# rebots-online/InstantIR

Measured on AMD Instinct MI355X. Metric: denoising steps/sec at 1024x1024 (InstantIR step: previewer UNet + LCM + Aggregator + UNet, CFG), higher is better.
Workload: dtype f16 (fp32 accumulate)

## Files before the change

### include/instantir_hip.h

```cpp
#ifndef INSTANTIR_HIP_H
#define INSTANTIR_HIP_H

#include <stdint.h>

#ifdef __cplusplus
extern "C" {
#endif

#define IIR_ABI_VERSION 1

#define IIR_EPI_PLAIN 0
#define IIR_EPI_GEGLU 1
#define IIR_EPI_SFT 2
#define IIR_EPI_XATTN 3
#define IIR_ACT_NONE 0
#define IIR_ACT_SILU 1
#define IIR_ACT_GELU 2
#define IIR_ACT_QUICKGELU 3


#define IIR_DT_F16 0
#define IIR_DT_BF16 1

typedef struct iir_attn_kv {
// ... 11 lines not shown
    const void* rowbias; int64_t ldrb; int32_t rows_per_rb;
    const void* res; int64_t ldr;
    int32_t epi, act;
    float out_scale;
    int32_t tile;
    const void* prefetch;
    int64_t prefetch_bytes;
    void* splitk_ws;
    int64_t splitk_ws_bytes;
    void* Ct; int64_t ldct;
    int32_t tr_from;
    int32_t dtype;
    int32_t c_f32;
    const void* wscale;
    void* ln_stats_out;
    const void* ln_stats_in;
    int32_t ln_parts, ln_part_cols;
    float ln_eps;
    const void* ln_colsum;
    void* gn_stats_out;
    const iir_attn_kv* xattn_kv;
    int32_t xattn_tq;
    int32_t a_fp8;
    float a_scale;
    int32_t c_fp8;
} iir_gemm_desc;

int iir_gemm_f16(const iir_gemm_desc* d, void* stream);
int iir_gemm_ln_parts(int32_t M, int32_t N, int32_t K);
int iir_gemm_pick_tile(int32_t M, int32_t N, int32_t K, int32_t paired);
int iir_gemm_resolve_tile(const iir_gemm_desc* d);
int iir_gemm_gn_supported(int32_t M, int32_t N, int32_t K, int32_t is_conv);
int iir_gemm_fp8_out_supported(int32_t M, int32_t N, int32_t K, int32_t paired);
int64_t iir_gemm_splitk_workspace_bytes(int32_t M, int32_t N);
int iir_gemm_uses_splitk(int32_t M, int32_t N, int32_t K, int64_t ws_bytes);
int iir_gemm_tile_bn(int32_t tile);

typedef struct iir_conv_desc {
    const void* X; int64_t ldx;
    int32_t R, H, Wd, Cin;
    const void* Wt;
    void* Y; int64_t ldy;
    int32_t Cout, ksize, stride, upsample;
    const void* bias;
    const void* rowbias; int64_t ldrb; int32_t rows_per_rb;
    const void* res; int64_t ldr;
    int32_t epi, act;
    float out_scale;
    int32_t tile;
    const void* zero_page;
    int64_t x_img_stride;
    int32_t y_img_rows;
    int32_t res_img_rows;
    int32_t pad_mode;
    const void* prefetch;
    int64_t prefetch_bytes;
    void* splitk_ws;
    int64_t splitk_ws_bytes;
    int32_t dtype;
    void* gn_stats_out;
} iir_conv_desc;

int iir_conv2d_nhwc_f16(const iir_conv_desc* c, void* stream);

typedef struct iir_attn_desc {
    const void* Q; int64_t ldq, q_batch_stride;
    void* O; int64_t ldo, o_batch_stride;
    int32_t batch, heads, Tq, nseg;
    float scale;
    iir_attn_kv kv[2];
    int32_t causal;
    int32_t q_prescaled;
    int32_t o_fp8;
} iir_attn_desc;

int iir_attention_d64_f16(const iir_attn_desc* a, void* stream);
int iir_attention_d64_ident_f16(const iir_attn_desc* a, int32_t ident_from, void* stream);

int iir_attention_f16(const iir_attn_desc* a, int32_t head_dim, void* stream);

int iir_groupnorm_nhwc_f16(const void* X, int64_t ldx, void* Y, int64_t ldy, int32_t R, int32_t HW, int32_t C,
                           int32_t groups, const void* gamma, const void* beta, float eps, int32_t silu,
                           void* workspace, int64_t workspace_bytes, void* stream);
int iir_groupnorm_from_partials(const void* partials, int64_t ldp, const void* X, int64_t ldx, void* Y, int64_t ldy, int32_t R,
                                int32_t HW, int32_t C, int32_t groups, const void* gamma, const void* beta, float eps, int32_t silu,
                                void* workspace, int64_t workspace_bytes, int32_t dtype, void* stream);
int iir_groupnorm_nhwc(const void* X, int64_t ldx, void* Y, int64_t ldy, int32_t R, int32_t HW, int32_t C,
                       int32_t groups, const void* gamma, const void* beta, float eps, int32_t silu,
                       void* workspace, int64_t workspace_bytes, int32_t dtype, void* stream);
int64_t iir_groupnorm_workspace_bytes(int32_t R, int32_t groups);

int iir_layernorm_f16(const void* X, int64_t ldx, void* Y, int64_t ldy, int32_t rows, int32_t C, const void* gamma,
                      const void* beta, float eps, const void* shift, const void* scale, int64_t ldmod,
                      int32_t rows_per_mod, int32_t transposed, int32_t tr_rows, int64_t tr_bstride, void* stream);

typedef struct iir_adaln_job {
    const void* X; void* Y; const void* shift; const void* scale;
    int64_t ldx, ldy;
    int32_t C, transposed;
} iir_adaln_job;
int iir_adaln_batch_f16(const iir_adaln_job* jobs_dev, int32_t njobs, int32_t rows, int32_t max_C, float eps, int64_t ldmod,
                        int32_t rows_per_mod, int32_t tr_rows, int64_t tr_bstride, void* stream);

int iir_softmax_rows_f16(void* X, int64_t ld, int32_t rows, int32_t cols, void* stream);
int iir_softmax_rows_f32(const float* S, int64_t lds, void* P, int64_t ldp, int32_t rows, int32_t cols, int32_t dtype, void* stream);

int iir_sinusoid_f16(const float* vals, int32_t n_vals, int32_t rows, int32_t dim, void* out, int64_t ldo,
                     int32_t col_off, void* stream);
int iir_silu_f16(const void* x, void* y, int64_t n, void* stream);

int iir_copy_add_f16(const void* src, int64_t lds, void* dst, int64_t ldd, int64_t dst_off, int64_t M, int32_t C,
                     const void* add, int64_t lda, const float* add_scale, int32_t rows_per_scale, void* stream);

#define IIR_FREEU_SLABS 16
int64_t iir_freeu_partials_bytes(int64_t rows, int32_t H, int32_t W, int32_t C);
int iir_freeu_stats_f16(const void* skip, int64_t lds, const void* add, int64_t lda, const float* add_scale, int64_t rows,
                        int32_t H, int32_t W, int32_t C, float* partials, int64_t partials_bytes, void* stream);
int iir_freeu_concat_f16(const void* x, int64_t ldx, int32_t cx, const void* mid_add, int64_t ldm, const void* skip, int64_t lds,
                         int32_t cs, const void* add, int64_t lda, const float* add_scale, int64_t rows, int32_t H, int32_t W,
                         float b, float s, const float* partials, int64_t partials_bytes, void* cat, int64_t ldc,
                         int64_t cat_off, void* stream);

int iir_pack_latent(const float* x, int32_t B, int32_t C, int32_t HW, void* out, int64_t ldo, int32_t rep, float scale,
                    void* stream);
int iir_unpack_latent(const void* in, int64_t ldi, int32_t R, int32_t C, int32_t HW, float* out, void* stream);
int iir_pack_latent_t(const float* x, int32_t B, int32_t C, int32_t HW, void* out, int64_t ldo, int32_t rep, float scale,
                      int32_t dtype, void* stream);
int iir_unpack_latent_t(const void* in, int64_t ldi, int32_t R, int32_t C, int32_t HW, float* out, int32_t dtype, void* stream);
int iir_pack_latent_dscale(const float* x, int32_t B, int32_t C, int32_t HW, void* out, int64_t ldo, int32_t rep, const float* scale,
                           int32_t dtype, void* stream);

int iir_sched_step(const void* eps_nhwc, int64_t lde, int32_t B, int32_t C, int32_t HW, int32_t cfg, const float* coef,
                   const float* x, const float* noise, float* prev, float* x0_out, float* eps_out,
                   const float* eps_factor, void* stream);
int iir_sched_step_hist(const void* eps_nhwc, int64_t lde, int32_t B, int32_t C, int32_t HW, int32_t cfg, const float* coef,
                        const float* x, const float* noise, float* hist, float* prev, float* x0_out, const float* eps_factor,
                        void* stream);
int iir_cfg_rescale_factor(const void* eps_nhwc, int64_t lde, int32_t B, int32_t C, int32_t HW, const float* coef,
                           float guidance_rescale, float* factor, void* stream);
int iir_sched_step_pag(const void* eps_nhwc, int64_t lde, int32_t B, int32_t C, int32_t HW, int32_t cfg, const float* coef,
                       const float* pag_scale, const float* x, const float* noise, float* prev, float* x0_out, float* eps_out,
                       const float* eps_factor, void* stream);
int iir_sched_step_hist_pag(const void* eps_nhwc, int64_t lde, int32_t B, int32_t C, int32_t HW, int32_t cfg, const float* coef,
                            const float* pag_scale, const float* x, const float* noise, float* hist, float* prev, float* x0_out,
                            const float* eps_factor, void* stream);
int iir_cfg_rescale_factor_pag(const void* eps_nhwc, int64_t lde, int32_t B, int32_t C, int32_t HW, const float* coef,
                               const float* pag_scale, float guidance_rescale, float* factor, void* stream);
int iir_copy_segments(const void* jobs, int32_t njobs, int64_t max_units, void* stream);

int iir_lcm_step(const void* eps_nhwc, int64_t lde, int32_t B, int32_t rep, int32_t C, int32_t HW, const float* coef,
                 const float* x, void* out_nhwc, int64_t ldo, float* out_nchw, void* stream);

int iir_sched_step_f32(const float* eps, const float* x, const float* noise, const float* coef, int64_t n, float* prev,
                       float* x0_out, void* stream);
int iir_axpby_f32(const float* x, const float* y, const float* coef, int64_t n, float* out, void* stream);
int iir_sched_step_hist_f32(const float* eps, const float* x, const float* noise, const float* coef, float* hist, int64_t n,
                            float* prev, float* x0_out, void* stream);

int iir_prefetch(const void* p, int64_t bytes, int32_t blocks, void* stream);

int iir_blend_tiles_f32(const float* a, float* b, int32_t planes, int32_t Ha, int32_t Wa, int32_t Hb, int32_t Wb,
                        int32_t extent, int32_t vertical, void* stream);

#define IIR_COLORFIX_SLABS 64
int64_t iir_colorfix_workspace_bytes(int32_t B, int32_t C, int32_t H, int32_t W);
int iir_colorfix_wavelet_f32(const float* content, const float* style, float* out, int32_t B, int32_t C, int32_t H, int32_t W,
                             void* ws, int64_t ws_bytes, void* stream);
int iir_colorfix_adain_f32(const float* content, const float* style, float* out, int32_t B, int32_t C, int32_t H, int32_t W,
                           void* ws, int64_t ws_bytes, void* stream);

int iir_transpose_f16(const void* in, int64_t ldi, int32_t rows, int32_t cols, void* out, int64_t ldo, int32_t rows_pad,
                      void* stream);
void* iir_timing_event_create(void);
void iir_timing_event_destroy(void* event);
int iir_timing_arm(void* start_event, void* stop_event);
int iir_timing_elapsed_us(void* start_event, void* stop_event, float* us);

int iir_abi_version(void);

#ifdef __cplusplus
}
#endif
#endif
```

### instantir_amd/csrc/freeu.hip

```cpp
#include "common.h"
#include "../../include/instantir_hip.h"

namespace {

constexpr int NSLAB = IIR_FREEU_SLABS;
constexpr int NSUM = 7;
constexpr int CB = 64;
constexpr int RL = 32;
constexpr int CONCAT_ROWS = 256;

__device__ __forceinline__ void phase_sc(int n, int N, float* s, float* c) {
    int m = 2 * n;
    if (m > N) m -= 2 * N;
    sincospif((float)m / (float)N, s, c);
}

__device__ __forceinline__ void pixel_trig(int p, int H, int W, float sc[6]) {
    const int h = p / W, w = p - h * W;
    const int HW = H * W;
    int n11 = h * W + w * H;
    if (n11 >= HW) n11 -= HW;
    phase_sc(h, H, &sc[1], &sc[0]);
    phase_sc(w, W, &sc[3], &sc[2]);
    phase_sc(n11, HW, &sc[5], &sc[4]);
}

__global__ __launch_bounds__(256) void freeu_stats_kernel(const f16* sk, long lds_, const f16* add, long lda, const float* add_scale,
                                                           int H, int W, int C, float* part) {
    __shared__ float red[RL][NSUM][CB];
    const int tid = threadIdx.x, oct = tid & 7, rl = tid >> 3;
    const int r = blockIdx.x / NSLAB, slab = blockIdx.x % NSLAB;
    const int HW = H * W;
    const int per = (HW + NSLAB - 1) / NSLAB;
    const int lo = min(slab * per, HW), hi = min(lo + per, HW);
    const int c0 = blockIdx.y * CB + oct * 8;
    const int cl = min(c0, C - 8);
    const float sc_r = add_scale ? add_scale[r] : 1.0f;
    float acc[NSUM][8];
#pragma unroll
    for (int k = 0; k < NSUM; ++k)
#pragma unroll
        for (int j = 0; j < 8; ++j) acc[k][j] = 0.0f;
    const int iters = (per + RL - 1) / RL;
    for (int it = 0; it < iters; ++it) {
        const int p = lo + it * RL + rl;
        const bool valid = p < hi;
        const int pl = min(p, HW - 1);
        const long m = (long)r * HW + pl;
        f16x8 v = *(const f16x8*)(sk + m * lds_ + cl);
        float t[8];
        if (add) {
            const f16x8 a = *(const f16x8*)(add + m * lda + cl);
#pragma unroll
            for (int j = 0; j < 8; ++j) t[j] = (float)v[j] + (float)a[j] * sc_r;
        } else {
#pragma unroll
            for (int j = 0; j < 8; ++j) t[j] = (float)v[j];
        }
#pragma unroll
        for (int j = 0; j < 8; ++j) t[j] = valid ? t[j] : 0.0f;
        float tr[6];
        pixel_trig(pl, H, W, tr);
#pragma unroll
        for (int j = 0; j < 8; ++j) {
            acc[0][j] += t[j];
#pragma unroll
            for (int k = 0; k < 6; ++k) acc[1 + k][j] += t[j] * tr[k];
        }
    }
#pragma unroll
    for (int k = 0; k < NSUM; ++k)
#pragma unroll
        for (int j = 0; j < 8; ++j) red[rl][k][oct * 8 + j] = acc[k][j];
    __syncthreads();
    for (int idx = tid; idx < NSUM * CB; idx += 256) {
        const int k = idx / CB, c = idx % CB;
        float s = 0.0f;
        for (int q = 0; q < RL; ++q) s += red[q][k][c];
        const int cg = blockIdx.y * CB + c;
        if (cg < C) part[(((long)r * NSLAB + slab) * NSUM + k) * C + cg] = s;
    }
}

__global__ __launch_bounds__(256) void freeu_concat_kernel(const f16* x, long ldx, int cx, const f16* mid, long ldm, const f16* sk,
                                                            long lds_, int cs, const f16* add, long lda, const float* add_scale,
                                                            int H, int W, float b, float s, const float* part, f16* cat,
                                                            long ldc, long cat_off) {
    __shared__ float coef[NSUM][CB];
    const int tid = threadIdx.x, oct = tid & 7, rl = tid >> 3;
    const int HW = H * W;
    const int ntile = (HW + CONCAT_ROWS - 1) / CONCAT_ROWS;
    const int r = blockIdx.x / ntile, p0 = (blockIdx.x % ntile) * CONCAT_ROWS;
    const int nbx = (cx + CB - 1) / CB;
    const float sc_r = add_scale ? add_scale[r] : 1.0f;
    if ((int)blockIdx.y < nbx) {
        const int c0 = blockIdx.y * CB + oct * 8;
        const int cl = min(c0, cx - 8);
        const int half = cx / 2;
#pragma unroll 4
        for (int i = 0; i < CONCAT_ROWS / RL; ++i) {
            const int p = p0 + i * RL + rl;
            const long m = (long)r * HW + min(p, HW - 1);
            const f16x8 v = *(const f16x8*)(x + m * ldx + cl);
            float t[8];
            if (mid) {
                const f16x8 a = *(const f16x8*)(mid + m * ldm + cl);
#pragma unroll
                for (int j = 0; j < 8; ++j) t[j] = (float)v[j] + (float)a[j] * sc_r;
            } else {
#pragma unroll
                for (int j = 0; j < 8; ++j) t[j] = (float)v[j];
            }
            f16x8 o;
#pragma unroll
            for (int j = 0; j < 8; ++j) o[j] = (f16)(cl + j < half ? t[j] * b : t[j]);
            if (p < HW && c0 < cx) *(f16x8*)(cat + m * ldc + cat_off + c0) = o;
        }
        return;
    }
    const int cb = blockIdx.y - nbx;
    for (int idx = tid; idx < NSUM * CB; idx += 256) {
        const int k = idx / CB, c = idx % CB;
        const int cc = min(cb * CB + c, cs - 1);
        float a = 0.0f;
        for (int sl = 0; sl < NSLAB; ++sl) a += part[(((long)r * NSLAB + sl) * NSUM + k) * cs + cc];
        const bool keep = k == 0 || ((k == 1 || k == 2) && H > 1) || ((k == 3 || k == 4) && W > 1) || (k >= 5 && H > 1 && W > 1);
        coef[k][c] = keep ? a : 0.0f;
    }
    __syncthreads();
    const int c0 = cb * CB + oct * 8;
    const int cl = min(c0, cs - 8);
    float cf[NSUM][8];
#pragma unroll
    for (int k = 0; k < NSUM; ++k)
#pragma unroll
        for (int j = 0; j < 8; ++j) cf[k][j] = coef[k][oct * 8 + j];
    const float ks = (s - 1.0f) / (float)HW;
#pragma unroll 4
    for (int i = 0; i < CONCAT_ROWS / RL; ++i) {
        const int p = p0 + i * RL + rl;
        const int pl = min(p, HW - 1);
        const long m = (long)r * HW + pl;
        const f16x8 v = *(const f16x8*)(sk + m * lds_ + cl);
        float t[8];
        if (add) {
            const f16x8 a = *(const f16x8*)(add + m * lda + cl);
#pragma unroll
            for (int j = 0; j < 8; ++j) t[j] = (float)v[j] + (float)a[j] * sc_r;
        } else {
#pragma unroll
            for (int j = 0; j < 8; ++j) t[j] = (float)v[j];
        }
        if (ks != 0.0f) {
            float tr[6];
            pixel_trig(pl, H, W, tr);
#pragma unroll
            for (int j = 0; j < 8; ++j) {
                float corr = cf[0][j];
#pragma unroll
                for (int k = 0; k < 6; ++k) corr = corr + cf[1 + k][j] * tr[k];
                t[j] = t[j] + ks * corr;
            }
        }
        f16x8 o;
#pragma unroll
        for (int j = 0; j < 8; ++j) o[j] = (f16)t[j];
        if (p < HW && c0 < cs) *(f16x8*)(cat + m * ldc + cat_off + cx + c0) = o;
    }
}

long planes(int64_t rows, int32_t H, int32_t W) {
    if (rows <= 0 || H < 1 || W < 1 || H > 65535 || W > 65535) return -1;
    const int64_t HW = (int64_t)H * W;
    if (HW > (1 << 26) || rows % HW) return -1;
    const int64_t R = rows / HW;
    if (R > 65535) return -1;
    return (long)R;
}

}

extern "C" int64_t iir_freeu_partials_bytes(int64_t rows, int32_t H, int32_t W, int32_t C) {
    const long R = planes(rows, H, W);
    if (R < 0 || C <= 0 || C % 8) return -1;
    return (int64_t)R * NSLAB * NSUM * C * (int64_t)sizeof(float);
}

extern "C" int iir_freeu_stats_f16(const void* skip, int64_t lds, const void* add, int64_t lda, const float* add_scale, int64_t rows,
                                   int32_t H, int32_t W, int32_t C, float* partials, int64_t partials_bytes, void* stream) {
    (void)hipGetLastError();
    const long R = planes(rows, H, W);
    if (!skip || !partials || R < 0 || C <= 0 || C % 8 || lds % 8 || lds < C) return IIR_EINVAL;
    if (add && (lda % 8 || lda < C)) return IIR_EINVAL;
    if (partials_bytes < iir_freeu_partials_bytes(rows, H, W, C)) return IIR_EINVAL;
    hipLaunchKernelGGL(freeu_stats_kernel, dim3((unsigned)(R * NSLAB), (C + CB - 1) / CB), dim3(256), 0, (hipStream_t)stream,
                       (const f16*)skip, (long)lds, (const f16*)add, (long)lda, add_scale, H, W, C, partials);
    return iir_launch_status();
}

extern "C" int iir_freeu_concat_f16(const void* x, int64_t ldx, int32_t cx, const void* mid_add, int64_t ldm, const void* skip,
                                    int64_t lds, int32_t cs, const void* add, int64_t lda, const float* add_scale, int64_t rows,
                                    int32_t H, int32_t W, float b, float s, const float* partials, int64_t partials_bytes,
                                    void* cat, int64_t ldc, int64_t cat_off, void* stream) {
    (void)hipGetLastError();
    const long R = planes(rows, H, W);
    if (!x || !skip || !cat || !partials || R < 0) return IIR_EINVAL;
    if (cx <= 0 || cx % 8 || cs <= 0 || cs % 8 || ldx % 8 || ldx < cx || lds % 8 || lds < cs) return IIR_EINVAL;
    if (mid_add && (ldm % 8 || ldm < cx)) return IIR_EINVAL;
    if (add && (lda % 8 || lda < cs)) return IIR_EINVAL;
    if (ldc % 8 || cat_off < 0 || cat_off % 8 || ldc < cat_off + cx + cs) return IIR_EINVAL;
    if (partials_bytes < iir_freeu_partials_bytes(rows, H, W, cs)) return IIR_EINVAL;
    const int64_t HW = (int64_t)H * W;
    const int ntile = (int)((HW + CONCAT_ROWS - 1) / CONCAT_ROWS);
    hipLaunchKernelGGL(freeu_concat_kernel, dim3((unsigned)(R * ntile), (cx + CB - 1) / CB + (cs + CB - 1) / CB), dim3(256), 0,
                       (hipStream_t)stream, (const f16*)x, (long)ldx, cx, (const f16*)mid_add, (long)ldm, (const f16*)skip, (long)lds,
                       cs, (const f16*)add, (long)lda, add_scale, H, W, b, s, partials, (f16*)cat, (long)ldc, (long)cat_off);
    return iir_launch_status();
}
```

### instantir_amd/csrc/norm.hip

```cpp
#include "common.h"
#include "../../include/instantir_hip.h"

namespace {

constexpr int GN_MAXC = 2560;
constexpr int GN_MIN_PIX = 8;

__device__ __forceinline__ void chan_merge(float& n, float& mean, float& m2, float nb, float mb, float m2b) {
    if (nb <= 0.f) return;
    const float tot = n + nb, d = mb - mean;
    mean += d * (nb / tot);
    m2 += m2b + d * d * (n * nb / tot);
    n = tot;
}

template <typename E>
__global__ __launch_bounds__(256) void gn_stats_kernel(const f16* Xp, long ldx, int HW, int C, int G, int pix_per_slab,
                                                       float* part ) {
    using E8 = typename ET<E>::x8;
    const E* X = (const E*)Xp;
    __shared__ float cmean[2048], cm2[2048];
    __shared__ float chmean[GN_MAXC], chm2[GN_MAXC];
    const int r = blockIdx.y, slab = blockIdx.x, nslab = gridDim.x;
    const int nchunk = C >> 3;
    const int p0 = slab * pix_per_slab;
    const int p1 = min(HW, p0 + pix_per_slab);
    const E* base = X + (long)r * HW * ldx;
    const int lanes_c = nchunk < 256 ? nchunk : 256;
    const int prows = 256 / lanes_c;
    const int tc = threadIdx.x % lanes_c, tp = threadIdx.x / lanes_c;
    for (int c0 = 0; c0 < nchunk; c0 += lanes_c) {
        const int ch = c0 + tc;
        if (tp < prows && ch < nchunk) {
            float s[8], q[8], k0[8];
#pragma unroll
            for (int j = 0; j < 8; ++j) { s[j] = 0.f; q[j] = 0.f; k0[j] = 0.f; }
            int p = p0 + tp, cnt = 0;
            if (p < p1) {
                const E8 v = *(const E8*)(base + (long)p * ldx + ch * 8);
#pragma unroll
                for (int j = 0; j < 8; ++j) k0[j] = (float)v[j];
            }
            for (; p + 3 * prows < p1; p += 4 * prows) {
                E8 v[4];
#pragma unroll
                for (int u = 0; u < 4; ++u) v[u] = *(const E8*)(base + (long)(p + u * prows) * ldx + ch * 8);
#pragma unroll
                for (int u = 0; u < 4; ++u)
#pragma unroll
                    for (int j = 0; j < 8; ++j) { const float f = (float)v[u][j] - k0[j]; s[j] += f; q[j] += f * f; }
                cnt += 4;
            }
            for (; p < p1; p += prows) {
                const E8 v = *(const E8*)(base + (long)p * ldx + ch * 8);
#pragma unroll
                for (int j = 0; j < 8; ++j) { const float f = (float)v[j] - k0[j]; s[j] += f; q[j] += f * f; }
                cnt += 1;
            }
            const float inv = cnt > 0 ? 1.0f / (float)cnt : 0.f;
#pragma unroll
            for (int j = 0; j < 8; ++j) {
                cmean[(tp * lanes_c + tc) * 8 + j] = k0[j] + s[j] * inv;
                cm2[(tp * lanes_c + tc) * 8 + j] = fmaxf(q[j] - s[j] * s[j] * inv, 0.f);
            }
        }
        __syncthreads();
        for (int c = threadIdx.x; c < lanes_c * 8 && c0 * 8 + c < C; c += 256) {
            float n = 0.f, mean = 0.f, m2 = 0.f;
            for (int t = 0; t < prows; ++t) {
                const int first = p0 + t;
                const float nt = first < p1 ? (float)((p1 - first + prows - 1) / prows) : 0.f;
                chan_merge(n, mean, m2, nt, cmean[t * lanes_c * 8 + c], cm2[t * lanes_c * 8 + c]);
            }
            chmean[c0 * 8 + c] = mean; chm2[c0 * 8 + c] = m2;
        }
        __syncthreads();
    }
    const int cpg = C / G;
    const float npix = (float)(p1 - p0);
    for (int gi = threadIdx.x; gi < G; gi += 256) {
        float n = 0.f, mean = 0.f, m2 = 0.f;
        for (int c = gi * cpg; c < (gi + 1) * cpg; ++c) chan_merge(n, mean, m2, npix, chmean[c], chm2[c]);
        float* o = part + (((long)r * nslab + slab) * G + gi) * 2;
        o[0] = mean; o[1] = m2;
    }
}

__global__ __launch_bounds__(256) void gn_finalize_kernel(const float* part, int nslab, int G, int HW, int pix_per_slab, int cpg,
                                                          float eps, float* stat , int gblocks) {
    __shared__ float sn[256], smean[256], sm2[256];
    const int r = blockIdx.x / gblocks, gb = blockIdx.x - r * gblocks;
    const int g8 = threadIdx.x & 7, sl = threadIdx.x >> 3;
    const int gi = gb * 8 + g8;
    constexpr int MAXS = 8;
    float n = 0.f, mean = 0.f, m2 = 0.f;
    if (gi < G) {
        const float* base = part + ((long)r * nslab * G + gi) * 2;
        float2 a[MAXS];
#pragma unroll
        for (int k = 0; k < MAXS; ++k) {
            const int s_ = min(sl + k * 32, nslab - 1);
            a[k] = *(const float2*)(base + (long)s_ * G * 2);
        }
#pragma unroll
        for (int k = 0; k < MAXS; ++k) {
            const int s_ = sl + k * 32;
            if (s_ < nslab) {
                const int p0 = s_ * pix_per_slab, p1 = min(HW, p0 + pix_per_slab);
                chan_merge(n, mean, m2, (float)(p1 - p0) * (float)cpg, a[k].x, a[k].y);
            }
        }
    }
    sn[threadIdx.x] = n; smean[threadIdx.x] = mean; sm2[threadIdx.x] = m2;
    __syncthreads();
    if (threadIdx.x < 64) {
        const int seg = threadIdx.x >> 3;
        float tn = 0.f, tm = 0.f, tq = 0.f;
#pragma unroll
        for (int l = 0; l < 4; ++l) {
            const int src = (seg * 4 + l) * 8 + g8;
            chan_merge(tn, tm, tq, sn[src], smean[src], sm2[src]);
        }
        n = tn; mean = tm; m2 = tq;
    }
    __syncthreads();
    if (threadIdx.x < 64) { sn[threadIdx.x] = n; smean[threadIdx.x] = mean; sm2[threadIdx.x] = m2; }
    __syncthreads();
    if (threadIdx.x < 8 && gi < G) {
        float tn = 0.f, tm = 0.f, tq = 0.f;
#pragma unroll
        for (int sgm = 0; sgm < 8; ++sgm) chan_merge(tn, tm, tq, sn[sgm * 8 + g8], smean[sgm * 8 + g8], sm2[sgm * 8 + g8]);
        stat[((long)r * G + gi) * 2] = tm;
        stat[((long)r * G + gi) * 2 + 1] = rsqrtf(tq / tn + eps);
    }
}

__global__ __launch_bounds__(256) void gn_finalize_cols_kernel(const float2* part, long ldp, int slabs_per_img, int G, int cpg, float eps,
                                                               float* stat ) {
    __shared__ float red[256];
    const int r = blockIdx.x / G, gi = blockIdx.x - r * G;
    const int n = slabs_per_img * cpg;
    constexpr int MAXP = 20;
    float2 a[MAXP];
    const float2* base = part + (long)r * slabs_per_img * ldp + gi * cpg;
#pragma unroll
    for (int k = 0; k < MAXP; ++k) {
        const int i = min((int)threadIdx.x + k * 256, n - 1);
        const int sl = i / cpg, c = i - sl * cpg;
        a[k] = base[(long)sl * ldp + c];
    }
    auto block_sum = [&](float v) {
        red[threadIdx.x] = v;
        __syncthreads();
#pragma unroll
        for (int o = 128; o > 0; o >>= 1) {
            if ((int)threadIdx.x < o) red[threadIdx.x] += red[threadIdx.x + o];
            __syncthreads();
        }
        const float t = red[0];
        __syncthreads();
        return t;
    };
    float sm = 0.f;
#pragma unroll
    for (int k = 0; k < MAXP; ++k) sm += ((int)threadIdx.x + k * 256 < n) ? a[k].x : 0.f;
    const float mean = block_sum(sm) / (float)n;
    float q = 0.f;
#pragma unroll
    for (int k = 0; k < MAXP; ++k) {
        const float d = a[k].x - mean;
        q += ((int)threadIdx.x + k * 256 < n) ? fmaf(64.0f * d, d, a[k].y) : 0.f;
    }
    const float m2 = block_sum(q);
    if (threadIdx.x == 0) {
        stat[((long)r * G + gi) * 2] = mean;
        stat[((long)r * G + gi) * 2 + 1] = rsqrtf(m2 / ((float)n * 64.0f) + eps);
    }
}

template <typename E>
__global__ __launch_bounds__(256) void gn_apply_kernel(const f16* Xp, long ldx, f16* Yp, long ldy, int HW, int C, int G,
                                                       int pix_per_blk, const float* stat, const f16* gammap,
                                                       const f16* betap, int silu) {
    using E8 = typename ET<E>::x8;
    const E* X = (const E*)Xp; E* Y = (E*)Yp; const E* gamma = (const E*)gammap; const E* beta = (const E*)betap;
    const int r = blockIdx.y;
    const int cpg = C / G;
    const int nchunk = C >> 3;
    const int lanes_c = nchunk < 256 ? nchunk : 256;
    const int prows = 256 / lanes_c;
    const int tc = threadIdx.x % lanes_c, tp = threadIdx.x / lanes_c;
    if (tp >= prows) return;
    const int p0 = blockIdx.x * pix_per_blk;
    const int p1 = min(HW, p0 + pix_per_blk);
    const E* xb = X + (long)r * HW * ldx;
    E* yb = Y + (long)r * HW * ldy;
    const float* st = stat + (long)r * G * 2;
    for (int ch = tc; ch < nchunk; ch += lanes_c) {
        float a[8], b[8];
        const E8 gm = *(const E8*)(gamma + ch * 8), bt = *(const E8*)(beta + ch * 8);
#pragma unroll
        for (int j = 0; j < 8; ++j) {
            const int gi = (ch * 8 + j) / cpg;
            const float mean = st[gi * 2], rstd = st[gi * 2 + 1];
            a[j] = rstd * (float)gm[j];
            b[j] = (float)bt[j] - mean * a[j];
        }
        for (int p = p0 + tp; p < p1; p += prows) {
            const E8 v = *(const E8*)(xb + (long)p * ldx + ch * 8);
            E8 o;
#pragma unroll
            for (int j = 0; j < 8; ++j) {
                float f = fmaf((float)v[j], a[j], b[j]);
                if (silu) f = silu_f(f);
                o[j] = (E)f;
            }
            *(E8*)(yb + (long)p * ldy + ch * 8) = o;
        }
    }
}

__device__ __forceinline__ void ln_row(const f16* X, long ldx, f16* Y, long ldy, int row, int C, const f16* gamma,
                                       const f16* beta, float eps, const f16* shift, const f16* scale, long ldmod,
                                       int rows_per_mod, int transposed, int tr_rows, long tr_bstride) {
    const int lane = threadIdx.x & 63;
    const int nchunk = C >> 3;
    constexpr int MAXK = GN_MAXC / 8 / 64;
    f16x8 v[MAXK];
    float s = 0.f;
    const f16* x = X + (long)row * ldx;
#pragma unroll
    for (int k = 0; k < MAXK; ++k) v[k] = *(const f16x8*)(x + min(lane + k * 64, nchunk - 1) * 8);
#pragma unroll
    for (int k = 0; k < MAXK; ++k) {
        const int ch = lane + k * 64;
        if (ch < nchunk) {
#pragma unroll
            for (int j = 0; j < 8; ++j) s += (float)v[k][j];
        }
    }
    const float mean = wave_sum(s) / (float)C;
    float q = 0.f;
#pragma unroll
    for (int k = 0; k < MAXK; ++k) {
        const int ch = lane + k * 64;
        if (ch < nchunk) {
#pragma unroll
            for (int j = 0; j < 8; ++j) { const float d = (float)v[k][j] - mean; q += d * d; }
        }
    }
    const float rstd = rsqrtf(wave_sum(q) / (float)C + eps);
    const f16* sh = shift ? shift + (long)(row / rows_per_mod) * ldmod : nullptr;
    const f16* sc = scale ? scale + (long)(row / rows_per_mod) * ldmod : nullptr;
#pragma unroll
    for (int k = 0; k < MAXK; ++k) {
        const int ch = lane + k * 64;
        if (ch < nchunk) {
            f16x8 o;
            f16x8 gm, bt, s8, c8;
            if (gamma) gm = *(const f16x8*)(gamma + ch * 8);
            if (beta) bt = *(const f16x8*)(beta + ch * 8);
            if (sh) { s8 = *(const f16x8*)(sh + ch * 8); c8 = *(const f16x8*)(sc + ch * 8); }
#pragma unroll
            for (int j = 0; j < 8; ++j) {
                float f = ((float)v[k][j] - mean) * rstd;
                if (gamma) f *= (float)gm[j];
                if (beta) f += (float)bt[j];
                if (sh) f = f * (1.0f + (float)c8[j]) + (float)s8[j];
                o[j] = (f16)f;
            }
            if (transposed == 2) {
                *(long*)((char*)Y + (long)row * ldy + ch * 8) = iir_fp8x8(o);
            } else if (!transposed) {
                *(f16x8*)(Y + (long)row * ldy + ch * 8) = o;
            } else {
                const long col = (long)(row / tr_rows) * tr_bstride + (row % tr_rows);
#pragma unroll
                for (int j = 0; j < 8; ++j) Y[(long)(ch * 8 + j) * ldy + col] = o[j];
            }
        }
    }
}

__global__ __launch_bounds__(256) void ln_kernel(const f16* X, long ldx, f16* Y, long ldy, int rows, int C, const f16* gamma,
                                                 const f16* beta, float eps, const f16* shift, const f16* scale, long ldmod,
                                                 int rows_per_mod, int transposed, int tr_rows, long tr_bstride) {
    const int row = blockIdx.x * 4 + (threadIdx.x >> 6);
    if (row >= rows) return;
    ln_row(X, ldx, Y, ldy, row, C, gamma, beta, eps, shift, scale, ldmod, rows_per_mod, transposed, tr_rows, tr_bstride);
}

__global__ __launch_bounds__(256) void adaln_batch_kernel(const iir_adaln_job* jobs, int rows, float eps, long ldmod,
                                                          int rows_per_mod, int tr_rows, long tr_bstride) {
    const int row = blockIdx.x * 4 + (threadIdx.x >> 6);
    if (row >= rows) return;
    const iir_adaln_job j = jobs[blockIdx.y];
    ln_row((const f16*)j.X, j.ldx, (f16*)j.Y, j.ldy, row, j.C, nullptr, nullptr, eps, (const f16*)j.shift, (const f16*)j.scale,
           ldmod, rows_per_mod, j.transposed, tr_rows, tr_bstride);
}

__global__ __launch_bounds__(256) void softmax_rows_kernel(f16* X, long ld, int cols) {
    __shared__ float red[4];
// ... 10 lines not shown
        const int ch = threadIdx.x + k * 256;
        if (ch < nchunk) {
#pragma unroll
            for (int j = 0; j < 8; ++j) mx = fmaxf(mx, (float)v[k][j]);
        }
    }
    mx = wave_max(mx);
    if (lane == 0) red[wv] = mx;
    __syncthreads();
    mx = fmaxf(fmaxf(red[0], red[1]), fmaxf(red[2], red[3]));
    __syncthreads();
    float e[MAXK][8];
    float sum = 0.f;
#pragma unroll
    for (int k = 0; k < MAXK; ++k) {
        const int ch = threadIdx.x + k * 256;
        if (ch < nchunk) {
#pragma unroll
            for (int j = 0; j < 8; ++j) { e[k][j] = __expf((float)v[k][j] - mx); sum += e[k][j]; }
        }
    }
    sum = wave_sum(sum);
    if (lane == 0) red[wv] = sum;
    __syncthreads();
    const float inv = 1.0f / (red[0] + red[1] + red[2] + red[3]);
#pragma unroll
    for (int k = 0; k < MAXK; ++k) {
        const int ch = threadIdx.x + k * 256;
        if (ch < nchunk) {
            f16x8 o;
#pragma unroll
            for (int j = 0; j < 8; ++j) o[j] = (f16)(e[k][j] * inv);
            *(f16x8*)(x + ch * 8) = o;
        }
    }
}

template <typename E>
__global__ __launch_bounds__(256) void softmax_rows_f32_kernel(const float* S, long lds, f16* Pp, long ldp, int cols) {
    using E4 = typename ET<E>::x4;
    __shared__ float red[4];
    const float* x = S + (long)blockIdx.x * lds;
    E* y = (E*)Pp + (long)blockIdx.x * ldp;
    const int nchunk = cols >> 2;
    const int lane = threadIdx.x & 63, wv = threadIdx.x >> 6;
    constexpr int MAXK = 16;
    f32x4 v[MAXK];
    float mx = -INFINITY;
#pragma unroll
    for (int k = 0; k < MAXK; ++k) v[k] = *(const f32x4*)(x + min((int)threadIdx.x + k * 256, nchunk - 1) * 4);
#pragma unroll
    for (int k = 0; k < MAXK; ++k) {
        const int ch = threadIdx.x + k * 256;
        if (ch < nchunk) mx = fmaxf(fmaxf(mx, fmaxf(v[k][0], v[k][1])), fmaxf(v[k][2], v[k][3]));
    }
    mx = wave_max(mx);
    if (lane == 0) red[wv] = mx;
    __syncthreads();
    mx = fmaxf(fmaxf(red[0], red[1]), fmaxf(red[2], red[3]));
    __syncthreads();
    float sum = 0.f;
#pragma unroll
    for (int k = 0; k < MAXK; ++k) {
        const int ch = threadIdx.x + k * 256;
        if (ch < nchunk) {
#pragma unroll
            for (int j = 0; j < 4; ++j) { v[k][j] = __expf(v[k][j] - mx); sum += v[k][j]; }
        }
    }
    sum = wave_sum(sum);
    if (lane == 0) red[wv] = sum;
    __syncthreads();
    const float inv = 1.0f / (red[0] + red[1] + red[2] + red[3]);
#pragma unroll
    for (int k = 0; k < MAXK; ++k) {
        const int ch = threadIdx.x + k * 256;
        if (ch < nchunk) {
            E4 o;
#pragma unroll
            for (int j = 0; j < 4; ++j) o[j] = (E)(v[k][j] * inv);
            *(E4*)(y + ch * 4) = o;
        }
    }
}

}

extern "C" int iir_softmax_rows_f32(const float* S, int64_t lds, void* P, int64_t ldp, int32_t rows, int32_t cols, int32_t dtype,
                                    void* stream) {
    (void)hipGetLastError();
    if (!S || !P || rows <= 0 || cols <= 0 || cols % 4 || cols > 16384 || lds % 4 || ldp % 4) return IIR_EINVAL;
    if (dtype == IIR_DT_BF16) hipLaunchKernelGGL(softmax_rows_f32_kernel<bf16>, dim3(rows), dim3(256), 0, (hipStream_t)stream, S, (long)lds, (f16*)P, (long)ldp, cols);
    else if (dtype == IIR_DT_F16) hipLaunchKernelGGL(softmax_rows_f32_kernel<f16>, dim3(rows), dim3(256), 0, (hipStream_t)stream, S, (long)lds, (f16*)P, (long)ldp, cols);
    else return IIR_EINVAL;
    return iir_launch_status();
}

extern "C" int iir_softmax_rows_f16(void* X, int64_t ld, int32_t rows, int32_t cols, void* stream) {
    (void)hipGetLastError();
    if (!X || rows <= 0 || cols <= 0 || cols % 8 || cols > 16384 || ld % 8) return IIR_EINVAL;
    hipLaunchKernelGGL(softmax_rows_kernel, dim3(rows), dim3(256), 0, (hipStream_t)stream, (f16*)X, (long)ld, cols);
    return iir_launch_status();
}

extern "C" int iir_groupnorm_nhwc(const void* X, int64_t ldx, void* Y, int64_t ldy, int32_t R, int32_t HW, int32_t C,
                                  int32_t groups, const void* gamma, const void* beta, float eps, int32_t silu,
                                  void* workspace, int64_t workspace_bytes, int32_t dtype, void* stream) {
    (void)hipGetLastError();
    if (!X || !Y || !gamma || !beta || !workspace) return IIR_EINVAL;
    if (C % 8 || C > GN_MAXC || groups <= 0 || groups > 64 || C % groups || ldx % 8 || ldy % 8) return IIR_EINVAL;
    if (R <= 0 || HW <= 0 || (dtype != IIR_DT_F16 && dtype != IIR_DT_BF16)) return IIR_EINVAL;
    int nslab = (HW + GN_MIN_PIX - 1) / GN_MIN_PIX;
    const int want = (1024 + R - 1) / R;
    if (nslab > want) nslab = want;
    if (nslab > 256) nslab = 256;
    if (nslab < 1) nslab = 1;
    const int pps = (HW + nslab - 1) / nslab;
    nslab = (HW + pps - 1) / pps;
    const int64_t part_floats = (int64_t)R * nslab * groups * 2;
    if ((part_floats + (int64_t)R * groups * 2) * 4 > workspace_bytes) return IIR_EINVAL;
    float* part = (float*)workspace;
    float* stat = part + part_floats;
    const hipStream_t st = (hipStream_t)stream;
    int nblk = (1024 + R - 1) / R;
    int ppb = (HW + nblk - 1) / nblk; if (ppb < GN_MIN_PIX) ppb = GN_MIN_PIX;
    nblk = (HW + ppb - 1) / ppb;
    if (dtype == IIR_DT_BF16) hipLaunchKernelGGL(gn_stats_kernel<bf16>, dim3(nslab, R), dim3(256), 0, st, (const f16*)X, (long)ldx, HW, C, groups, pps, part);
    else hipLaunchKernelGGL(gn_stats_kernel<f16>, dim3(nslab, R), dim3(256), 0, st, (const f16*)X, (long)ldx, HW, C, groups, pps, part);
    const int gblocks = (groups + 7) / 8;
    hipLaunchKernelGGL(gn_finalize_kernel, dim3(R * gblocks), dim3(256), 0, st, (const float*)part, nslab, groups, HW, pps, C / groups, eps, stat, gblocks);
    if (dtype == IIR_DT_BF16) hipLaunchKernelGGL(gn_apply_kernel<bf16>, dim3(nblk, R), dim3(256), 0, st, (const f16*)X, (long)ldx, (f16*)Y, (long)ldy, HW, C, groups, ppb, (const float*)stat, (const f16*)gamma, (const f16*)beta, silu);
    else hipLaunchKernelGGL(gn_apply_kernel<f16>, dim3(nblk, R), dim3(256), 0, st, (const f16*)X, (long)ldx, (f16*)Y, (long)ldy, HW, C, groups, ppb, (const float*)stat, (const f16*)gamma, (const f16*)beta, silu);
    return iir_launch_status();
}

extern "C" int iir_groupnorm_from_partials(const void* partials, int64_t ldp, const void* X, int64_t ldx, void* Y, int64_t ldy, int32_t R,
                                           int32_t HW, int32_t C, int32_t groups, const void* gamma, const void* beta, float eps,
                                           int32_t silu, void* workspace, int64_t workspace_bytes, int32_t dtype, void* stream) {
    (void)hipGetLastError();
    if (!partials || !X || !Y || !gamma || !beta || !workspace || (uintptr_t)partials % 8) return IIR_EINVAL;
    if (C % 8 || C > GN_MAXC || groups <= 0 || groups > 64 || C % groups || ldx % 8 || ldy % 8 || ldp < C) return IIR_EINVAL;
    if (R <= 0 || HW <= 0 || HW % 64 || (dtype != IIR_DT_F16 && dtype != IIR_DT_BF16)) return IIR_EINVAL;
    const int slabs = HW / 64, cpg = C / groups;
    if ((long)slabs * cpg > 20 * 256) return IIR_EINVAL;
    if ((int64_t)R * groups * 2 * 4 > workspace_bytes) return IIR_EINVAL;
    float* stat = (float*)workspace;
    const hipStream_t st = (hipStream_t)stream;
    hipLaunchKernelGGL(gn_finalize_cols_kernel, dim3(R * groups), dim3(256), 0, st, (const float2*)partials, (long)ldp, slabs, groups, cpg, eps, stat);
    int nblk = (1024 + R - 1) / R;
    int ppb = (HW + nblk - 1) / nblk; if (ppb < GN_MIN_PIX) ppb = GN_MIN_PIX;
    nblk = (HW + ppb - 1) / ppb;
    if (dtype == IIR_DT_BF16) hipLaunchKernelGGL(gn_apply_kernel<bf16>, dim3(nblk, R), dim3(256), 0, st, (const f16*)X, (long)ldx, (f16*)Y, (long)ldy, HW, C, groups, ppb, (const float*)stat, (const f16*)gamma, (const f16*)beta, silu);
    else hipLaunchKernelGGL(gn_apply_kernel<f16>, dim3(nblk, R), dim3(256), 0, st, (const f16*)X, (long)ldx, (f16*)Y, (long)ldy, HW, C, groups, ppb, (const float*)stat, (const f16*)gamma, (const f16*)beta, silu);
    return iir_launch_status();
}

extern "C" int iir_groupnorm_nhwc_f16(const void* X, int64_t ldx, void* Y, int64_t ldy, int32_t R, int32_t HW, int32_t C,
                                      int32_t groups, const void* gamma, const void* beta, float eps, int32_t silu,
                                      void* workspace, int64_t workspace_bytes, void* stream) {
    return iir_groupnorm_nhwc(X, ldx, Y, ldy, R, HW, C, groups, gamma, beta, eps, silu, workspace, workspace_bytes, IIR_DT_F16, stream);
}

extern "C" int64_t iir_groupnorm_workspace_bytes(int32_t R, int32_t groups) { return (int64_t)R * 257 * groups * 2 * 4; }

extern "C" int iir_layernorm_f16(const void* X, int64_t ldx, void* Y, int64_t ldy, int32_t rows, int32_t C, const void* gamma,
                                 const void* beta, float eps, const void* shift, const void* scale, int64_t ldmod,
                                 int32_t rows_per_mod, int32_t transposed, int32_t tr_rows, int64_t tr_bstride, void* stream) {
    (void)hipGetLastError();
    if (!X || !Y || rows <= 0 || C % 8 || C > GN_MAXC || ldx % 8) return IIR_EINVAL;
    if ((shift == nullptr) != (scale == nullptr)) return IIR_EINVAL;
    if (shift && (rows_per_mod <= 0 || ldmod % 8)) return IIR_EINVAL;
    if (transposed < 0 || transposed > 2) return IIR_EINVAL;
    if (transposed != 1 && ldy % 8) return IIR_EINVAL;
    if (transposed == 1 && tr_rows <= 0) return IIR_EINVAL;
    hipLaunchKernelGGL(ln_kernel, dim3((rows + 3) / 4), dim3(256), 0, (hipStream_t)stream, (const f16*)X, (long)ldx, (f16*)Y,
                       (long)ldy, rows, C, (const f16*)gamma, (const f16*)beta, eps, (const f16*)shift, (const f16*)scale,
                       (long)ldmod, rows_per_mod, transposed, tr_rows, (long)tr_bstride);
    return iir_launch_status();
}

extern "C" int iir_adaln_batch_f16(const iir_adaln_job* jobs_dev, int32_t njobs, int32_t rows, int32_t max_C, float eps,
                                   int64_t ldmod, int32_t rows_per_mod, int32_t tr_rows, int64_t tr_bstride, void* stream) {
    (void)hipGetLastError();
    if (!jobs_dev || njobs <= 0 || njobs > 65535 || rows <= 0 || rows_per_mod <= 0) return IIR_EINVAL;
    if (max_C <= 0 || max_C > GN_MAXC || max_C % 8) return IIR_EINVAL;
    hipLaunchKernelGGL(adaln_batch_kernel, dim3((rows + 3) / 4, njobs), dim3(256), 0, (hipStream_t)stream, jobs_dev, rows, eps,
                       (long)ldmod, rows_per_mod, tr_rows, (long)tr_bstride);
    return iir_launch_status();
}
```

### instantir_amd/csrc/pointwise.hip

```cpp
#include "common.h"
#include "../../include/instantir_hip.h"

namespace {

__global__ void sinusoid_kernel(const float* vals, int n_vals, int rows, int dim, f16* out, long ldo, int col_off) {
    const int half = dim >> 1;
    const int idx = blockIdx.x * blockDim.x + threadIdx.x;
    const int total = rows * n_vals * half;
    if (idx >= total) return;
    const int k = idx % half;
    const int v = (idx / half) % n_vals;
    const int r = idx / (half * n_vals);
    const float w = expf(-9.210340371976184f * (float)k / (float)half);
    const float a = vals[r * n_vals + v] * w;
    f16* o = out + (long)r * ldo + col_off + v * dim;
    o[k] = (f16)cosf(a);
    o[half + k] = (f16)sinf(a);
}

__global__ void silu_kernel(const f16* x, f16* y, long n8) {
    const long i = (long)blockIdx.x * blockDim.x + threadIdx.x;
    if (i >= n8) return;
    const f16x8 v = *(const f16x8*)(x + i * 8);
    f16x8 o;
#pragma unroll
    for (int j = 0; j < 8; ++j) o[j] = (f16)silu_f((float)v[j]);
    *(f16x8*)(y + i * 8) = o;
}

__global__ void copy_add_kernel(const f16* src, long lds_, f16* dst, long ldd, long dst_off, long M, int C, const f16* add,
                                long lda, const float* add_scale, int rows_per_scale) {
    const int nchunk = C >> 3;
    const long i = (long)blockIdx.x * blockDim.x + threadIdx.x;
    if (i >= M * nchunk) return;
    const long m = i / nchunk;
    const int ch = (int)(i % nchunk);
    f16x8 v = *(const f16x8*)(src + m * lds_ + ch * 8);
    if (add) {
        const f16x8 a = *(const f16x8*)(add + m * lda + ch * 8);
        const float s = add_scale ? add_scale[m / rows_per_scale] : 1.0f;
#pragma unroll
        for (int j = 0; j < 8; ++j) v[j] = (f16)((float)v[j] + (float)a[j] * s);
    }
    *(f16x8*)(dst + m * ldd + dst_off + ch * 8) = v;
}

template <typename E>
__global__ void pack_latent_kernel(const float* x, int B, int C, int HW, E* out, long ldo, int rep, float scale) {
    const long i = (long)blockIdx.x * blockDim.x + threadIdx.x;
    if (i >= (long)B * HW) return;
    const int b = (int)(i / HW), p = (int)(i % HW);
    for (int c = 0; c < C; ++c) {
        const E v = (E)(x[((long)b * C + c) * HW + p] * scale);
        for (int k = 0; k < rep; ++k) out[((long)(k * B + b) * HW + p) * ldo + c] = v;
    }
}

template <typename E>
__global__ void unpack_latent_kernel(const E* in, long ldi, int R, int C, int HW, float* out) {
    const long i = (long)blockIdx.x * blockDim.x + threadIdx.x;
    if (i >= (long)R * HW) return;
    const int r = (int)(i / HW), p = (int)(i % HW);
    for (int c = 0; c < C; ++c) out[((long)r * C + c) * HW + p] = (float)in[((long)r * HW + p) * ldi + c];
}

template <bool PAG>
__global__ __launch_bounds__(1024) void cfg_rescale_kernel(const f16* eps_nhwc, long lde, int B, int C, int HW, const float* coef,
                                                           const float* pag_s, float phi, float* factor) {
    __shared__ double red[4][16];
    const int b = blockIdx.x;
    const float g = coef[0];
    const float ps = PAG ? *pag_s : 0.f;
    double st = 0., st2 = 0., sc = 0., sc2 = 0.;
    for (int p = threadIdx.x; p < HW; p += blockDim.x)
        for (int c = 0; c < C; ++c) {
            const float u = (float)eps_nhwc[((long)b * HW + p) * lde + c];
            const float t = (float)eps_nhwc[((long)(B + b) * HW + p) * lde + c];
            float e = u + g * (t - u);
            if (PAG && ps != 0.f) e = e + ps * (t - (float)eps_nhwc[((long)(2 * B + b) * HW + p) * lde + c]);
            st += t; st2 += (double)t * t; sc += e; sc2 += (double)e * e;
        }
    double v[4] = {st, st2, sc, sc2};
    const int lane = threadIdx.x & 63, wv = threadIdx.x >> 6;
    for (int k = 0; k < 4; ++k) {
        for (int o = 32; o > 0; o >>= 1) v[k] += __shfl_xor(v[k], o, 64);
        if (lane == 0) red[k][wv] = v[k];
    }
    __syncthreads();
    if (threadIdx.x == 0) {
        const int nw = blockDim.x >> 6;
        double s[4] = {0., 0., 0., 0.};
        for (int k = 0; k < 4; ++k)
            for (int w = 0; w < nw; ++w) s[k] += red[k][w];
        const double n = (double)C * HW;
        const double var_t = (s[1] - s[0] * s[0] / n) / (n - 1.), var_c = (s[3] - s[2] * s[2] / n) / (n - 1.);
        factor[b] = (float)((double)phi * sqrt(var_t / var_c) + (1. - (double)phi));
    }
}

template <bool PAG>
__device__ __forceinline__ float guided_eps(const f16* eps_nhwc, long lde, int B, int HW, int cfg, float g, float ps,
                                            const float* eps_factor, int b, int p, int c) {
    float e;
    if (cfg) {
        const float u = (float)eps_nhwc[((long)b * HW + p) * lde + c];
        const float t = (float)eps_nhwc[((long)(B + b) * HW + p) * lde + c];
        e = u + g * (t - u);
        if (PAG && ps != 0.f) e = e + ps * (t - (float)eps_nhwc[((long)(2 * B + b) * HW + p) * lde + c]);
        if (eps_factor) e *= eps_factor[b];
    } else {
        e = (float)eps_nhwc[((long)b * HW + p) * lde + c];
        if (PAG && ps != 0.f) e = e + ps * (e - (float)eps_nhwc[((long)(B + b) * HW + p) * lde + c]);
    }
    return e;
}

template <bool PAG>
__global__ void sched_step_kernel(const f16* eps_nhwc, long lde, int B, int C, int HW, int cfg, const float* coef,
                                  const float* pag_s, const float* x, const float* noise, float* prev, float* x0_out,
                                  float* eps_out, const float* eps_factor) {
    const long i = (long)blockIdx.x * blockDim.x + threadIdx.x;
    if (i >= (long)B * HW) return;
    const int b = (int)(i / HW), p = (int)(i % HW);
    const float g = coef[0], sb = coef[1], sa = coef[2], k0 = coef[3], k1 = coef[4], k2 = coef[5], k3 = coef[6];
    const float ps = PAG ? *pag_s : 0.f;
    for (int c = 0; c < C; ++c) {
        const long o = ((long)b * C + c) * HW + p;
// ... 38 lines not shown
    for (int j = threadIdx.y; j < 32; j += blockDim.y) {
        const int c = bx + j, r = by + threadIdx.x;
        if (c < cols && r < rows_pad) out[(long)c * ldo + r] = tile[threadIdx.x][j];
    }
}

template <typename E>
__global__ void pack_latent_dscale_kernel(const float* x, int B, int C, int HW, E* out, long ldo, int rep, const float* scale_dev) {
    const long i = (long)blockIdx.x * blockDim.x + threadIdx.x;
    if (i >= (long)B * HW) return;
    const float scale = *scale_dev;
    const int b = (int)(i / HW), p = (int)(i % HW);
    for (int c = 0; c < C; ++c) {
        const E v = (E)(x[((long)b * C + c) * HW + p] * scale);
        for (int k = 0; k < rep; ++k) out[((long)(k * B + b) * HW + p) * ldo + c] = v;
    }
}

template <bool PAG>
__global__ void sched_step_hist_kernel(const f16* eps_nhwc, long lde, int B, int C, int HW, int cfg, const float* coef,
                                       const float* pag_s, const float* x, const float* noise, float* hist, float* prev,
                                       float* x0_out, const float* eps_factor) {
    const long i = (long)blockIdx.x * blockDim.x + threadIdx.x;
    if (i >= (long)B * HW) return;
    const int b = (int)(i / HW), p = (int)(i % HW);
    const float g = coef[0], sb = coef[1], sa = coef[2], k0 = coef[3], k1 = coef[4], k2 = coef[5], k3 = coef[6], kh = coef[7];
    const float ps = PAG ? *pag_s : 0.f;
    for (int c = 0; c < C; ++c) {
        const long o = ((long)b * C + c) * HW + p;
        const float e = guided_eps<PAG>(eps_nhwc, lde, B, HW, cfg, g, ps, eps_factor, b, p, c);
        const float xv = x[o];
        const float x0 = (xv - sb * e) / sa;
        float pv = k0 * x0 + k1 * xv;
        if (k2 != 0.f) pv = pv + k2 * e;
        if (kh != 0.f) pv = pv + kh * hist[o];
        if (noise && k3 != 0.f) pv = pv + k3 * noise[o];
        prev[o] = pv;
        hist[o] = x0;
        if (x0_out) x0_out[o] = x0;
    }
}

__global__ void copy_segments_kernel(const long long* jobs) {
    const long long* jb = jobs + 3 * blockIdx.y;
    const long n = (long)jb[2];
    const uint4* src = (const uint4*)jb[0];
    uint4* dst = (uint4*)jb[1];
    for (long i = (long)blockIdx.x * blockDim.x + threadIdx.x; i < n; i += (long)gridDim.x * blockDim.x) dst[i] = src[i];
}

inline int nblk(long n, int t) { return (int)((n + t - 1) / t); }

}

extern "C" int iir_sinusoid_f16(const float* vals, int32_t n_vals, int32_t rows, int32_t dim, void* out, int64_t ldo,
                                int32_t col_off, void* stream) {
    (void)hipGetLastError();
    if (!vals || !out || n_vals <= 0 || rows <= 0 || dim <= 0 || dim % 2) return IIR_EINVAL;
    const int total = rows * n_vals * (dim / 2);
    hipLaunchKernelGGL(sinusoid_kernel, dim3(nblk(total, 256)), dim3(256), 0, (hipStream_t)stream, vals, n_vals, rows, dim,
                       (f16*)out, (long)ldo, col_off);
    return iir_launch_status();
}

extern "C" int iir_silu_f16(const void* x, void* y, int64_t n, void* stream) {
    (void)hipGetLastError();
    if (!x || !y || n <= 0 || n % 8) return IIR_EINVAL;
    hipLaunchKernelGGL(silu_kernel, dim3(nblk(n / 8, 256)), dim3(256), 0, (hipStream_t)stream, (const f16*)x, (f16*)y, n / 8);
    return iir_launch_status();
}

extern "C" int iir_copy_add_f16(const void* src, int64_t lds, void* dst, int64_t ldd, int64_t dst_off, int64_t M, int32_t C,
                                const void* add, int64_t lda, const float* add_scale, int32_t rows_per_scale, void* stream) {
    (void)hipGetLastError();
    if (!src || !dst || M <= 0 || C <= 0 || C % 8 || lds % 8 || ldd % 8 || dst_off % 8) return IIR_EINVAL;
    if (add && (lda % 8)) return IIR_EINVAL;
    if (add_scale && rows_per_scale <= 0) return IIR_EINVAL;
    hipLaunchKernelGGL(copy_add_kernel, dim3(nblk(M * (C / 8), 256)), dim3(256), 0, (hipStream_t)stream, (const f16*)src,
                       (long)lds, (f16*)dst, (long)ldd, (long)dst_off, (long)M, C, (const f16*)add, (long)lda, add_scale,
                       rows_per_scale);
    return iir_launch_status();
}

extern "C" int iir_pack_latent_t(const float* x, int32_t B, int32_t C, int32_t HW, void* out, int64_t ldo, int32_t rep,
                                 float scale, int32_t dtype, void* stream) {
    (void)hipGetLastError();
    if (!x || !out || B <= 0 || C <= 0 || HW <= 0 || rep <= 0 || ldo < C) return IIR_EINVAL;
    if (dtype == IIR_DT_BF16) hipLaunchKernelGGL(pack_latent_kernel<bf16>, dim3(nblk((long)B * HW, 256)), dim3(256), 0, (hipStream_t)stream, x, B, C, HW, (bf16*)out, (long)ldo, rep, scale);
    else if (dtype == IIR_DT_F16) hipLaunchKernelGGL(pack_latent_kernel<f16>, dim3(nblk((long)B * HW, 256)), dim3(256), 0, (hipStream_t)stream, x, B, C, HW, (f16*)out, (long)ldo, rep, scale);
    else return IIR_EINVAL;
    return iir_launch_status();
}

extern "C" int iir_pack_latent(const float* x, int32_t B, int32_t C, int32_t HW, void* out, int64_t ldo, int32_t rep,
                               float scale, void* stream) {
    return iir_pack_latent_t(x, B, C, HW, out, ldo, rep, scale, IIR_DT_F16, stream);
}

extern "C" int iir_pack_latent_dscale(const float* x, int32_t B, int32_t C, int32_t HW, void* out, int64_t ldo, int32_t rep,
                                      const float* scale, int32_t dtype, void* stream) {
    (void)hipGetLastError();
    if (!x || !out || !scale || B <= 0 || C <= 0 || HW <= 0 || rep <= 0 || ldo < C) return IIR_EINVAL;
    if (dtype != IIR_DT_F16 && dtype != IIR_DT_BF16) return IIR_EINVAL;
    if (dtype == IIR_DT_BF16) hipLaunchKernelGGL(pack_latent_dscale_kernel<bf16>, dim3(nblk((long)B * HW, 256)), dim3(256), 0, (hipStream_t)stream, x, B, C, HW, (bf16*)out, (long)ldo, rep, scale);
    else hipLaunchKernelGGL(pack_latent_dscale_kernel<f16>, dim3(nblk((long)B * HW, 256)), dim3(256), 0, (hipStream_t)stream, x, B, C, HW, (f16*)out, (long)ldo, rep, scale);
    return iir_launch_status();
}

extern "C" int iir_unpack_latent_t(const void* in, int64_t ldi, int32_t R, int32_t C, int32_t HW, float* out, int32_t dtype,
                                   void* stream) {
    (void)hipGetLastError();
    if (!in || !out || R <= 0 || C <= 0 || HW <= 0 || ldi < C) return IIR_EINVAL;
    if (dtype == IIR_DT_BF16) hipLaunchKernelGGL(unpack_latent_kernel<bf16>, dim3(nblk((long)R * HW, 256)), dim3(256), 0, (hipStream_t)stream, (const bf16*)in, (long)ldi, R, C, HW, out);
    else if (dtype == IIR_DT_F16) hipLaunchKernelGGL(unpack_latent_kernel<f16>, dim3(nblk((long)R * HW, 256)), dim3(256), 0, (hipStream_t)stream, (const f16*)in, (long)ldi, R, C, HW, out);
    else return IIR_EINVAL;
    return iir_launch_status();
}

extern "C" int iir_unpack_latent(const void* in, int64_t ldi, int32_t R, int32_t C, int32_t HW, float* out, void* stream) {
    return iir_unpack_latent_t(in, ldi, R, C, HW, out, IIR_DT_F16, stream);
}

extern "C" int iir_cfg_rescale_factor(const void* eps_nhwc, int64_t lde, int32_t B, int32_t C, int32_t HW, const float* coef,
                                      float guidance_rescale, float* factor, void* stream) {
    (void)hipGetLastError();
    if (!eps_nhwc || !coef || !factor || B <= 0 || C <= 0 || HW <= 0 || lde < C || (long)C * HW < 2) return IIR_EINVAL;
    hipLaunchKernelGGL(cfg_rescale_kernel<false>, dim3(B), dim3(1024), 0, (hipStream_t)stream, (const f16*)eps_nhwc, (long)lde, B, C,
                       HW, coef, (const float*)nullptr, guidance_rescale, factor);
    return iir_launch_status();
}

extern "C" int iir_cfg_rescale_factor_pag(const void* eps_nhwc, int64_t lde, int32_t B, int32_t C, int32_t HW, const float* coef,
                                          const float* pag_scale, float guidance_rescale, float* factor, void* stream) {
    if (!eps_nhwc || !coef || !pag_scale || !factor || B <= 0 || C <= 0 || HW <= 0 || lde < C || (long)C * HW < 2) return IIR_EINVAL;
    (void)hipGetLastError();
    hipLaunchKernelGGL(cfg_rescale_kernel<true>, dim3(B), dim3(1024), 0, (hipStream_t)stream, (const f16*)eps_nhwc, (long)lde, B, C,
                       HW, coef, pag_scale, guidance_rescale, factor);
    return iir_launch_status();
}

extern "C" int iir_sched_step(const void* eps_nhwc, int64_t lde, int32_t B, int32_t C, int32_t HW, int32_t cfg,
                              const float* coef, const float* x, const float* noise, float* prev, float* x0_out,
                              float* eps_out, const float* eps_factor, void* stream) {
    (void)hipGetLastError();
    if (!eps_nhwc || !coef || !x || !prev || B <= 0 || C <= 0 || HW <= 0 || lde < C) return IIR_EINVAL;
    if (eps_factor && !cfg) return IIR_EINVAL;
    hipLaunchKernelGGL(sched_step_kernel<false>, dim3(nblk((long)B * HW, 256)), dim3(256), 0, (hipStream_t)stream,
                       (const f16*)eps_nhwc, (long)lde, B, C, HW, cfg, coef, (const float*)nullptr, x, noise, prev, x0_out, eps_out,
                       eps_factor);
    return iir_launch_status();
}

extern "C" int iir_sched_step_pag(const void* eps_nhwc, int64_t lde, int32_t B, int32_t C, int32_t HW, int32_t cfg,
                                  const float* coef, const float* pag_scale, const float* x, const float* noise, float* prev,
                                  float* x0_out, float* eps_out, const float* eps_factor, void* stream) {
    if (!eps_nhwc || !coef || !pag_scale || !x || !prev || B <= 0 || C <= 0 || HW <= 0 || lde < C) return IIR_EINVAL;
    if (eps_factor && !cfg) return IIR_EINVAL;
    (void)hipGetLastError();
    hipLaunchKernelGGL(sched_step_kernel<true>, dim3(nblk((long)B * HW, 256)), dim3(256), 0, (hipStream_t)stream,
                       (const f16*)eps_nhwc, (long)lde, B, C, HW, cfg, coef, pag_scale, x, noise, prev, x0_out, eps_out, eps_factor);
    return iir_launch_status();
}

extern "C" int iir_sched_step_hist(const void* eps_nhwc, int64_t lde, int32_t B, int32_t C, int32_t HW, int32_t cfg,
                                   const float* coef, const float* x, const float* noise, float* hist, float* prev, float* x0_out,
                                   const float* eps_factor, void* stream) {
// ... 174 lines not shown
```

### instantir_amd/engine.py

```python
from __future__ import annotations

import os

from typing import Dict, List, Optional

import torch

from . import ops, pag
from .config import UNetConfig
from .packing import conv_weight_nhwc, pair_rows
from .weights import skip_channels

F16 = torch.float16
CPAD = 64


class _NullOps:

    def __getattr__(self, name):
        return lambda *a, **k: None


class Arena:

# ... 7 lines not shown
    def reserve(self, n_elems):
        self.buf = torch.empty(n_elems, dtype=self.dtype, device=self.device)

    def alloc(self, rows, cols):
        n = (rows * cols + 127) // 128 * 128
        off = self.off
        self.off += n
        self.high = max(self.high, self.off)
        if self.buf is None:
            return torch.empty(rows, cols, dtype=self.dtype, device="meta")
        if self.off > self.buf.numel():
            raise RuntimeError("activation arena overflow (forward differs from its sizing run)")
        return self.buf[off:off + rows * cols].view(rows, cols)

    def mark(self):
        return self.off

    def release(self, m):
        self.off = m

    def reset(self):
        self.off = 0


def _merge_lora(sd: Dict[str, torch.Tensor], lora: Dict[str, torch.Tensor], scaling: float) -> Dict[str, torch.Tensor]:
    out = dict(sd)
    for k in lora:
        if not k.endswith(".lora_A.weight"):
            continue
        path = k[: -len(".lora_A.weight")]
        w = sd[path + ".weight"]
        dev = w.device
        if not w.is_cuda:
            raise RuntimeError("_merge_lora: weights must be on the GPU (the merge runs in the HIP library)")
        a, b = lora[k].to(dev), lora[path + ".lora_B.weight"].to(dev)
        r = a.shape[0]
        rp = (r + 63) // 64 * 64
        n_out = w.shape[0]
        kk = w.numel() // n_out
        bs = torch.zeros(n_out, rp, dtype=F16, device=dev)
        bs[:, :r] = (b.reshape(n_out, r).float() * scaling).to(F16)
        at = torch.zeros(kk, rp, dtype=F16, device=dev)
        at[:, :r] = a.reshape(r, kk).t().to(F16)
        w2 = w.reshape(n_out, kk).to(F16).contiguous()
        merged = torch.empty_like(w2)
        ops.gemm(bs, at, merged, res=w2)
        out[path + ".weight"] = merged.reshape(w.shape).to(w.dtype)
    return out


class _RecDict(dict):

    def __init__(self, base, note):
        super().__init__(base)
        self._note = note

    def __getitem__(self, k):
        self._note(k)
        return dict.__getitem__(self, k)


class _Net:

    def __init__(self, cfg: UNetConfig, sd: Dict[str, torch.Tensor], cross: bool, device, fp8_linear: bool = False):
        self.cfg = cfg
        self.cross = cross
        self.device = device
        self.fp8_linear = fp8_linear
        self.arena = Arena(device)
        self.o = ops
        self.w: Dict[str, torch.Tensor] = {}
        self._temb_slices: Dict[str, slice] = {}
        self._ada_slices: Dict[str, slice] = {}
        self.units: List[tuple] = []
        self._use_log: Optional[list] = None
        self._gnws = None
        self._skws = None
        self._warena = None
        self.inkernel_prefetch = True
        self.arena_gen = 0
        self.fuse_qkv = os.environ.get("IIR_FUSE_QKV", "1") != "0"
        self.ln_fold = os.environ.get("IIR_LN_FOLD", "1") != "0" and not fp8_linear
        self.gn_fuse = os.environ.get("IIR_GN_FUSE", "1") != "0"
        self.xattn_fuse = os.environ.get("IIR_XATTN_FUSE", "1") != "0"
        self.pag = None
        self.fp8_act = fp8_linear and os.environ.get("IIR_FP8_ACT", "1") != "0"
        self._pack_encoder(sd)

    def _t(self, sd, name):
        return sd[name].to(device=self.device, dtype=F16)

    def _qw(self, sd, name):
        f = ops.attn_q_factor(self.cfg.head_dim ** -0.5)
        return (sd[name].to(device=self.device, dtype=torch.float32) * f).to(F16)

    def _pack_linear(self, sd, path, dst=None):
        dst = dst or path
        self.w[dst + ".w"] = self._t(sd, path + ".weight").contiguous()
        if (path + ".bias") in sd:
            self.w[dst + ".b"] = self._t(sd, path + ".bias").contiguous()

    def _pack_conv3(self, sd, path, cin_pad=None):
        self.w[path + ".w"] = conv_weight_nhwc(self._t(sd, path + ".weight"), cin_pad)
        self.w[path + ".b"] = self._t(sd, path + ".bias").contiguous()

    def _pack_fold(self, dst, w32, sd, norm, bias=None, pair=None):
        f = ops.LnFold(w32, sd[norm + ".weight"].to(self.device), sd[norm + ".bias"].to(self.device), bias=bias, eps=1e-5, pair=pair)
        self.w[dst + ".lnw"], self.w[dst + ".lnb"], self.w[dst + ".lncs"] = f.w, f.bias, f.colsum

    def _pack_norm(self, sd, path):
        self.w[path + ".g"] = self._t(sd, path + ".weight").contiguous()
        self.w[path + ".b"] = self._t(sd, path + ".bias").contiguous()

    def _pack_resnet(self, sd, path, temb_list):
        self._pack_norm(sd, path + ".norm1")
        self._pack_conv3(sd, path + ".conv1")
        self._pack_norm(sd, path + ".norm2")
        self._pack_conv3(sd, path + ".conv2")
        temb_list.append((path, self._t(sd, path + ".time_emb_proj.weight"), self._t(sd, path + ".time_emb_proj.bias")))
        if (path + ".conv_shortcut.weight") in sd:
            w = self._t(sd, path + ".conv_shortcut.weight")
            self.w[path + ".conv_shortcut.w"] = w.reshape(w.shape[0], w.shape[1]).contiguous()
            self.w[path + ".conv_shortcut.b"] = self._t(sd, path + ".conv_shortcut.bias").contiguous()

    def _pack_transformer(self, sd, path, depth, ada_list):
        self._pack_norm(sd, path + ".norm")
        self._pack_linear(sd, path + ".proj_in")
        self._pack_linear(sd, path + ".proj_out")
        for k in range(depth):
            p = f"{path}.transformer_blocks.{k}"
            self._pack_norm(sd, p + ".norm1")
            self.w[p + ".attn1.qkv.w"] = torch.cat([self._qw(sd, p + ".attn1.to_q.weight"), self._t(sd, p + ".attn1.to_k.weight"),
                                                    self._t(sd, p + ".attn1.to_v.weight")], 0).contiguous()
            f32 = lambda n_: sd[n_].to(device=self.device, dtype=torch.float32)
            qf = ops.attn_q_factor(self.cfg.head_dim ** -0.5)
            if self.ln_fold:
                self._pack_fold(p + ".attn1.qkv", torch.cat([f32(p + ".attn1.to_q.weight") * qf, f32(p + ".attn1.to_k.weight"),
                                                             f32(p + ".attn1.to_v.weight")], 0), sd, p + ".norm1")
            self._pack_linear(sd, p + ".attn1.to_out.0")
            if self.cross:
                self._pack_norm(sd, p + ".norm2")
                if self.ln_fold:
                    self._pack_fold(p + ".attn2.to_q", f32(p + ".attn2.to_q.weight") * qf, sd, p + ".norm2")
                self.w[p + ".attn2.to_q.w"] = self._qw(sd, p + ".attn2.to_q.weight").contiguous()
                self._pack_linear(sd, p + ".attn2.to_k")
                self._pack_linear(sd, p + ".attn2.to_v")
                self._pack_linear(sd, p + ".attn2.to_out.0")
                pp = p + ".attn2.processor"
                self._pack_linear(sd, pp + ".to_k_ip")
                self._pack_linear(sd, pp + ".to_v_ip")
                for kv in ("k", "v"):
                    ada_list.append((f"{p}.{kv}", self._t(sd, f"{pp}.ln_{kv}_ip.linear.weight"), self._t(sd, f"{pp}.ln_{kv}_ip.linear.bias")))
            self._pack_norm(sd, p + ".norm3")
            w1, b1 = self._t(sd, p + ".ff.net.0.proj.weight"), self._t(sd, p + ".ff.net.0.proj.bias")
            n = w1.shape[0] // 2
            self.w[p + ".ff1.w"] = pair_rows(w1[:n], w1[n:])
            self.w[p + ".ff1.b"] = pair_rows(b1[:n], b1[n:])
            if self.ln_fold:
                self._pack_fold(p + ".ff1", f32(p + ".ff.net.0.proj.weight"), sd, p + ".norm3", bias=f32(p + ".ff.net.0.proj.bias"), pair=pair_rows)
            self._pack_linear(sd, p + ".ff.net.2", p + ".ff2")
            if self.fp8_linear:
                for key in ([p + ".attn1.qkv.w", p + ".attn1.to_out.0.w", p + ".ff1.w", p + ".ff2.w"]
                            + ([p + ".attn2.to_q.w", p + ".attn2.to_out.0.w"] if self.cross else [])):
                    self.w[key] = ops.Fp8Weight(*ops.quantize_fp8_rows(self.w[key]))
        if self.fp8_linear:
            for key in (path + ".proj_in.w", path + ".proj_out.w"):
# ... 46 lines not shown
            self._skws = torch.zeros(4096 + 256 * 128 * 160 * 4, dtype=torch.uint8, device=self.device)
        if first:
            self._use_log = []
            self.w = _RecDict(plain, lambda k: self._use_log.append(k))
        try:
            fn()
        finally:
            self.o = ops
            self.w = plain
        if first:
            self._consolidate_weights()
        self.arena.reserve(self.arena.high + 1024)
        self.arena.reset()

    def _consolidate_weights(self):
        order, seen, marks = [], set(), []
        for k in self._use_log:
            if isinstance(k, tuple):
                marks.append(len(order))
            elif k not in seen:
                seen.add(k)
                order.append(k)
        order += [k for k in self.w if k not in seen]
        order = [k for k in order if torch.is_tensor(self.w[k]) and self.w[k].dtype == F16]
        al = lambda n: (n + 127) // 128 * 128
        offs, tot = [], 0
        for k in order:
            offs.append(tot)
            tot += al(self.w[k].numel())
        arena = torch.empty(tot, dtype=F16, device=self.device)
        for k, off in zip(order, offs):
            t = self.w[k]
            v = arena[off:off + t.numel()].view(t.shape)
            v.copy_(t)
            self.w[k] = v
        self._warena = arena
        self.units = [None]
        self._use_log = None

    def _unit(self, name):
        if self._use_log is not None:
            self._use_log.append(("unit", name))

    import os as _os
    PF_MULT = float(_os.environ.get("IIR_PF_MULT", "1"))
    PF_LOOKAHEAD = int(_os.environ.get("IIR_PF_MB", "0")) << 20

    def _pf(self, wt):
        if not self.inkernel_prefetch or self._warena is None or self.o is not ops:
            return None
        base, end = self._warena.data_ptr(), self._warena.data_ptr() + self._warena.numel() * 2
        n = wt.numel() * 2
        lo = wt.data_ptr() + n + self.PF_LOOKAHEAD
        if lo < base or lo >= end or n < (256 << 10):
            return None
        return (lo, min(int(n * self.PF_MULT), end - lo))

    def _begin(self):
        self.arena.reset()

    def _gn_alloc(self, rows, hw, C, K, conv):
        if not self.gn_fuse or hw % 64 or self.arena.dtype != F16 or not ops.gn_supported(rows, C, K, conv):
            return None
        if (hw // 64) * (C // self.cfg.norm_groups) > ops.GN_PARTIALS_MAX:
            return None
        return self.arena.alloc(rows // 64 * C, 4).view(torch.float32).view(rows // 64, C, 2)

    @staticmethod
    def _gn_of(x):
        return getattr(x, "_gn_parts", None)

    def _resnet(self, path, x, R, H, W, temb_all, out=None, eps=1e-5):
        self._unit(path)
        o, w, A = self.o, self.w, self.arena
        HW = H * W
        cin = x.shape[1]
        cout = w[path + ".conv1.w"].shape[0]
        if out is None:
            out = A.alloc(R * HW, cout)
        p_out = self._gn_alloc(R * HW, HW, cout, 9 * cout, True) if self._skws is None else None
        m = A.mark()
        h = A.alloc(R * HW, cin)
        o.groupnorm(x, h, R, HW, w[path + ".norm1.g"], w[path + ".norm1.b"], eps, True, self.cfg.norm_groups, self._gnws,
                    partials=self._gn_of(x))
        h2 = A.alloc(R * HW, cout)
        p2 = self._gn_alloc(R * HW, HW, cout, 9 * cin, True) if self._skws is None else None
        o.conv2d(h.view(R, H, W, cin), w[path + ".conv1.w"], h2, bias=w[path + ".conv1.b"],
                 rowbias=temb_all[:, self._temb_slices[path]], rows_per_rb=HW, prefetch=self._pf(w[path + ".conv1.w"]),
                 splitk_ws=self._skws, gn_out=p2)
        h3 = A.alloc(R * HW, cout)
        o.groupnorm(h2, h3, R, HW, w[path + ".norm2.g"], w[path + ".norm2.b"], eps, True, self.cfg.norm_groups, self._gnws, partials=p2)
        if (path + ".conv_shortcut.w") in w:
            sc = A.alloc(R * HW, cout)
            o.gemm(x, w[path + ".conv_shortcut.w"], sc, bias=w[path + ".conv_shortcut.b"])
        else:
            sc = x
        o.conv2d(h3.view(R, H, W, cout), w[path + ".conv2.w"], out, bias=w[path + ".conv2.b"], res=sc,
                 prefetch=self._pf(w[path + ".conv2.w"]), splitk_ws=self._skws, gn_out=p_out)
        if p_out is not None:
            out._gn_parts = p_out
        A.release(m)
        return out

    def _tblock(self, p, h, R, T, heads, st, ada, lnst=None, last=False):
        self._unit(p)
        o, w, A = self.o, self.w, self.arena
        C = h.shape[1]
        M = R * T
        m = A.mark()
        fold = lnst is not None
        if self.fp8_act and not fold and C % 128 == 0 and isinstance(w[p + ".attn1.qkv.w"], ops.Fp8Weight) and h.dtype == F16:
            assert self.pag is None
            self._tblock_fp8(p, h, R, T, heads, st)
            A.release(m)
            return
        n = None if fold else A.alloc(M, C)
        qk = A.alloc(M, 2 * C)
        vt = A.alloc(C, M)
        if fold:
            wqkv = w[p + ".attn1.qkv.lnw"]
            o.gemm(h, wqkv, qk, bias=w[p + ".attn1.qkv.lnb"], prefetch=self._pf(wqkv), out_t=(vt, 2 * C),
                   ln_in=(lnst, w[p + ".attn1.qkv.lncs"], 1e-5))
        else:
            o.layernorm(h, n, w[p + ".norm1.g"], w[p + ".norm1.b"], 1e-5)
            wqkv = w[p + ".attn1.qkv.w"]
            if self.fuse_qkv:
                o.gemm(n, wqkv, qk, prefetch=self._pf(wqkv), out_t=(vt, 2 * C))
            else:
                o.gemm(n, wqkv[:2 * C], qk, prefetch=self._pf(wqkv))
                o.gemm(wqkv[2 * C:], n, vt)
        a = A.alloc(M, C)
        ident = self.pag[1] if self.pag is not None and (p + ".attn1") in self.pag[0] else 0
        o.attention(qk[:, :C], a, [(qk[:, C:], T, vt, T, T)], R, heads, T, q_prescaled=True, ident_from=ident)
        o.gemm(a, w[p + ".attn1.to_out.0.w"], h, bias=w[p + ".attn1.to_out.0.b"], res=h,
               prefetch=self._pf(w[p + ".attn1.to_out.0.w"]), ln_out=lnst)
        if self.cross:
            q = qk[:, :C]
            cfg = self.cfg
            nip, ipad = cfg.num_ip_tokens, (cfg.num_ip_tokens + 7) // 8 * 8
            kv = st["kv"][p]
            ipk, ipvt = kv["ipk"], kv["ipvt"]
            segs = [(kv["tk"], cfg.text_len, kv["tvt"], kv["tpad"], cfg.text_len), (ipk, nip, ipvt, ipad, nip)]
            wq = w[p + (".attn2.to_q.lnw" if fold else ".attn2.to_q.w")]
            fuse = (self.xattn_fuse and cfg.head_dim == 64 and C % 128 == 0 and T % 64 == 0 and cfg.text_len <= 80 and nip <= 64 and h.dtype == F16
                    and not isinstance(wq, ops.Fp8Weight))
            if not fold:
                o.layernorm(h, n, w[p + ".norm2.g"], w[p + ".norm2.b"], 1e-5)
            src = h if fold else n
            kw = dict(bias=w[p + ".attn2.to_q.lnb"], ln_in=(lnst, w[p + ".attn2.to_q.lncs"], 1e-5)) if fold else {}
            if fuse:
                o.gemm(src, wq, a, prefetch=self._pf(wq), epi=ops.EPI_XATTN, xattn=(segs, T), **kw)
            else:
                o.gemm(src, wq, q, prefetch=self._pf(wq), **kw)
                o.attention(q, a, segs, R, heads, T, q_prescaled=True)
            o.gemm(a, w[p + ".attn2.to_out.0.w"], h, bias=w[p + ".attn2.to_out.0.b"], res=h,
                   prefetch=self._pf(w[p + ".attn2.to_out.0.w"]), ln_out=lnst)
        f = A.alloc(M, 4 * C)
        if fold:
            o.gemm(h, w[p + ".ff1.lnw"], f, bias=w[p + ".ff1.lnb"], epi=ops.EPI_GEGLU, prefetch=self._pf(w[p + ".ff1.lnw"]),
                   ln_in=(lnst, w[p + ".ff1.lncs"], 1e-5))
        else:
            o.layernorm(h, n, w[p + ".norm3.g"], w[p + ".norm3.b"], 1e-5)
            o.gemm(n, w[p + ".ff1.w"], f, bias=w[p + ".ff1.b"], epi=ops.EPI_GEGLU, prefetch=self._pf(w[p + ".ff1.w"]))
        o.gemm(f, w[p + ".ff2.w"], h, bias=w[p + ".ff2.b"], res=h, prefetch=self._pf(w[p + ".ff2.w"]),
               splitk_ws=None if fold else self._skws, ln_out=None if last else lnst)
        A.release(m)

    def _tblock_fp8(self, p, h, R, T, heads, st):
        o, w, A, cfg = self.o, self.w, self.arena, self.cfg
        C, M = h.shape[1], R * T
        a8 = lambda rows, cols: A.alloc(rows, cols // 2).view(torch.uint8).view(rows, cols)
        n8 = a8(M, C)
        qk = A.alloc(M, 2 * C)
        vt = A.alloc(C, M)
        o.layernorm(h, n8, w[p + ".norm1.g"], w[p + ".norm1.b"], 1e-5)
        wqkv = w[p + ".attn1.qkv.w"]
        o.gemm_fp8(n8, wqkv, qk, prefetch=self._pf(wqkv), out_t=(vt, 2 * C))
        at8 = a8(M, C)
        o.attention(qk[:, :C], at8, [(qk[:, C:], T, vt, T, T)], R, heads, T, q_prescaled=True)
        o.gemm_fp8(at8, w[p + ".attn1.to_out.0.w"], h, bias=w[p + ".attn1.to_out.0.b"], res=h, prefetch=self._pf(w[p + ".attn1.to_out.0.w"]))
        if self.cross:
            q = qk[:, :C]
            nip, ipad = cfg.num_ip_tokens, (cfg.num_ip_tokens + 7) // 8 * 8
            kv = st["kv"][p]
            o.layernorm(h, n8, w[p + ".norm2.g"], w[p + ".norm2.b"], 1e-5)
            o.gemm_fp8(n8, w[p + ".attn2.to_q.w"], q, prefetch=self._pf(w[p + ".attn2.to_q.w"]))
            o.attention(q, at8, [(kv["tk"], cfg.text_len, kv["tvt"], kv["tpad"], cfg.text_len), (kv["ipk"], nip, kv["ipvt"], ipad, nip)],
                        R, heads, T, q_prescaled=True)
            o.gemm_fp8(at8, w[p + ".attn2.to_out.0.w"], h, bias=w[p + ".attn2.to_out.0.b"], res=h, prefetch=self._pf(w[p + ".attn2.to_out.0.w"]))
        o.layernorm(h, n8, w[p + ".norm3.g"], w[p + ".norm3.b"], 1e-5)
        if ops.fp8_out_supported(M, 8 * C, C, True):
            f8 = a8(M, 4 * C)
            o.gemm_fp8(n8, w[p + ".ff1.w"], f8, bias=w[p + ".ff1.b"], epi=ops.EPI_GEGLU, prefetch=self._pf(w[p + ".ff1.w"]))
            o.gemm_fp8(f8, w[p + ".ff2.w"], h, bias=w[p + ".ff2.b"], res=h, prefetch=self._pf(w[p + ".ff2.w"]))
        else:
            f = A.alloc(M, 4 * C)
            o.gemm_fp8(n8, w[p + ".ff1.w"], f, bias=w[p + ".ff1.b"], epi=ops.EPI_GEGLU, prefetch=self._pf(w[p + ".ff1.w"]))
            o.gemm(f, w[p + ".ff2.w"], h, bias=w[p + ".ff2.b"], res=h, prefetch=self._pf(w[p + ".ff2.w"]))

    def _transformer(self, path, x, depth, R, H, W, st, ada, out=None):
        o, w, A = self.o, self.w, self.arena
        C = x.shape[1]
        T = H * W
        if out is None:
            out = A.alloc(R * T, C)
        p_out = self._gn_alloc(R * T, T, C, C, False)
        m = A.mark()
        g = A.alloc(R * T, C)
        o.groupnorm(x, g, R, T, w[path + ".norm.g"], w[path + ".norm.b"], 1e-6, False, self.cfg.norm_groups, self._gnws,
                    partials=self._gn_of(x))
        h = A.alloc(R * T, C)
        lnst = None
        if self.ln_fold and depth > 0:
            parts = {ops.ln_parts(R * T, C, K) for K in (C, 4 * C)}
            if len(parts) == 1 and 0 not in parts:
                lnst = A.alloc(parts.pop() * R * T, 4).view(torch.float32).view(-1, R * T, 2)
        o.gemm(g, w[path + ".proj_in.w"], h, bias=w[path + ".proj_in.b"], ln_out=lnst)
        for k in range(depth):
            self._tblock(f"{path}.transformer_blocks.{k}", h, R, T, C // self.cfg.head_dim, st, ada, lnst, last=k == depth - 1)
        o.gemm(h, w[path + ".proj_out.w"], out, bias=w[path + ".proj_out.b"], res=x,
               gn_out=p_out if not isinstance(w[path + ".proj_out.w"], ops.Fp8Weight) else None)
        if p_out is not None and not isinstance(w[path + ".proj_out.w"], ops.Fp8Weight):
            out._gn_parts = p_out
        A.release(m)
        return out

    def _embeddings(self, t_dev, st):
        o, w, A, cfg = self.o, self.w, self.arena, self.cfg
        R = st["R"]
        c0, td = cfg.block_out_channels[0], cfg.time_embed_dim
        sin = A.alloc(R, c0)
        o.sinusoid(t_dev, sin, c0)
        e1 = A.alloc(R, td)
        o.gemm(sin, w["time_embedding.linear_1.w"], e1, bias=w["time_embedding.linear_1.b"], act=ops.ACT_SILU)
        emb = A.alloc(R, td)
        o.gemm(e1, w["time_embedding.linear_2.w"], emb, bias=w["time_embedding.linear_2.b"], res=st["aug_emb"])
        act = A.alloc(R, td)
        o.silu(emb, act)
        temb_all = A.alloc(R, w["temb_all.w"].shape[0])
        o.gemm(act, w["temb_all.w"], temb_all, bias=w["temb_all.b"])
        ada = None
        if "ada_all.w" in w:
            ada = st["ada"]
            o.gemm(act, w["ada_all.w"], ada, bias=w["ada_all.b"])
            nip = cfg.num_ip_tokens
            o.adaln_batch(st["ada_jobs"], st["ada_njobs"], R * nip, max(cfg.block_out_channels), ada.stride(0), nip, nip,
                          (nip + 7) // 8 * 8)
        return temb_all, ada

    def _aug_emb(self, text_embeds, time_ids):
        cfg, w = self.cfg, self.w
        R = text_embeds.shape[0]
        a = torch.zeros(R, cfg.add_embed_in, dtype=F16, device=self.device)
        a[:, :cfg.pooled_dim] = text_embeds.to(self.device, F16)
        ops.sinusoid(time_ids.to(self.device, torch.float32).contiguous(), a, cfg.addition_time_embed_dim, col_off=cfg.pooled_dim)
        h = torch.empty(R, cfg.time_embed_dim, dtype=F16, device=self.device)
        ops.gemm(a, w["add_embedding.linear_1.w"], h, bias=w["add_embedding.linear_1.b"], act=ops.ACT_SILU)
        out = torch.empty(R, cfg.time_embed_dim, dtype=F16, device=self.device)
        ops.gemm(h, w["add_embedding.linear_2.w"], out, bias=w["add_embedding.linear_2.b"])
        return out

    def _down_and_mid(self, x, R, H, W, temb_all, ada, st):
        cfg, o, w, A = self.cfg, self.o, self.w, self.arena
        skips = [(x, H, W)]
        nb = len(cfg.block_out_channels)
        for i, c in enumerate(cfg.block_out_channels):
            for j in range(cfg.layers_per_block):
                x = self._resnet(f"down_blocks.{i}.resnets.{j}", x, R, H, W, temb_all)
                if cfg.transformer_depth[i] > 0:
                    x = self._transformer(f"down_blocks.{i}.attentions.{j}", x, cfg.transformer_depth[i], R, H, W, st, ada)
                skips.append((x, H, W))
            if i < nb - 1:
                p = f"down_blocks.{i}.downsamplers.0.conv"
                H2, W2 = (H + 1) // 2, (W + 1) // 2
                y = A.alloc(R * H2 * W2, c)
                py = self._gn_alloc(R * H2 * W2, H2 * W2, c, 9 * c, True)
                o.conv2d(x.view(R, H, W, c), w[p + ".w"], y, stride=2, bias=w[p + ".b"], gn_out=py)
                if py is not None:
                    y._gn_parts = py
                x, H, W = y, H2, W2
                skips.append((x, H, W))
        x = self._resnet("mid_block.resnets.0", x, R, H, W, temb_all)
        x = self._transformer("mid_block.attentions.0", x, cfg.mid_depth, R, H, W, st, ada)
        x = self._resnet("mid_block.resnets.1", x, R, H, W, temb_all)
        return x, H, W, skips


class HipUNet(_Net):

    def __init__(self, cfg: UNetConfig, sd: Dict[str, torch.Tensor], device, lora=None, lora_scaling=1.0, fp8_linear=False):
        if lora is not None:
            sd = _merge_lora({k: v.to(device) for k, v in sd.items()}, {k: v.to(device) for k, v in lora.items()}, lora_scaling)
        super().__init__(cfg, sd, True, device, fp8_linear=fp8_linear)
# ... 93 lines not shown
        R, L = ctx.shape[0], ctx.shape[1]
        assert L == cfg.text_len and ip_tokens.shape[1] == cfg.num_ip_tokens
        ctx2 = ctx.to(dev, F16).reshape(R * L, -1).contiguous()
        ip2 = ip_tokens.to(dev, F16).reshape(R * cfg.num_ip_tokens, -1).contiguous()
        tpad = (L + 7) // 8 * 8
        nip, ipad = cfg.num_ip_tokens, (cfg.num_ip_tokens + 7) // 8 * 8
        st = {"R": R, "H": H, "W": W, "aug_emb": self._aug_emb(text_embeds, time_ids), "kv": {}}
        blocks = sorted({k[: -len(".attn2.to_k.w")] for k in w if k.endswith(".attn2.to_k.w")})
        for p in blocks:
            C = w[p + ".attn2.to_k.w"].shape[0]
            tk = torch.empty(R * L, C, dtype=F16, device=dev)
            ops.gemm(ctx2, w[p + ".attn2.to_k.w"], tk)
            tv = torch.empty(R * L, C, dtype=F16, device=dev)
            ops.gemm(ctx2, w[p + ".attn2.to_v.w"], tv)
            tvt = torch.zeros(C, R * tpad, dtype=F16, device=dev)
            for r in range(R):
                ops.transpose(tv[r * L:(r + 1) * L], tvt[:, r * tpad:(r + 1) * tpad], tpad)
            ipk = torch.empty(R * cfg.num_ip_tokens, C, dtype=F16, device=dev)
            ops.gemm(ip2, w[p + ".attn2.processor.to_k_ip.w"], ipk)
            ipv = torch.empty(R * cfg.num_ip_tokens, C, dtype=F16, device=dev)
            ops.gemm(ip2, w[p + ".attn2.processor.to_v_ip.w"], ipv)
            st["kv"][p] = {"tk": tk, "tvt": tvt, "tpad": tpad, "ipk_raw": ipk, "ipv_raw": ipv,
                           "ipk": torch.zeros(R * nip, C, dtype=F16, device=dev), "ipvt": torch.zeros(C, R * ipad, dtype=F16, device=dev)}
        st["ada"] = torch.zeros(R, w["ada_all.w"].shape[0], dtype=F16, device=dev)
        jobs = []
        for p in blocks:
            kv, C = st["kv"][p], w[p + ".attn2.to_k.w"].shape[0]
            sk, sv = self._ada_slices[p + ".k"], self._ada_slices[p + ".v"]
            ada = st["ada"]
            jobs.append((kv["ipk_raw"], kv["ipk"], ada[:, sk.start:sk.start + C], ada[:, sk.start + C:sk.stop], False))
            jobs.append((kv["ipv_raw"], kv["ipvt"], ada[:, sv.start:sv.start + C], ada[:, sv.start + C:sv.stop], True))
        st["ada_jobs"], st["ada_njobs"] = ops.adaln_job_table(jobs, dev), len(jobs)
        key = (R, H, W, self.freeu is not None)
        if self._sized != key:
            dummy = torch.empty(R * H * W, CPAD, dtype=F16, device="meta")
            self._size_arena(lambda: self._forward(dummy, None, st, None, None, None))
            self._sized = key
        return st

    def forward(self, sample, t_dev, st, down_res=None, mid_res=None, res_scale=None):
        self._begin()
        return self._forward(sample, t_dev, st, down_res, mid_res, res_scale)

    def encode(self, sample, t_dev, st):
        self._begin()
        return self._encode(sample, t_dev, st)

    def decode(self, enc, st, down_res=None, mid_res=None, res_scale=None, late_event=None):
        return self._decode(enc, st, down_res, mid_res, res_scale, late_event)

    def _forward(self, sample, t_dev, st, down_res, mid_res, res_scale):
        return self._decode(self._encode(sample, t_dev, st), st, down_res, mid_res, res_scale)

    def _encode(self, sample, t_dev, st):
        cfg, o, w, A = self.cfg, self.o, self.w, self.arena
        R, H, W = st["R"], st["H"], st["W"]
        temb_all, ada = self._embeddings(t_dev, st)
        x = A.alloc(R * H * W, cfg.block_out_channels[0])
        px = self._gn_alloc(R * H * W, H * W, cfg.block_out_channels[0], 9 * CPAD, True)
        o.conv2d(sample.view(R, H, W, CPAD), w["conv_in.w"], x, bias=w["conv_in.b"], gn_out=px)
        if px is not None:
            x._gn_parts = px
        x, h, wd, skips = self._down_and_mid(x, R, H, W, temb_all, ada, st)
        return x, h, wd, skips, temb_all, ada

    def _decode(self, enc, st, down_res, mid_res, res_scale, late_event=None, late_from_block=1):
        cfg, o, w, A = self.cfg, self.o, self.w, self.arena
        R = st["R"]
        x, h, wd, skips, temb_all, ada = enc
        skips = list(skips)
        rev = list(reversed(cfg.block_out_channels))
        depth = list(reversed(cfg.transformer_depth))
        nb = len(rev)
        pending_mid = mid_res
        for i, c in enumerate(rev):
            if late_event is not None and i == late_from_block:
                torch.cuda.current_stream().wait_event(late_event)
            for j in range(cfg.layers_per_block + 1):
                sk, sh, sw = skips.pop()
                k = len(skips)
                cx, cs = x.shape[1], sk.shape[1]
                cat = A.alloc(R * h * wd, cx + cs)
                add = down_res[k] if down_res is not None else None
                if self.freeu is not None and i < 2:
                    s_f, b_f = self.freeu[i], self.freeu[2 + i]
                    parts = A.alloc(R * ops.FREEU_SLABS * 7, 2 * cs).view(torch.float32)
                    o.freeu_stats(sk, parts, h, wd, add=add, add_scale=res_scale if add is not None else None)
                    o.freeu_concat(x, sk, cat, parts, h, wd, b_f, s_f, mid_add=pending_mid, add=add,
                                   add_scale=res_scale if (add is not None or pending_mid is not None) else None)
                    pending_mid = None
                else:
                    o.copy_add(x, cat, 0, add=pending_mid, add_scale=res_scale if pending_mid is not None else None,
                               rows_per_scale=h * wd)
                    pending_mid = None
                    o.copy_add(sk, cat, cx, add=add, add_scale=res_scale if down_res is not None else None,
                               rows_per_scale=h * wd)
                x = self._resnet(f"up_blocks.{i}.resnets.{j}", cat, R, h, wd, temb_all)
                if depth[i] > 0:
                    x = self._transformer(f"up_blocks.{i}.attentions.{j}", x, depth[i], R, h, wd, st, ada)
            if i < nb - 1:
                p = f"up_blocks.{i}.upsamplers.0.conv"
                y = A.alloc(R * 4 * h * wd, c)
                o.conv2d(x.view(R, h, wd, c), w[p + ".w"], y, upsample=True, bias=w[p + ".b"])
                x, h, wd = y, 2 * h, 2 * wd
        c0 = cfg.block_out_channels[0]
        g = A.alloc(R * h * wd, c0)
        o.groupnorm(x, g, R, h * wd, w["conv_norm_out.g"], w["conv_norm_out.b"], 1e-5, True, cfg.norm_groups, self._gnws,
                    partials=self._gn_of(x))
        eps = A.alloc(R * h * wd, cfg.out_channels)
        o.conv2d(g.view(R, h, wd, c0), w["conv_out.w"], eps, bias=w["conv_out.b"])
        return eps


class HipAggregator(_Net):

    def __init__(self, cfg: UNetConfig, sd: Dict[str, torch.Tensor], device):
        super().__init__(cfg, sd, False, device)
        self.defer_shallow = False
        self._late = []
        self._pack_conv3(sd, "ref_conv_in", CPAD)
        names = [f"controlnet_down_blocks.{k}" for k in range(len(skip_channels(cfg)))] + ["controlnet_mid_block"]
        for p in names:
            w0 = conv_weight_nhwc(self._t(sd, p + ".0.mlp_shared.0.weight"))
            self.w[p + ".shared.w"], self.w[p + ".shared.b"] = w0, self._t(sd, p + ".0.mlp_shared.0.bias").contiguous()
            wm, wa = conv_weight_nhwc(self._t(sd, p + ".0.mul.weight")), conv_weight_nhwc(self._t(sd, p + ".0.add.weight"))
            self.w[p + ".ga.w"] = pair_rows(wm, wa)
            self.w[p + ".ga.b"] = pair_rows(self._t(sd, p + ".0.mul.bias"), self._t(sd, p + ".0.add.bias"))
            w1 = self._t(sd, p + ".1.weight")
            self.w[p + ".zero.w"] = w1.reshape(w1.shape[0], w1.shape[1]).contiguous()
            self.w[p + ".zero.b"] = self._t(sd, p + ".1.bias").contiguous()
        self._finish_pack()
        self._sized = None
        self._out: Optional[List[torch.Tensor]] = None

    def prepare(self, text_embeds, time_ids, H, W, out_rows=None):
        R = text_embeds.shape[0]
        st = {"R": R, "H": H, "W": W, "aug_emb": self._aug_emb(text_embeds, time_ids), "kv": {}}
        Ro = R if out_rows is None else int(out_rows)
        assert Ro >= R
        key = (R, H, W) if Ro == R else (R, H, W, Ro)
        if self._sized != key:
            cfgc = skip_channels(self.cfg)
            hs, h, wd = [], H, W
            hs.append((h, wd))
            for i in range(len(self.cfg.block_out_channels)):
                hs += [(h, wd)] * self.cfg.layers_per_block
                if i < len(self.cfg.block_out_channels) - 1:
                    h, wd = (h + 1) // 2, (wd + 1) // 2
                    hs.append((h, wd))
            self._out = [torch.empty(Ro * a * b, c, dtype=F16, device=self.device) for (a, b), c in zip(hs, cfgc)]
            self._out_mid = torch.empty(Ro * h * wd, self.cfg.block_out_channels[-1], dtype=F16, device=self.device)
            dummy = torch.empty(R * H * W, CPAD, dtype=F16, device="meta")
            self._size_arena(lambda: self._forward(dummy, dummy, None, st))
            self._sized = key
        return st

    def forward(self, lq, preview, t_dev, st):
        self._begin()
        return self._forward(lq, preview, t_dev, st)

    def _sft(self, p, s, R, h2, wd, out):
        self._unit(p)
        o, w, A, cfg = self.o, self.w, self.arena, self.cfg
        C = s.shape[1]
        h = h2 // 2
        m = A.mark()
        s4 = s.view(R, h2, wd, C)
        actv = A.alloc(R * h * wd, cfg.sft_hidden)
        o.conv2d(s4[:, :h], w[p + ".shared.w"], actv, bias=w[p + ".shared.b"], act=ops.ACT_SILU)
        mod = A.alloc(R * h * wd, C)
        ref = s[h * wd:]
        o.conv2d(actv.view(R, h, wd, cfg.sft_hidden), w[p + ".ga.w"], mod, bias=w[p + ".ga.b"], res=ref, epi=ops.EPI_SFT,
                 res_img_rows=h2 * wd)
        o.gemm(mod, w[p + ".zero.w"], out[:R * h * wd], bias=w[p + ".zero.b"])
        A.release(m)

    def _forward(self, lq, preview, t_dev, st):
        cfg, o, w, A = self.cfg, self.o, self.w, self.arena
        R, H, W = st["R"], st["H"], st["W"]
        temb_all, ada = self._embeddings(t_dev, st)
        c0 = cfg.block_out_channels[0]
        x = A.alloc(R * 2 * H * W, c0)
        o.conv2d(lq.view(R, H, W, CPAD), w["conv_in.w"], x, bias=w["conv_in.b"], y_img_rows=2 * H * W)
        o.conv2d(preview.view(R, H, W, CPAD), w["ref_conv_in.w"], x[H * W:], bias=w["ref_conv_in.b"], y_img_rows=2 * H * W)
        xm, h2, wd, skips = self._down_and_mid(x, R, 2 * H, W, temb_all, ada, st)
        self._sft("controlnet_mid_block", xm, R, h2, wd, self._out_mid)
        n_deep = cfg.layers_per_block + 1
        self._late = []
        for k in reversed(range(len(skips))):
            s, sh, sw = skips[k]
            if self.defer_shallow and k < len(skips) - n_deep:
# ... 11 lines not shown
```

### instantir_amd/lib.py

```python
from __future__ import annotations

import ctypes as C
import os
import re

_HERE = os.path.dirname(os.path.abspath(__file__))
LIB_PATH = os.path.join(_HERE, "libinstantir_hip.so")
HEADER_PATH = os.path.join(os.path.dirname(_HERE), "include", "instantir_hip.h")

EPI_PLAIN, EPI_GEGLU, EPI_SFT, EPI_XATTN = 0, 1, 2, 3
ACT_NONE, ACT_SILU, ACT_GELU, ACT_QUICKGELU = 0, 1, 2, 3


class AttnKV(C.Structure):
    _fields_ = [
        ("K", C.c_void_p), ("ldk", C.c_int64), ("k_batch_stride", C.c_int64),
        ("Vt", C.c_void_p), ("ldvt", C.c_int64), ("vt_batch_stride", C.c_int64),
        ("Tkv", C.c_int32),
    ]


class GemmDesc(C.Structure):
    _fields_ = [
        ("A", C.c_void_p), ("lda", C.c_int64),
        ("W", C.c_void_p),
        ("C", C.c_void_p), ("ldc", C.c_int64),
        ("M", C.c_int32), ("N", C.c_int32), ("K", C.c_int32),
        ("bias", C.c_void_p),
        ("rowbias", C.c_void_p), ("ldrb", C.c_int64), ("rows_per_rb", C.c_int32),
        ("res", C.c_void_p), ("ldr", C.c_int64),
        ("epi", C.c_int32), ("act", C.c_int32),
        ("out_scale", C.c_float),
        ("tile", C.c_int32),
        ("prefetch", C.c_void_p), ("prefetch_bytes", C.c_int64),
        ("splitk_ws", C.c_void_p), ("splitk_ws_bytes", C.c_int64),
        ("Ct", C.c_void_p), ("ldct", C.c_int64), ("tr_from", C.c_int32),
        ("dtype", C.c_int32), ("c_f32", C.c_int32),
        ("wscale", C.c_void_p),
        ("ln_stats_out", C.c_void_p), ("ln_stats_in", C.c_void_p), ("ln_parts", C.c_int32), ("ln_part_cols", C.c_int32),
        ("ln_eps", C.c_float), ("ln_colsum", C.c_void_p),
        ("gn_stats_out", C.c_void_p),
        ("xattn_kv", C.POINTER(AttnKV)), ("xattn_tq", C.c_int32),
        ("a_fp8", C.c_int32), ("a_scale", C.c_float), ("c_fp8", C.c_int32),
    ]


class ConvDesc(C.Structure):
    _fields_ = [
        ("X", C.c_void_p), ("ldx", C.c_int64),
        ("R", C.c_int32), ("H", C.c_int32), ("Wd", C.c_int32), ("Cin", C.c_int32),
        ("Wt", C.c_void_p),
        ("Y", C.c_void_p), ("ldy", C.c_int64),
        ("Cout", C.c_int32), ("ksize", C.c_int32), ("stride", C.c_int32), ("upsample", C.c_int32),
        ("bias", C.c_void_p),
        ("rowbias", C.c_void_p), ("ldrb", C.c_int64), ("rows_per_rb", C.c_int32),
        ("res", C.c_void_p), ("ldr", C.c_int64),
        ("epi", C.c_int32), ("act", C.c_int32),
        ("out_scale", C.c_float),
        ("tile", C.c_int32),
        ("zero_page", C.c_void_p),
        ("x_img_stride", C.c_int64), ("y_img_rows", C.c_int32), ("res_img_rows", C.c_int32), ("pad_mode", C.c_int32),
        ("prefetch", C.c_void_p), ("prefetch_bytes", C.c_int64),
        ("splitk_ws", C.c_void_p), ("splitk_ws_bytes", C.c_int64),
        ("dtype", C.c_int32),
        ("gn_stats_out", C.c_void_p),
    ]


class AdaLNJob(C.Structure):
    _fields_ = [
        ("X", C.c_void_p), ("Y", C.c_void_p), ("shift", C.c_void_p), ("scale", C.c_void_p),
        ("ldx", C.c_int64), ("ldy", C.c_int64), ("C", C.c_int32), ("transposed", C.c_int32),
    ]


class AttnDesc(C.Structure):
    _fields_ = [
        ("Q", C.c_void_p), ("ldq", C.c_int64), ("q_batch_stride", C.c_int64),
        ("O", C.c_void_p), ("ldo", C.c_int64), ("o_batch_stride", C.c_int64),
        ("batch", C.c_int32), ("heads", C.c_int32), ("Tq", C.c_int32), ("nseg", C.c_int32),
        ("scale", C.c_float),
        ("kv", AttnKV * 2),
        ("causal", C.c_int32),
        ("q_prescaled", C.c_int32),
        ("o_fp8", C.c_int32),
    ]


_P, _I32, _I64, _F = C.c_void_p, C.c_int32, C.c_int64, C.c_float

SIGNATURES = {
    "iir_gemm_f16": (C.c_int, [C.POINTER(GemmDesc), _P]),
    "iir_gemm_splitk_workspace_bytes": (C.c_int64, [_I32, _I32]),
    "iir_gemm_uses_splitk": (C.c_int, [_I32, _I32, _I32, _I64]),
    "iir_gemm_pick_tile": (C.c_int, [_I32, _I32, _I32, _I32]),
    "iir_gemm_resolve_tile": (C.c_int, [_P]),
    "iir_gemm_gn_supported": (C.c_int, [_I32, _I32, _I32, _I32]),
    "iir_gemm_fp8_out_supported": (C.c_int, [_I32, _I32, _I32, _I32]),
    "iir_gemm_tile_bn": (C.c_int, [_I32]),
    "iir_gemm_ln_parts": (C.c_int, [_I32, _I32, _I32]),
    "iir_conv2d_nhwc_f16": (C.c_int, [C.POINTER(ConvDesc), _P]),
    "iir_attention_d64_f16": (C.c_int, [C.POINTER(AttnDesc), _P]),
    "iir_attention_d64_ident_f16": (C.c_int, [C.POINTER(AttnDesc), _I32, _P]),
    "iir_attention_f16": (C.c_int, [C.POINTER(AttnDesc), _I32, _P]),
    "iir_groupnorm_nhwc_f16": (C.c_int, [_P, _I64, _P, _I64, _I32, _I32, _I32, _I32, _P, _P, _F, _I32, _P, _I64, _P]),
    "iir_groupnorm_nhwc": (C.c_int, [_P, _I64, _P, _I64, _I32, _I32, _I32, _I32, _P, _P, _F, _I32, _P, _I64, _I32, _P]),
    "iir_groupnorm_from_partials": (C.c_int, [_P, _I64, _P, _I64, _P, _I64, _I32, _I32, _I32, _I32, _P, _P, _F, _I32, _P, _I64, _I32, _P]),
    "iir_groupnorm_workspace_bytes": (C.c_int64, [_I32, _I32]),
    "iir_layernorm_f16": (C.c_int, [_P, _I64, _P, _I64, _I32, _I32, _P, _P, _F, _P, _P, _I64, _I32, _I32, _I32, _I64, _P]),
    "iir_adaln_batch_f16": (C.c_int, [_P, _I32, _I32, _I32, _F, _I64, _I32, _I32, _I64, _P]),
    "iir_softmax_rows_f16": (C.c_int, [_P, _I64, _I32, _I32, _P]),
    "iir_softmax_rows_f32": (C.c_int, [_P, _I64, _P, _I64, _I32, _I32, _I32, _P]),
    "iir_sinusoid_f16": (C.c_int, [_P, _I32, _I32, _I32, _P, _I64, _I32, _P]),
    "iir_silu_f16": (C.c_int, [_P, _P, _I64, _P]),
    "iir_copy_add_f16": (C.c_int, [_P, _I64, _P, _I64, _I64, _I64, _I32, _P, _I64, _P, _I32, _P]),
    "iir_freeu_partials_bytes": (C.c_int64, [_I64, _I32, _I32, _I32]),
    "iir_freeu_stats_f16": (C.c_int, [_P, _I64, _P, _I64, _P, _I64, _I32, _I32, _I32, _P, _I64, _P]),
    "iir_freeu_concat_f16": (C.c_int, [_P, _I64, _I32, _P, _I64, _P, _I64, _I32, _P, _I64, _P, _I64, _I32, _I32, _F, _F, _P, _I64,
                                       _P, _I64, _I64, _P]),
    "iir_pack_latent": (C.c_int, [_P, _I32, _I32, _I32, _P, _I64, _I32, _F, _P]),
    "iir_unpack_latent": (C.c_int, [_P, _I64, _I32, _I32, _I32, _P, _P]),
    "iir_pack_latent_t": (C.c_int, [_P, _I32, _I32, _I32, _P, _I64, _I32, _F, _I32, _P]),
    "iir_unpack_latent_t": (C.c_int, [_P, _I64, _I32, _I32, _I32, _P, _I32, _P]),
    "iir_pack_latent_dscale": (C.c_int, [_P, _I32, _I32, _I32, _P, _I64, _I32, _P, _I32, _P]),
    "iir_sched_step": (C.c_int, [_P, _I64, _I32, _I32, _I32, _I32, _P, _P, _P, _P, _P, _P, _P, _P]),
    "iir_sched_step_hist": (C.c_int, [_P, _I64, _I32, _I32, _I32, _I32, _P, _P, _P, _P, _P, _P, _P, _P]),
    "iir_cfg_rescale_factor": (C.c_int, [_P, _I64, _I32, _I32, _I32, _P, _F, _P, _P]),
    "iir_sched_step_pag": (C.c_int, [_P, _I64, _I32, _I32, _I32, _I32, _P, _P, _P, _P, _P, _P, _P, _P, _P]),
    "iir_sched_step_hist_pag": (C.c_int, [_P, _I64, _I32, _I32, _I32, _I32, _P, _P, _P, _P, _P, _P, _P, _P, _P]),
    "iir_cfg_rescale_factor_pag": (C.c_int, [_P, _I64, _I32, _I32, _I32, _P, _P, _F, _P, _P]),
    "iir_copy_segments": (C.c_int, [_P, _I32, _I64, _P]),
    "iir_lcm_step": (C.c_int, [_P, _I64, _I32, _I32, _I32, _I32, _P, _P, _P, _I64, _P, _P]),
    "iir_sched_step_f32": (C.c_int, [_P, _P, _P, _P, _I64, _P, _P, _P]),
    "iir_axpby_f32": (C.c_int, [_P, _P, _P, _I64, _P, _P]),
    "iir_sched_step_hist_f32": (C.c_int, [_P, _P, _P, _P, _P, _I64, _P, _P, _P]),
    "iir_prefetch": (C.c_int, [_P, _I64, _I32, _P]),
    "iir_blend_tiles_f32": (C.c_int, [_P, _P, _I32, _I32, _I32, _I32, _I32, _I32, _I32, _P]),
    "iir_colorfix_workspace_bytes": (C.c_int64, [_I32, _I32, _I32, _I32]),
    "iir_colorfix_wavelet_f32": (C.c_int, [_P, _P, _P, _I32, _I32, _I32, _I32, _P, _I64, _P]),
    "iir_colorfix_adain_f32": (C.c_int, [_P, _P, _P, _I32, _I32, _I32, _I32, _P, _I64, _P]),
    "iir_transpose_f16": (C.c_int, [_P, _I64, _I32, _I32, _P, _I64, _I32, _P]),
    "iir_timing_event_create": (C.c_void_p, []),
    "iir_timing_event_destroy": (None, [_P]),
    "iir_timing_arm": (C.c_int, [_P, _P]),
    "iir_timing_elapsed_us": (C.c_int, [_P, _P, C.POINTER(C.c_float)]),
    "iir_abi_version": (C.c_int, []),
}

_lib = None


class HipLibraryError(RuntimeError):
    pass


def declared_symbols(header_path: str = HEADER_PATH):
    text = open(header_path).read()
    text = re.sub(r"/\*.*?\*/", "", text, flags=re.S)
    return sorted(set(re.findall(r"\b(iir_[a-z0-9_]+)\s*\(", text)))


def load():
    global _lib
    if _lib is not None:
        return _lib
    import torch
    if not os.path.exists(LIB_PATH):
        raise HipLibraryError(
            f"{LIB_PATH} not found: build it with instantir_amd/csrc/build.sh (hipcc --offload-arch=gfx950). "
            "There is no CPU fallback for the denoising path.")
    lib = C.CDLL(LIB_PATH)
    for name in declared_symbols():
        if name not in SIGNATURES:
            raise HipLibraryError(f"header declares {name} but lib.py has no signature for it")
        try:
            fn = getattr(lib, name)
        except AttributeError as e:
            raise HipLibraryError(f"{LIB_PATH} does not export {name}") from e
        fn.restype, fn.argtypes = SIGNATURES[name]
    if lib.iir_abi_version() != 1:
        raise HipLibraryError("ABI version mismatch")
    _lib = lib
    return lib


def check(rc: int, what: str):
    if rc != 0:
        raise HipLibraryError(f"{what} failed with code {rc} ({'invalid argument' if rc == -1 else 'launch failure'})")
```

### instantir_amd/ops.py

```python
from __future__ import annotations

import ctypes as C

import torch

from . import lib as L
from .lib import ACT_GELU, ACT_NONE, ACT_QUICKGELU, ACT_SILU, EPI_GEGLU, EPI_PLAIN, EPI_SFT, EPI_XATTN


def _stream():
    return torch.cuda.current_stream().cuda_stream


def _p(t):
    return None if t is None else t.data_ptr()


_DT = {torch.float16: 0, torch.bfloat16: 1}


def _chk2d(t, name, dtype=torch.float16):
    if t.dtype != dtype or t.dim() != 2 or t.stride(1) != 1 or not t.is_cuda:
        raise ValueError(f"{name}: expected a 2-D {dtype} CUDA tensor with unit column stride, got {t.dtype} {tuple(t.shape)} {t.stride()}")

# ... 100 lines not shown
        raise ValueError("gemm_fp8: w8 must be an Fp8Weight")
    if a8.dtype not in _FP8_DTYPES or a8.dim() != 2 or a8.stride(1) != 1 or not a8.is_cuda:
        raise ValueError("gemm_fp8: a8 must be a 2-D CUDA view of torch.float8_e4m3fn (or its bytes) with contiguous rows")
    M, K = a8.shape
    N = w8.q.shape[0]
    if w8.q.shape[1] != K or K % 128 or a8.stride(0) % 16:
        raise ValueError("gemm_fp8: K must match, K % 128 == 0, row stride % 16 == 0")
    dt = torch.float16
    c_fp8 = out.dtype in _FP8_DTYPES
    if c_fp8:
        if out.dim() != 2 or out.stride(1) != 1 or out.stride(0) % 8 or not out.is_cuda:
            raise ValueError("gemm_fp8: an fp8 `out` needs contiguous rows with a stride % 8 == 0")
    else:
        _chk2d(out, "out", dt)
    n_out = (N if epi == EPI_PLAIN else N // 2) if out_t is None else out_t[1]
    if out.shape != (M, n_out):
        raise ValueError(f"out shape {tuple(out.shape)} != {(M, n_out)}")
    for t_, n_ in ((bias, "bias"), (res, "res")):
        if t_ is not None and t_.dtype != dt:
            raise ValueError(f"{n_}: fp16 expected")
    d = L.GemmDesc()
    d.c_fp8 = int(c_fp8)
    if out_t is not None:
        ct, tr_from = out_t
        _chk2d(ct, "out_t", dt)
        if c_fp8 or ct.shape[0] < N - tr_from or ct.shape[1] < M:
            raise ValueError("out_t: fp16 (N - tr_from, M), with an fp16 `out`")
        d.Ct, d.ldct, d.tr_from = ct.data_ptr(), ct.stride(0), tr_from
    d.A, d.lda = a8.data_ptr(), a8.stride(0)
    d.W, d.wscale = w8.q.data_ptr(), w8.scale.data_ptr()
    d.C, d.ldc = out.data_ptr(), out.stride(0)
    d.M, d.N, d.K = M, N, K
    d.bias = _p(bias)
    if res is not None:
        _chk2d(res, "res", dt)
        d.res, d.ldr = res.data_ptr(), res.stride(0)
    d.epi, d.act, d.out_scale, d.tile = epi, act, 1.0, tile
    d.dtype, d.a_fp8, d.a_scale = _DT[dt], 1, float(a_scale)
    if prefetch is not None:
        d.prefetch, d.prefetch_bytes = prefetch
    t_name = tile if tile else auto_tile(M, N, epi != EPI_PLAIN, K)
    cls = "gemm_kernel<%s,gemm-f8>" % _TILE_NAMES[t_name % 10]
    if tile == 91 or (PROFILER is not None and tile == 0 and L.load().iir_gemm_resolve_tile(C.byref(d)) == 91):
        cls = "gemm8_kernel<256x320,gemm-f8>"
    with _Timed(cls, 2.0 * M * N * K, 1.0 * (M * K + N * K) + 2.0 * M * n_out * (2 if res is not None else 1)):
        L.check(L.load().iir_gemm_f16(C.byref(d), _stream()), "iir_gemm_f16")
    return out


def fp8_out_supported(M, N, K, paired=False):
    return bool(L.load().iir_gemm_fp8_out_supported(M, N, K, int(paired)))


def quantize_fp8_tensor(x):
    x32 = x.float()
    scale = float(x32.abs().amax().clamp_min(1e-12) / FP8_MAX)
    return (x32 / scale).clamp(-FP8_MAX, FP8_MAX).to(torch.float8_e4m3fn).contiguous(), scale


class LnFold:

    def __init__(self, weight, gamma, beta, bias=None, eps=1e-5, fp8=False, pair=None):
        w32 = weight.float() * gamma.float()[None, :]
        b32 = weight.float() @ beta.float() + (bias.float() if bias is not None else 0.0)
        if pair is not None:
            n = w32.shape[0] // 2
            w32, b32 = pair(w32[:n], w32[n:]), pair(b32[:n], b32[n:])
        w16 = w32.to(torch.float16).contiguous()
        if fp8:
            q, sc = quantize_fp8_rows(w16)
            self.w = Fp8Weight(q, sc)
            self.colsum = (q.float().sum(dim=1) * sc).contiguous()
        else:
            self.w = w16
            self.colsum = w16.float().sum(dim=1).contiguous()
        self.bias = b32.to(torch.float16).contiguous()
        self.eps = float(eps)


def ln_parts(M, N, K):
    return L.load().iir_gemm_ln_parts(M, N, K)


GN_PARTIALS_MAX = 20 * 256


def gn_supported(M, N, K, conv=False):
    return bool(L.load().iir_gemm_gn_supported(M, N, K, int(conv)))


def _chk_gn_out(gn_out, M, N):
    if gn_out.dtype != torch.float32 or not gn_out.is_contiguous() or M % 64 or tuple(gn_out.shape) != (M // 64, N, 2):
        raise ValueError(f"gn_out: contiguous fp32 ({M} // 64, {N}, 2) with M % 64 == 0, got {tuple(gn_out.shape)} {gn_out.dtype}")


def gemm(a, w, out, bias=None, rowbias=None, rows_per_rb=1, res=None, epi=EPI_PLAIN, act=ACT_NONE, out_scale=1.0,
         tile=0, prefetch=None, splitk_ws=None, out_t=None, wscale=None, ln_out=None, ln_in=None, gn_out=None, xattn=None):
    dt = a.dtype
    if isinstance(w, Fp8Weight):
        w, wscale = w.q, w.scale
    if wscale is not None:
        if w.dtype not in (torch.float8_e4m3fn, torch.uint8) or w.dim() != 2 or not w.is_contiguous() or not w.is_cuda:
            raise ValueError("fp8 weights: contiguous 2-D CUDA tensor of torch.float8_e4m3fn (or its bytes)")
        if wscale.dtype != torch.float32 or wscale.numel() != w.shape[0] or not wscale.is_contiguous():
            raise ValueError("wscale: contiguous fp32 (N,)")
        if dt != torch.float16:
            raise ValueError("fp8 weights take fp16 activations")
    if dt not in _DT:
        raise ValueError(f"a: fp16 or bf16 expected, got {dt}")
    c_f32 = out.dtype == torch.float32
    _chk2d(a, "a", dt); _chk2d(out, "out", torch.float32 if c_f32 else dt)
    if wscale is None:
        _chk2d(w, "w", dt)
    for t_, n_ in ((bias, "bias"), (rowbias, "rowbias"), (res, "res")):
        if t_ is not None and t_.dtype != dt:
            raise ValueError(f"{n_}: dtype {t_.dtype} does not match the operands ({dt})")
    M, K = a.shape
    N = w.shape[0]
    if w.shape[1] != K or not w.is_contiguous():
        raise ValueError("w must be contiguous (N,K) with K matching a")
    n_out = (N if epi in (EPI_PLAIN, EPI_XATTN) else N // 2) if out_t is None else out_t[1]
    if out.shape != (M, n_out):
        raise ValueError(f"out shape {tuple(out.shape)} != {(M, n_out)}")
    d = L.GemmDesc()
    d.A, d.lda = a.data_ptr(), a.stride(0)
    d.W = w.data_ptr()
    d.C, d.ldc = out.data_ptr(), out.stride(0)
    d.M, d.N, d.K = M, N, K
    d.bias = _p(bias)
    if rowbias is not None:
        _chk2d(rowbias, "rowbias", dt)
        d.rowbias, d.ldrb, d.rows_per_rb = rowbias.data_ptr(), rowbias.stride(0), rows_per_rb
    if res is not None:
        _chk2d(res, "res", dt)
        d.res, d.ldr = res.data_ptr(), res.stride(0)
    d.epi, d.act, d.out_scale, d.tile = epi, act, out_scale, tile
    d.dtype, d.c_f32 = _DT[dt], int(c_f32)
    if wscale is not None:
        d.wscale = wscale.data_ptr()
    if ln_out is not None:
        if ln_out.dtype != torch.float32 or not ln_out.is_contiguous() or ln_out.dim() != 3 or ln_out.shape[1:] != (M, 2) \
                or ln_out.shape[0] != ln_parts(M, N, K) or tile != 0:
            raise ValueError("ln_out: contiguous fp32 (ln_parts(M, N, K), M, 2), tile = 0")
        d.ln_stats_out = ln_out.data_ptr()
    if gn_out is not None:
        _chk_gn_out(gn_out, M, N)
        d.gn_stats_out = gn_out.data_ptr()
    if ln_in is not None:
        part, colsum, eps = ln_in
        if part.dtype != torch.float32 or not part.is_contiguous() or part.dim() != 3 or part.shape[1:] != (M, 2) or K % part.shape[0]:
            raise ValueError("ln_in partials: contiguous fp32 (parts, M, 2) with parts dividing K")
        if colsum.dtype != torch.float32 or colsum.numel() != N or not colsum.is_contiguous():
            raise ValueError("ln_in colsum: contiguous fp32 (N,)")
        d.ln_stats_in, d.ln_colsum, d.ln_parts, d.ln_part_cols, d.ln_eps = part.data_ptr(), colsum.data_ptr(), part.shape[0], K // part.shape[0], eps
    kv_keep = None
    if (epi == EPI_XATTN) != (xattn is not None):
        raise ValueError("epi = EPI_XATTN goes with xattn = (kv, Tq)")
    if xattn is not None:
        kvs, tq = xattn
        if len(kvs) != 2:
            raise ValueError("xattn: two K / V^T segments (text, IP tokens)")
        kv_keep = (L.AttnKV * 2)()
        for i, (k, k_rows, vt, vbs, tkv) in enumerate(kvs):
            _chk2d(k, "k"); _chk2d(vt, "vt")
            kv_keep[i].K, kv_keep[i].ldk, kv_keep[i].k_batch_stride = k.data_ptr(), k.stride(0), k_rows * k.stride(0)
            kv_keep[i].Vt, kv_keep[i].ldvt, kv_keep[i].vt_batch_stride = vt.data_ptr(), vt.stride(0), vbs
            kv_keep[i].Tkv = tkv
# ... 57 lines not shown
    Hi, Wi = (2 * H, 2 * Wd) if upsample else (H, Wd)
    pad2 = 1 if pad_mode == 1 else 2 * (ksize // 2)
    Mo = R * ((Hi + pad2 - ksize) // stride + 1) * ((Wi + pad2 - ksize) // stride + 1)
    d.epi, d.act, d.out_scale, d.tile = epi, act, out_scale, tile
    if gn_out is not None:
        _chk_gn_out(gn_out, Mo, Cout)
        d.gn_stats_out = gn_out.data_ptr()
    if tile == 0:
        Kc = ksize * ksize * Cin
        tile = 4 if splitk_ws is not None and L.load().iir_gemm_uses_splitk(Mo, Cout, Kc, splitk_ws.numel()) else auto_tile(Mo, Cout, epi != EPI_PLAIN, Kc)
    d.zero_page = zero_page(x.device).data_ptr()
    if prefetch is not None:
        d.prefetch, d.prefetch_bytes = prefetch
    if splitk_ws is not None:
        d.splitk_ws, d.splitk_ws_bytes = splitk_ws.data_ptr(), splitk_ws.numel()
    d.x_img_stride, d.y_img_rows, d.res_img_rows, d.pad_mode = x.stride(0), y_img_rows, res_img_rows, pad_mode
    Co = Cout // 2 if epi != EPI_PLAIN else Cout
    with _Timed("gemm_kernel<%s,conv>" % _TILE_NAMES[tile % 10], 2.0 * Mo * Cout * ksize * ksize * Cin,
                2.0 * (R * H * Wd * Cin + Cout * ksize * ksize * Cin + Mo * Co + (Mo * Co if res is not None else 0))):
        L.check(L.load().iir_conv2d_nhwc_f16(C.byref(d), _stream()), "iir_conv2d_nhwc_f16")
    return out


ATTN_LOG2E = 1.4426950408889634


def attn_q_factor(scale=0.125):
    import numpy as np
    return float(np.float32(scale) * np.float32(ATTN_LOG2E))


def attention(q, o, kv, batch, heads, Tq, scale=0.125, causal=False, q_prescaled=False, head_dim=64, ident_from=0):
    _chk2d(q, "q")
    d = L.AttnDesc()
    if o.dtype in _FP8_DTYPES:
        if o.dim() != 2 or o.stride(1) != 1 or o.stride(0) % 4 or not o.is_cuda:
            raise ValueError("attention: an fp8 `o` needs contiguous rows with a stride % 4 == 0")
        d.o_fp8 = 1
    else:
        _chk2d(o, "o")
    d.Q, d.ldq, d.q_batch_stride = q.data_ptr(), q.stride(0), Tq * q.stride(0)
    d.O, d.ldo, d.o_batch_stride = o.data_ptr(), o.stride(0), Tq * o.stride(0)
    d.batch, d.heads, d.Tq, d.nseg, d.scale = batch, heads, Tq, len(kv), scale
    d.causal = int(bool(causal))
    d.q_prescaled = int(bool(q_prescaled))
    for i, (k, k_rows, vt, vbs, tkv) in enumerate(kv):
        _chk2d(k, "k"); _chk2d(vt, "vt")
        d.kv[i].K, d.kv[i].ldk, d.kv[i].k_batch_stride = k.data_ptr(), k.stride(0), k_rows * k.stride(0)
        d.kv[i].Vt, d.kv[i].ldvt, d.kv[i].vt_batch_stride = vt.data_ptr(), vt.stride(0), vbs
        d.kv[i].Tkv = tkv
    if ident_from:
        if head_dim != 64:
            raise ValueError("attention: identity rows need head_dim 64")
        with _Timed("attn_kernel", 4.0 * ident_from * heads * Tq * head_dim * kv[0][4],
                    2.0 * ident_from * heads * head_dim * (2 * Tq + 2 * kv[0][4]) + 4.0 * (batch - ident_from) * heads * Tq * head_dim):
            L.check(L.load().iir_attention_d64_ident_f16(C.byref(d), int(ident_from), _stream()), "iir_attention_d64_ident_f16")
        return o
    with _Timed("attn_kernel", 4.0 * batch * heads * Tq * head_dim * sum(k[4] for k in kv),
                2.0 * batch * heads * head_dim * (2 * Tq + 2 * sum(k[4] for k in kv))):
        if head_dim == 64:
            L.check(L.load().iir_attention_d64_f16(C.byref(d), _stream()), "iir_attention_d64_f16")
        else:
            L.check(L.load().iir_attention_f16(C.byref(d), head_dim, _stream()), "iir_attention_f16")
    return o


_gn_ws = {}


def _gn_workspace(device, R, groups):
    need = L.load().iir_groupnorm_workspace_bytes(R, groups)
    key = (device, _stream())
    ws = _gn_ws.get(key)
    if ws is None or ws.numel() * 4 < need:
        ws = torch.empty(need // 4, dtype=torch.float32, device=device)
        _gn_ws[key] = ws
    return ws


def gn_workspace(device, R, groups=32):
    return torch.empty(L.load().iir_groupnorm_workspace_bytes(R, groups) // 4, dtype=torch.float32, device=device)


def groupnorm(x, out, R, HW, gamma, beta, eps, silu, groups=32, ws=None, partials=None):
    dt = x.dtype
    _chk2d(x, "x", dt if dt in _DT else torch.float16); _chk2d(out, "out", dt)
    if gamma.dtype != dt or beta.dtype != dt:
        raise ValueError(f"gamma / beta must have the activations' dtype ({dt})")
    Cc = x.shape[1]
    if ws is None:
        ws = _gn_workspace(x.device, R, groups)
    if partials is not None:
        _chk_gn_out(partials, R * HW, Cc)
        if HW % 64 or (HW // 64) * (Cc // groups) > GN_PARTIALS_MAX:
            raise ValueError(f"groupnorm(partials=): images of whole 64-row slabs and at most {GN_PARTIALS_MAX} partials per (image, group); "
                             f"got HW={HW}, {Cc // groups} channels per group")
        L.check(L.load().iir_groupnorm_from_partials(partials.data_ptr(), Cc, x.data_ptr(), x.stride(0), out.data_ptr(), out.stride(0),
                                                     R, HW, Cc, groups, gamma.data_ptr(), beta.data_ptr(), eps, int(silu), ws.data_ptr(),
                                                     ws.numel() * 4, _DT[dt], _stream()), "iir_groupnorm_from_partials")
        return out
    L.check(L.load().iir_groupnorm_nhwc(x.data_ptr(), x.stride(0), out.data_ptr(), out.stride(0), R, HW, Cc, groups,
                                        gamma.data_ptr(), beta.data_ptr(), eps, int(silu), ws.data_ptr(),
                                        ws.numel() * 4, _DT[dt], _stream()), "iir_groupnorm_nhwc")
    return out


def layernorm(x, out, gamma=None, beta=None, eps=1e-5, shift=None, scale=None, rows_per_mod=1, transposed=False,
              tr_rows=1, tr_bstride=0):
    _chk2d(x, "x")
    if out.dtype in (torch.float8_e4m3fn, torch.uint8):
        if transposed or out.dim() != 2 or out.stride(1) != 1 or out.stride(0) % 8 or not out.is_cuda or out.shape != x.shape:
            raise ValueError("layernorm: an fp8 `out` needs x's shape, contiguous rows with a stride % 8 == 0, no transposition")
        transposed = 2
    else:
        _chk2d(out, "out")
    rows, Cc = x.shape
    ldmod = shift.stride(0) if shift is not None else 0
    L.check(L.load().iir_layernorm_f16(x.data_ptr(), x.stride(0), out.data_ptr(), out.stride(0), rows, Cc, _p(gamma),
                                       _p(beta), eps, _p(shift), _p(scale), ldmod, rows_per_mod, int(transposed), tr_rows,
                                       tr_bstride, _stream()), "iir_layernorm_f16")
    return out


def adaln_job_table(jobs, device):
    arr = (L.AdaLNJob * len(jobs))()
    for i, (x, out, shift, scale, tr) in enumerate(jobs):
        _chk2d(x, "x"); _chk2d(out, "out")
        arr[i] = L.AdaLNJob(x.data_ptr(), out.data_ptr(), shift.data_ptr(), scale.data_ptr(), x.stride(0), out.stride(0),
                            x.shape[1], int(tr))
    raw = torch.frombuffer(bytearray(bytes(arr)), dtype=torch.uint8)
    return raw.to(device)


def adaln_batch(table, njobs, rows, max_C, ldmod, rows_per_mod, tr_rows, tr_bstride, eps=1e-6):
    L.check(L.load().iir_adaln_batch_f16(table.data_ptr(), njobs, rows, max_C, eps, ldmod, rows_per_mod, tr_rows, tr_bstride,
                                         _stream()), "iir_adaln_batch_f16")


def sinusoid(vals, out, dim, col_off=0):
    rows, n_vals = vals.shape
    L.check(L.load().iir_sinusoid_f16(vals.data_ptr(), n_vals, rows, dim, out.data_ptr(), out.stride(0), col_off,
                                      _stream()), "iir_sinusoid_f16")
    return out


def silu(x, out):
    L.check(L.load().iir_silu_f16(x.data_ptr(), out.data_ptr(), x.numel(), _stream()), "iir_silu_f16")
    return out


def copy_add(src, dst, dst_off=0, add=None, add_scale=None, rows_per_scale=1):
    _chk2d(src, "src"); _chk2d(dst, "dst")
    M, Cc = src.shape
    L.check(L.load().iir_copy_add_f16(src.data_ptr(), src.stride(0), dst.data_ptr(), dst.stride(0), dst_off, M, Cc,
                                      _p(add), add.stride(0) if add is not None else 0, _p(add_scale), rows_per_scale,
                                      _stream()), "iir_copy_add_f16")
    return dst


FREEU_SLABS = 16


def freeu_partials_floats(rows, H, W, C):
    n = L.load().iir_freeu_partials_bytes(rows, H, W, C)
    if n < 0:
        raise ValueError(f"freeu: invalid geometry rows={rows} H={H} W={W} C={C}")
    return n // 4


def freeu_stats(skip, partials, H, W, add=None, add_scale=None):
    _chk2d(skip, "skip")
    M, Cc = skip.shape
    L.check(L.load().iir_freeu_stats_f16(skip.data_ptr(), skip.stride(0), _p(add), add.stride(0) if add is not None else 0,
                                         _p(add_scale), M, H, W, Cc, partials.data_ptr(), partials.numel() * 4, _stream()),
            "iir_freeu_stats_f16")
    return partials


def freeu_concat(x, skip, dst, partials, H, W, b, s, dst_off=0, mid_add=None, add=None, add_scale=None):
    _chk2d(x, "x"); _chk2d(skip, "skip"); _chk2d(dst, "dst")
    M, cx = x.shape
    cs = skip.shape[1]
    if skip.shape[0] != M or dst.shape[0] != M:
        raise ValueError("freeu_concat: x, skip and dst must have the same rows")
    L.check(L.load().iir_freeu_concat_f16(x.data_ptr(), x.stride(0), cx, _p(mid_add), mid_add.stride(0) if mid_add is not None else 0,
                                          skip.data_ptr(), skip.stride(0), cs, _p(add), add.stride(0) if add is not None else 0,
                                          _p(add_scale), M, H, W, float(b), float(s), partials.data_ptr(), partials.numel() * 4,
                                          dst.data_ptr(), dst.stride(0), dst_off, _stream()), "iir_freeu_concat_f16")
    return dst


def pack_latent(x, out, rep=1, scale=1.0):
    B, Cc, H, Wd = x.shape
    assert x.dtype == torch.float32 and x.is_contiguous() and out.dtype in _DT
    L.check(L.load().iir_pack_latent_t(x.data_ptr(), B, Cc, H * Wd, out.data_ptr(), out.stride(0), rep, scale, _DT[out.dtype],
                                       _stream()), "iir_pack_latent_t")
    return out


def pack_latent_dscale(x, out, scale, rep=1):
    B, Cc, H, Wd = x.shape
    assert x.dtype == torch.float32 and x.is_contiguous() and out.dtype in _DT
    assert scale.dtype == torch.float32 and scale.is_cuda and scale.numel() >= 1
    L.check(L.load().iir_pack_latent_dscale(x.data_ptr(), B, Cc, H * Wd, out.data_ptr(), out.stride(0), rep, scale.data_ptr(),
                                            _DT[out.dtype], _stream()), "iir_pack_latent_dscale")
    return out


def unpack_latent(x2d, out):
    R, Cc, H, Wd = out.shape
    assert out.dtype == torch.float32 and out.is_contiguous() and x2d.dtype in _DT
    L.check(L.load().iir_unpack_latent_t(x2d.data_ptr(), x2d.stride(0), R, Cc, H * Wd, out.data_ptr(), _DT[x2d.dtype], _stream()),
            "iir_unpack_latent_t")
    return out


def _chk_pag(pag_scale):
    if not (torch.is_tensor(pag_scale) and pag_scale.is_cuda and pag_scale.dtype == torch.float32 and pag_scale.numel() >= 1):
        raise ValueError("pag_scale must be a CUDA fp32 tensor (the step's s_t, read at launch time)")


def sched_step(eps2d, B, coef, x, prev, noise=None, cfg=True, x0_out=None, eps_out=None, eps_factor=None, pag_scale=None):
    _, Cc, H, Wd = x.shape
    if pag_scale is not None:
        _chk_pag(pag_scale)
        L.check(L.load().iir_sched_step_pag(eps2d.data_ptr(), eps2d.stride(0), B, Cc, H * Wd, int(cfg), coef.data_ptr(),
                                            pag_scale.data_ptr(), x.data_ptr(), _p(noise), prev.data_ptr(), _p(x0_out), _p(eps_out),
                                            _p(eps_factor), _stream()), "iir_sched_step_pag")
        return prev
    L.check(L.load().iir_sched_step(eps2d.data_ptr(), eps2d.stride(0), B, Cc, H * Wd, int(cfg), coef.data_ptr(),
                                    x.data_ptr(), _p(noise), prev.data_ptr(), _p(x0_out), _p(eps_out), _p(eps_factor),
                                    _stream()), "iir_sched_step")
    return prev


def sched_step_hist(eps2d, B, coef, x, hist, prev, noise=None, cfg=True, x0_out=None, eps_factor=None, pag_scale=None):
    _, Cc, H, Wd = x.shape
    assert hist.shape == x.shape and hist.dtype == torch.float32 and hist.is_contiguous()
    if pag_scale is not None:
        _chk_pag(pag_scale)
        L.check(L.load().iir_sched_step_hist_pag(eps2d.data_ptr(), eps2d.stride(0), B, Cc, H * Wd, int(cfg), coef.data_ptr(),
                                                 pag_scale.data_ptr(), x.data_ptr(), _p(noise), hist.data_ptr(), prev.data_ptr(),
                                                 _p(x0_out), _p(eps_factor), _stream()), "iir_sched_step_hist_pag")
        return prev
    L.check(L.load().iir_sched_step_hist(eps2d.data_ptr(), eps2d.stride(0), B, Cc, H * Wd, int(cfg), coef.data_ptr(),
                                         x.data_ptr(), _p(noise), hist.data_ptr(), prev.data_ptr(), _p(x0_out), _p(eps_factor),
                                         _stream()), "iir_sched_step_hist")
    return prev


def cfg_rescale_factor(eps2d, B, coef, x, guidance_rescale, factor, pag_scale=None):
    _, Cc, H, Wd = x.shape
    if pag_scale is not None:
        _chk_pag(pag_scale)
        L.check(L.load().iir_cfg_rescale_factor_pag(eps2d.data_ptr(), eps2d.stride(0), B, Cc, H * Wd, coef.data_ptr(),
                                                    pag_scale.data_ptr(), float(guidance_rescale), factor.data_ptr(), _stream()),
                "iir_cfg_rescale_factor_pag")
        return factor
    L.check(L.load().iir_cfg_rescale_factor(eps2d.data_ptr(), eps2d.stride(0), B, Cc, H * Wd, coef.data_ptr(),
                                            float(guidance_rescale), factor.data_ptr(), _stream()), "iir_cfg_rescale_factor")
    return factor


def segment_job_table(jobs, device):
    rows = []
    for src, dst in jobs:
        nb = src.numel() * src.element_size()
        if (not src.is_contiguous() or not dst.is_contiguous() or dst.numel() * dst.element_size() != nb or nb % 16
                or src.data_ptr() % 16 or dst.data_ptr() % 16):
            raise ValueError("copy_segments: each job needs contiguous, 16-byte aligned tensors of the same size (a multiple of 16 B)")
        rows.append([src.data_ptr(), dst.data_ptr(), nb // 16])
# ... 97 lines not shown
```

### instantir_amd/pipeline.py

```python
from __future__ import annotations

import os
from types import SimpleNamespace
from typing import Callable, Dict, List, Optional, Union

import torch

from . import ops, pag
from .config import UNetConfig, VAEConfig
from .engine import CPAD, F16, HipAggregator, HipUNet
from .schedulers import (DDIMScheduler, DDPMScheduler, DPMSolverMultistepScheduler, EulerAncestralDiscreteScheduler,
                         EulerDiscreteScheduler, LCMSingleStepScheduler)
from .weights import LCM_LORA_MODULES, PREVIEWER_LORA_MODULES, lora_target

COLOR_FIX_MODES = (None,) + ops.COLOR_FIX_MODES

class StableDiffusionXLPipelineOutput(SimpleNamespace):
    """`.images` like diffusers' output class (pipelines/sdxl_instantir.py:1739)."""


class _AggregatorHandle:

    def __init__(self, pipe):
        self._pipe = pipe
# ... 222 lines not shown
    def set_pag_applied_layers(self, pag_applied_layers: Union[str, List[str]]):
        layers = pag.normalize_layers(pag_applied_layers)
        self._pag_paths = tuple(pag.select(layers, pag.attn1_paths(self.cfg)))
        self._pag_layers = layers

    def disable_pag(self):
        self._pag_layers = self._pag_paths = None

    @property
    def pag_applied_layers(self):
        return None if self._pag_layers is None else list(self._pag_layers)

    def _main_state(self, ctx, pooled, time_ids, img, Hl, Wl, B, rep, pag_on):
        ip = self._unet.resampler(img)
        if pag_on:
            c = slice((rep - 1) * B, rep * B)
            ctx, pooled, time_ids, ip = (torch.cat([v, v[c]], 0) for v in (ctx, pooled, time_ids, ip))
        return self._unet.prepare(ctx, pooled, time_ids, ip, Hl, Wl)

    def _apply_freeu(self, *nets):
        for n in nets:
            if n is not None:
                n.freeu = self._freeu

    @property
    def do_classifier_free_guidance(self):
        return self._guidance_scale > 1

    def prepare_previewers(self, lora_state_dict: Dict[str, torch.Tensor], use_lcm=False, lora_alpha=None):
        targets = LCM_LORA_MODULES if use_lcm else PREVIEWER_LORA_MODULES
        if isinstance(lora_state_dict, (str, os.PathLike)):
            from .loaders import read_previewer_lora
            lora_state_dict, file_alpha = read_previewer_lora(os.fspath(lora_state_dict))
            lora_alpha = file_alpha if lora_alpha is None else lora_alpha
        ranks = {v.shape[0] for k, v in lora_state_dict.items() if k.endswith(".lora_A.weight")}
        if len(ranks) == 1 and next(iter(ranks)) != self.cfg.lora_rank:
            import dataclasses
            self.cfg = dataclasses.replace(self.cfg, lora_rank=next(iter(ranks)))
        unexpected = []
        for k in lora_state_dict:
            for suf in (".lora_A.weight", ".lora_B.weight"):
                if k.endswith(suf):
                    path = k[: -len(suf)]
                    if not lora_target(path, targets) or (path + ".weight") not in self._unet_sd:
                        unexpected.append(k)
                    break
            else:
                unexpected.append(k)
        if unexpected:
            raise ValueError("Loading adapter weights from state_dict led to unexpected keys not found in the model: "
                             f" {unexpected}. ")
        lora_alpha = 1 if lora_alpha is None else lora_alpha
        name = "lcm" if use_lcm else "previewer"
        self._adapters[name] = (dict(lora_state_dict), lora_alpha / self.cfg.lora_rank)
        for k in [k for k in self._prev_nets if k[0] == name]:
            del self._prev_nets[k]
        self._unet_prev8 = None
        self.unet.set_adapter(name)
        return lora_alpha

    def _build(self, lora_mult: float = 1.0):
        if self._unet is None:
            self._unet = HipUNet(self.cfg, self._unet_sd, self.device)
        if self._active_adapter is not None:
            key = (self._active_adapter, float(lora_mult))
            if key not in self._prev_nets and float(lora_mult) != 1.0:
                for k_old in [k for k in self._prev_nets if k[0] == self._active_adapter and k[1] != 1.0 and len(k) == 2]:
                    del self._prev_nets[k_old]
            if key not in self._prev_nets:
                if self._lora is None:
                    raise RuntimeError(f"LoRA adapter {self._active_adapter!r}: the host copy was released; call prepare_previewers again")
                self._prev_nets[key] = HipUNet(self.cfg, self._unet_sd, self.device, lora=self._lora,
                                               lora_scaling=self._lora_scaling * float(lora_mult))
            self._unet_prev = self._prev_nets[key]
        if self._agg is None:
            if self._agg_sd is None:
                self._agg_sd = self.aggregator.from_unet()
            self._agg = HipAggregator(self.cfg, self._agg_sd, self.device)
        self._apply_freeu(self._unet, self._unet_prev)

    def _loop_for(self, B, rep, Hl, Wl, st, st_prev, st_agg, lq, reference_latents, previewer_scheduler, guidance_rescale, pag_on=False):
        nets = (self._unet, self._unet_prev, self._agg)
        key = (B, rep, Hl, Wl, reference_latents is not None, float(guidance_rescale or 0.0), self.use_graphs, self.overlap_streams,
               self.overlap_sft, tuple(None if n is None else (id(n), n.arena_gen, n.inkernel_prefetch, n.gn_fuse) for n in nets),
               self._freeu,
               _sched_form(self.scheduler),
               self._pag_paths if pag_on else None)
        cached = self._loop_cache
        if cached is not None and cached[0] == key and os.environ.get("IIR_LOOP_CACHE", "1") != "0":
            if cached[1].adopt(st, st_prev, st_agg, lq, reference_latents, previewer_scheduler):
                return cached[1]
        self._loop_cache = None
        loop = _DenoiseLoop(self, B, rep, Hl, Wl, st, st_prev, st_agg, lq, reference_latents, previewer_scheduler,
                            guidance_rescale=guidance_rescale, pag_on=pag_on)
        self._loop_cache = (key, loop, nets)
        return loop

    def check_inputs(self, prompt, prompt_embeds, negative_prompt_embeds, pooled_prompt_embeds, negative_pooled_prompt_embeds,
                     ip_adapter_image, ip_adapter_image_embeds, control_guidance_start, control_guidance_end,
                     callback_on_step_end_tensor_inputs):
        if callback_on_step_end_tensor_inputs is not None and not all(
                k in ("latents", "prompt_embeds", "negative_prompt_embeds") for k in callback_on_step_end_tensor_inputs):
            raise ValueError(f"`callback_on_step_end_tensor_inputs` has to be in ['latents', 'prompt_embeds', "
                             f"'negative_prompt_embeds'], but found {callback_on_step_end_tensor_inputs}")
        if prompt is not None and prompt_embeds is not None:
            raise ValueError(f"Cannot forward both `prompt`: {prompt} and `prompt_embeds`: {prompt_embeds}. Please make sure to"
                             " only forward one of the two.")
        if prompt is None and prompt_embeds is None:
            raise ValueError("Provide either `prompt` or `prompt_embeds`. Cannot leave both `prompt` and `prompt_embeds` undefined.")
        if prompt is not None and (self.text_encoder is None or self.text_encoder_2 is None or self.tokenizer is None):
            raise NotImplementedError("`prompt` strings need text encoders + tokenizers attached to the pipeline "
                                      "(tokenizer vocabularies are not available offline): pass `prompt_embeds` / "
                                      "`pooled_prompt_embeds`, or `prompt_ids` / `prompt_ids_2`")
        if prompt_embeds is not None and negative_prompt_embeds is not None and prompt_embeds.shape != negative_prompt_embeds.shape:
            raise ValueError("`prompt_embeds` and `negative_prompt_embeds` must have the same shape when passed directly, but"
                             f" got: `prompt_embeds` {prompt_embeds.shape} != `negative_prompt_embeds` {negative_prompt_embeds.shape}.")
        if prompt is None and prompt_embeds is not None and pooled_prompt_embeds is None:
            raise ValueError("If `prompt_embeds` are provided, `pooled_prompt_embeds` also have to be passed. Make sure to "
                             "generate `pooled_prompt_embeds` from the same text encoder that was used to generate `prompt_embeds`.")
        if negative_prompt_embeds is not None and negative_pooled_prompt_embeds is None:
            raise ValueError("If `negative_prompt_embeds` are provided, `negative_pooled_prompt_embeds` also have to be passed.")
        for s, e in [(control_guidance_start, control_guidance_end)]:
            if s >= e:
                raise ValueError(f"control guidance start: {s} cannot be larger or equal to control guidance end: {e}.")
            if s < 0.0:
                raise ValueError(f"control guidance start: {s} can't be smaller than 0.")
            if e > 1.0:
                raise ValueError(f"control guidance end: {e} can't be larger than 1.0.")
        if ip_adapter_image is not None and ip_adapter_image_embeds is not None:
            raise ValueError("Provide either `ip_adapter_image` or `ip_adapter_image_embeds`. Cannot leave both "
                             "`ip_adapter_image` and `ip_adapter_image_embeds` defined.")
        if ip_adapter_image_embeds is not None:
            if not isinstance(ip_adapter_image_embeds, list):
                raise ValueError(f"`ip_adapter_image_embeds` has to be of type `list` but is {type(ip_adapter_image_embeds)}")
            if ip_adapter_image_embeds[0].ndim not in [3, 4]:
                raise ValueError("`ip_adapter_image_embeds` has to be a list of 3D or 4D tensors but is "
                                 f"{ip_adapter_image_embeds[0].ndim}D")

    def encode_prompt(self, prompt=None, prompt_2=None, negative_prompt=None, negative_prompt_2=None, prompt_ids=None,
                      prompt_ids_2=None, negative_prompt_ids=None, negative_prompt_ids_2=None, do_cfg=True, clip_skip=None):
        from .encoders import encode_prompt_ids

        def ids_of(texts, tok):
            texts = [texts] if isinstance(texts, str) else list(texts)
            return tok(texts)

        if prompt_ids is None:
            prompt_ids = ids_of(prompt, self.tokenizer)
            prompt_ids_2 = ids_of(prompt_2 if prompt_2 is not None else prompt, self.tokenizer_2 or self.tokenizer)
        if prompt_ids_2 is None:
            prompt_ids_2 = prompt_ids
        def encode(ids, ids2, skip):
            key = (ids.cpu().numpy().tobytes(), ids2.cpu().numpy().tobytes(), tuple(ids.shape), skip, id(self.text_encoder), id(self.text_encoder_2))
            hit = self._prompt_cache.get(key)
            if hit is None or hit[2] is not self.text_encoder or hit[3] is not self.text_encoder_2:
                hit = (*encode_prompt_ids(self.text_encoder, self.text_encoder_2, ids, ids2, skip), self.text_encoder, self.text_encoder_2)
                if len(self._prompt_cache) >= 8:
                    self._prompt_cache.pop(next(iter(self._prompt_cache)))
                self._prompt_cache[key] = hit
            return hit[0], hit[1]

        pe, pooled = encode(prompt_ids, prompt_ids_2, clip_skip)
        npe = npooled = None
        if do_cfg:
            if negative_prompt_ids is None and negative_prompt is not None:
                negative_prompt_ids = ids_of(negative_prompt, self.tokenizer)
                negative_prompt_ids_2 = ids_of(negative_prompt_2 if negative_prompt_2 is not None else negative_prompt,
# ... 604 lines not shown
```

Baseline: 17.68.

## Fuse groupnorm partial stats into skip-concat and merge GN finalize with apply

The up-block concat kernels (plain and FreeU) now stage each output tile in shared memory and emit per-64-row slab mean/M2 partials for the following resnet's groupnorm. This removes a separate statistics pass over the concatenated tensor. A new single-launch groupnorm kernel merges the column partials and applies the normalisation in one kernel, replacing the finalize-then-apply pair. In exchange the concat kernels use more shared memory and add a barrier, and each apply block redundantly re-merges the partials for its groups.

```diff
diff --git a/include/instantir_hip.h b/include/instantir_hip.h
--- a/include/instantir_hip.h
+++ b/include/instantir_hip.h
@@ -117,6 +117,8 @@
 int iir_groupnorm_nhwc_f16(const void* X, int64_t ldx, void* Y, int64_t ldy, int32_t R, int32_t HW, int32_t C,
                            int32_t groups, const void* gamma, const void* beta, float eps, int32_t silu,
                            void* workspace, int64_t workspace_bytes, void* stream);
+#define IIR_GN_SILU 1
+#define IIR_GN_TWO_LAUNCH 2
 int iir_groupnorm_from_partials(const void* partials, int64_t ldp, const void* X, int64_t ldx, void* Y, int64_t ldy, int32_t R,
                                 int32_t HW, int32_t C, int32_t groups, const void* gamma, const void* beta, float eps, int32_t silu,
                                 void* workspace, int64_t workspace_bytes, int32_t dtype, void* stream);
@@ -124,6 +126,7 @@
                        int32_t groups, const void* gamma, const void* beta, float eps, int32_t silu,
                        void* workspace, int64_t workspace_bytes, int32_t dtype, void* stream);
 int64_t iir_groupnorm_workspace_bytes(int32_t R, int32_t groups);
+int iir_groupnorm_one_launch(int32_t R, int32_t HW, int32_t C, int32_t groups);
 
 int iir_layernorm_f16(const void* X, int64_t ldx, void* Y, int64_t ldy, int32_t rows, int32_t C, const void* gamma,
                       const void* beta, float eps, const void* shift, const void* scale, int64_t ldmod,
@@ -155,6 +158,13 @@
                          int32_t cs, const void* add, int64_t lda, const float* add_scale, int64_t rows, int32_t H, int32_t W,
                          float b, float s, const float* partials, int64_t partials_bytes, void* cat, int64_t ldc,
                          int64_t cat_off, void* stream);
+int iir_concat_gn_f16(const void* x, int64_t ldx, int32_t cx, const void* mid_add, int64_t ldm, const void* skip, int64_t lds,
+                      int32_t cs, const void* add, int64_t lda, const float* add_scale, int64_t M, int32_t rows_per_scale,
+                      void* cat, int64_t ldc, void* gn_out, void* stream);
+int iir_freeu_concat_gn_f16(const void* x, int64_t ldx, int32_t cx, const void* mid_add, int64_t ldm, const void* skip, int64_t lds,
+                            int32_t cs, const void* add, int64_t lda, const float* add_scale, int64_t rows, int32_t H, int32_t W,
+                            float b, float s, const float* partials, int64_t partials_bytes, void* cat, int64_t ldc,
+                            int64_t cat_off, void* gn_out, void* stream);
 
 int iir_pack_latent(const float* x, int32_t B, int32_t C, int32_t HW, void* out, int64_t ldo, int32_t rep, float scale,
                     void* stream);
diff --git a/instantir_amd/csrc/freeu.hip b/instantir_amd/csrc/freeu.hip
--- a/instantir_amd/csrc/freeu.hip
+++ b/instantir_amd/csrc/freeu.hip
@@ -1,4 +1,5 @@
 #include "common.h"
+#include "gn_slab.h"
 #include "../../include/instantir_hip.h"
 
 namespace {
@@ -8,6 +9,7 @@
 constexpr int CB = 64;
 constexpr int RL = 32;
 constexpr int CONCAT_ROWS = 256;
+constexpr int TILE_LD = CB + 8;
 
 __device__ __forceinline__ void phase_sc(int n, int N, float* s, float* c) {
     int m = 2 * n;
@@ -85,8 +87,16 @@
 __global__ __launch_bounds__(256) void freeu_concat_kernel(const f16* x, long ldx, int cx, const f16* mid, long ldm, const f16* sk,
                                                             long lds_, int cs, const f16* add, long lda, const float* add_scale,
                                                             int H, int W, float b, float s, const float* part, f16* cat,
-                                                            long ldc, long cat_off) {
+                                                            long ldc, long cat_off, float2* gn ) {
     __shared__ float coef[NSUM][CB];
+    __shared__ f16 tile[CONCAT_ROWS * TILE_LD];
+    auto emit_gn = [&](int r_, int p0_, int cb0, int width, int off) {
+        __syncthreads();
+        const int sl = threadIdx.x >> 6, c = threadIdx.x & 63;
+        if (p0_ + sl * GN_SLAB_ROWS < H * W && cb0 + c < width)
+            gn[(((long)r_ * H * W + p0_) / GN_SLAB_ROWS + sl) * (long)(cx + cs) + off + cb0 + c] =
+                gn_slab_partial(tile + sl * GN_SLAB_ROWS * TILE_LD + c, TILE_LD);
+    };
     const int tid = threadIdx.x, oct = tid & 7, rl = tid >> 3;
     const int HW = H * W;
     const int ntile = (HW + CONCAT_ROWS - 1) / CONCAT_ROWS;
@@ -115,7 +125,9 @@
 #pragma unroll
             for (int j = 0; j < 8; ++j) o[j] = (f16)(cl + j < half ? t[j] * b : t[j]);
             if (p < HW && c0 < cx) *(f16x8*)(cat + m * ldc + cat_off + c0) = o;
-        }
+            if (gn) *(f16x8*)(tile + (i * RL + rl) * TILE_LD + oct * 8) = o;
+        }
+        if (gn) emit_gn(r, p0, blockIdx.y * CB, cx, 0);
         return;
     }
     const int cb = blockIdx.y - nbx;
@@ -166,7 +178,9 @@
 #pragma unroll
         for (int j = 0; j < 8; ++j) o[j] = (f16)t[j];
         if (p < HW && c0 < cs) *(f16x8*)(cat + m * ldc + cat_off + cx + c0) = o;
-    }
+        if (gn) *(f16x8*)(tile + (i * RL + rl) * TILE_LD + oct * 8) = o;
+    }
+    if (gn) emit_gn(r, p0, cb * CB, cs, cx);
 }
 
 long planes(int64_t rows, int32_t H, int32_t W) {
@@ -198,11 +212,12 @@
     return iir_launch_status();
 }
 
-extern "C" int iir_freeu_concat_f16(const void* x, int64_t ldx, int32_t cx, const void* mid_add, int64_t ldm, const void* skip,
-                                    int64_t lds, int32_t cs, const void* add, int64_t lda, const float* add_scale, int64_t rows,
-                                    int32_t H, int32_t W, float b, float s, const float* partials, int64_t partials_bytes,
-                                    void* cat, int64_t ldc, int64_t cat_off, void* stream) {
+extern "C" int iir_freeu_concat_gn_f16(const void* x, int64_t ldx, int32_t cx, const void* mid_add, int64_t ldm, const void* skip,
+                                       int64_t lds, int32_t cs, const void* add, int64_t lda, const float* add_scale, int64_t rows,
+                                       int32_t H, int32_t W, float b, float s, const float* partials, int64_t partials_bytes,
+                                       void* cat, int64_t ldc, int64_t cat_off, void* gn_out, void* stream) {
     (void)hipGetLastError();
+    if (gn_out && ((uintptr_t)gn_out % 8 || ((int64_t)H * W) % GN_SLAB_ROWS)) return IIR_EINVAL;
     const long R = planes(rows, H, W);
     if (!x || !skip || !cat || !partials || R < 0) return IIR_EINVAL;
     if (cx <= 0 || cx % 8 || cs <= 0 || cs % 8 || ldx % 8 || ldx < cx || lds % 8 || lds < cs) return IIR_EINVAL;
@@ -214,6 +229,14 @@
     const int ntile = (int)((HW + CONCAT_ROWS - 1) / CONCAT_ROWS);
     hipLaunchKernelGGL(freeu_concat_kernel, dim3((unsigned)(R * ntile), (cx + CB - 1) / CB + (cs + CB - 1) / CB), dim3(256), 0,
                        (hipStream_t)stream, (const f16*)x, (long)ldx, cx, (const f16*)mid_add, (long)ldm, (const f16*)skip, (long)lds,
-                       cs, (const f16*)add, (long)lda, add_scale, H, W, b, s, partials, (f16*)cat, (long)ldc, (long)cat_off);
+                       cs, (const f16*)add, (long)lda, add_scale, H, W, b, s, partials, (f16*)cat, (long)ldc, (long)cat_off, (float2*)gn_out);
     return iir_launch_status();
 }
+
+extern "C" int iir_freeu_concat_f16(const void* x, int64_t ldx, int32_t cx, const void* mid_add, int64_t ldm, const void* skip,
+                                    int64_t lds, int32_t cs, const void* add, int64_t lda, const float* add_scale, int64_t rows,
+                                    int32_t H, int32_t W, float b, float s, const float* partials, int64_t partials_bytes,
+                                    void* cat, int64_t ldc, int64_t cat_off, void* stream) {
+    return iir_freeu_concat_gn_f16(x, ldx, cx, mid_add, ldm, skip, lds, cs, add, lda, add_scale, rows, H, W, b, s, partials, partials_bytes,
+                                   cat, ldc, cat_off, nullptr, stream);
+}
diff --git a/instantir_amd/csrc/gn_slab.h b/instantir_amd/csrc/gn_slab.h
--- /dev/null
+++ b/instantir_amd/csrc/gn_slab.h
@@ -0,0 +1,18 @@
+#pragma once
+#include "common.h"
+
+constexpr int GN_SLAB_ROWS = 64;
+
+__device__ __forceinline__ float2 gn_slab_partial(const f16* col , int ld) {
+    float s = 0.f;
+#pragma unroll 16
+    for (int i = 0; i < GN_SLAB_ROWS; ++i) s += (float)col[i * ld];
+    const float mean = s * (1.0f / GN_SLAB_ROWS);
+    float q = 0.f;
+#pragma unroll 16
+    for (int i = 0; i < GN_SLAB_ROWS; ++i) {
+        const float d = (float)col[i * ld] - mean;
+        q = __builtin_fmaf(d, d, q);
+    }
+    return make_float2(mean, q);
+}
diff --git a/instantir_amd/csrc/norm.hip b/instantir_amd/csrc/norm.hip
--- a/instantir_amd/csrc/norm.hip
+++ b/instantir_amd/csrc/norm.hip
@@ -4,6 +4,9 @@
 namespace {
 
 constexpr int GN_MAXC = 2560;
+constexpr int GN_ONE_WGS = 256;
+constexpr int GN_ONE_WIDE = 160;
+constexpr int GN_ONE_MAXP = 5;
 constexpr int GN_MIN_PIX = 8;
 
 __device__ __forceinline__ void chan_merge(float& n, float& mean, float& m2, float nb, float mb, float m2b) {
@@ -135,47 +138,78 @@
     }
 }
 
+template <int MAXP, int NG>
+__device__ __forceinline__ void gn_merge_cols(const float2* base, long ldp, int n, int cpg, float eps, float* red ,
+                                              float (&mean)[NG], float (&rstd)[NG]) {
+    float2 a[NG][MAXP];
+#pragma unroll
+    for (int g = 0; g < NG; ++g)
+#pragma unroll
+        for (int k = 0; k < MAXP; ++k) {
+            const int i = min((int)threadIdx.x + k * 256, n - 1);
+            const int sl = i / cpg, c = i - sl * cpg;
+            a[g][k] = base[(long)sl * ldp + g * cpg + c];
+        }
+    auto block_sum = [&](float (&v)[NG]) {
+#pragma unroll
+        for (int g = 0; g < NG; ++g) red[g * 256 + threadIdx.x] = v[g];
+        __syncthreads();
+#pragma unroll
+        for (int o = 128; o > 0; o >>= 1) {
+            if ((int)threadIdx.x < o) {
+#pragma unroll
+                for (int g = 0; g < NG; ++g) red[g * 256 + threadIdx.x] += red[g * 256 + threadIdx.x + o];
+            }
+            __syncthreads();
+        }
+#pragma unroll
+        for (int g = 0; g < NG; ++g) v[g] = red[g * 256];
+        __syncthreads();
+    };
+    float sm[NG];
+#pragma unroll
+    for (int g = 0; g < NG; ++g) {
+        sm[g] = 0.f;
+#pragma unroll
+        for (int k = 0; k < MAXP; ++k) sm[g] += ((int)threadIdx.x + k * 256 < n) ? a[g][k].x : 0.f;
+    }
+    block_sum(sm);
+    float q[NG];
+#pragma unroll
+    for (int g = 0; g < NG; ++g) {
+        mean[g] = sm[g] / (float)n;
+        q[g] = 0.f;
+#pragma unroll
+        for (int k = 0; k < MAXP; ++k) {
+            const float d = a[g][k].x - mean[g];
+            q[g] += ((int)threadIdx.x + k * 256 < n) ? fmaf(64.0f * d, d, a[g][k].y) : 0.f;
+        }
+    }
+    block_sum(q);
+#pragma unroll
+    for (int g = 0; g < NG; ++g) rstd[g] = rsqrtf(q[g] / ((float)n * 64.0f) + eps);
+}
+
+constexpr int GN_COLS_MAXP = 20;
+constexpr int GN_COLS_MAXP_WIDE = 30;
+
+template <int MAXP>
 __global__ __launch_bounds__(256) void gn_finalize_cols_kernel(const float2* part, long ldp, int slabs_per_img, int G, int cpg, float eps,
                                                                float* stat ) {
     __shared__ float red[256];
     const int r = blockIdx.x / G, gi = blockIdx.x - r * G;
     const int n = slabs_per_img * cpg;
-    constexpr int MAXP = 20;
-    float2 a[MAXP];
-    const float2* base = part + (long)r * slabs_per_img * ldp + gi * cpg;
-#pragma unroll
-    for (int k = 0; k < MAXP; ++k) {
-        const int i = min((int)threadIdx.x + k * 256, n - 1);
-        const int sl = i / cpg, c = i - sl * cpg;
-        a[k] = base[(long)sl * ldp + c];
-    }
-    auto block_sum = [&](float v) {
-        red[threadIdx.x] = v;
-        __syncthreads();
-#pragma unroll
-        for (int o = 128; o > 0; o >>= 1) {
-            if ((int)threadIdx.x < o) red[threadIdx.x] += red[threadIdx.x + o];
-            __syncthreads();
-        }
-        const float t = red[0];
-        __syncthreads();
-        return t;
-    };
-    float sm = 0.f;
-#pragma unroll
-    for (int k = 0; k < MAXP; ++k) sm += ((int)threadIdx.x + k * 256 < n) ? a[k].x : 0.f;
-    const float mean = block_sum(sm) / (float)n;
-    float q = 0.f;
-#pragma unroll
-    for (int k = 0; k < MAXP; ++k) {
-        const float d = a[k].x - mean;
-        q += ((int)threadIdx.x + k * 256 < n) ? fmaf(64.0f * d, d, a[k].y) : 0.f;
-    }
-    const float m2 = block_sum(q);
+    float mean[1], rstd[1];
+    gn_merge_cols<MAXP, 1>(part + (long)r * slabs_per_img * ldp + gi * cpg, ldp, n, cpg, eps, red, mean, rstd);
     if (threadIdx.x == 0) {
-        stat[((long)r * G + gi) * 2] = mean;
-        stat[((long)r * G + gi) * 2 + 1] = rsqrtf(m2 / ((float)n * 64.0f) + eps);
-    }
+        stat[((long)r * G + gi) * 2] = mean[0];
+        stat[((long)r * G + gi) * 2 + 1] = rstd[0];
+    }
+}
+
+__device__ __forceinline__ void gn_coef(float mean, float rstd, float gm, float bt, float& a, float& b) {
+    a = rstd * gm;
+    b = bt - mean * a;
 }
 
 template <typename E>
@@ -202,9 +236,7 @@
 #pragma unroll
         for (int j = 0; j < 8; ++j) {
             const int gi = (ch * 8 + j) / cpg;
-            const float mean = st[gi * 2], rstd = st[gi * 2 + 1];
-            a[j] = rstd * (float)gm[j];
-            b[j] = (float)bt[j] - mean * a[j];
+            gn_coef(st[gi * 2], st[gi * 2 + 1], (float)gm[j], (float)bt[j], a[j], b[j]);
         }
         for (int p = p0 + tp; p < p1; p += prows) {
             const E8 v = *(const E8*)(xb + (long)p * ldx + ch * 8);
@@ -218,6 +250,60 @@
             *(E8*)(yb + (long)p * ldy + ch * 8) = o;
         }
     }
+}
+
+template <typename E, int MAXP, int NG>
+__global__ __launch_bounds__(256) void gn_one_kernel(const float2* part, long ldp, int slabs_per_img, const f16* Xp, long ldx, f16* Yp,
+                                                     long ldy, int HW, int G, int cpg, int pix_per_blk, float eps, const f16* gammap,
+                                                     const f16* betap, int silu) {
+    using E8 = typename ET<E>::x8;
+    __shared__ float red[NG * 256];
+    __shared__ float smean[NG], srstd[NG];
+    const E* X = (const E*)Xp; E* Y = (E*)Yp; const E* gamma = (const E*)gammap; const E* beta = (const E*)betap;
+    const int r = blockIdx.z, g0 = blockIdx.y * NG, c0 = g0 * cpg;
+    {
+        float mean[NG], rstd[NG];
+        gn_merge_cols<MAXP, NG>(part + (long)r * slabs_per_img * ldp + c0, ldp, slabs_per_img * cpg, cpg, eps, red, mean, rstd);
+        if (threadIdx.x == 0) {
+#pragma unroll
+            for (int g = 0; g < NG; ++g) { smean[g] = mean[g]; srstd[g] = rstd[g]; }
+        }
+        __syncthreads();
+    }
+    const int lanes_c = NG * cpg >> 3;
+    const int prows = 256 / lanes_c;
+    const int tc = threadIdx.x % lanes_c, tp = threadIdx.x / lanes_c;
+    if (tp >= prows) return;
+    const int p0 = blockIdx.x * pix_per_blk;
+    const int p1 = min(HW, p0 + pix_per_blk);
+    const E* xb = X + (long)r * HW * ldx + c0 + tc * 8;
+    E* yb = Y + (long)r * HW * ldy;
+    float a[8], b[8];
+    const E8 gm = *(const E8*)(gamma + c0 + tc * 8), bt = *(const E8*)(beta + c0 + tc * 8);
+#pragma unroll
+    for (int j = 0; j < 8; ++j) {
+        const int gl = (tc * 8 + j) / cpg;
+        gn_coef(smean[gl], srstd[gl], (float)gm[j], (float)bt[j], a[j], b[j]);
+    }
+    auto put = [&](int p, const E8& v) {
+        E8 o;
+#pragma unroll
+        for (int j = 0; j < 8; ++j) {
+            float f = fmaf((float)v[j], a[j], b[j]);
+            if (silu) f = silu_f(f);
+            o[j] = (E)f;
+        }
+        *(E8*)(yb + (long)p * ldy + c0 + tc * 8) = o;
+    };
+    int p = p0 + tp;
+    for (; p + 3 * prows < p1; p += 4 * prows) {
+        E8 v[4];
+#pragma unroll
+        for (int u = 0; u < 4; ++u) v[u] = *(const E8*)(xb + (long)(p + u * prows) * ldx);
+#pragma unroll
+        for (int u = 0; u < 4; ++u) put(p + u * prows, v[u]);
+    }
+    for (; p < p1; p += prows) put(p, *(const E8*)(xb + (long)p * ldx));
 }
 
 __device__ __forceinline__ void ln_row(const f16* X, long ldx, f16* Y, long ldy, int row, int C, const f16* gamma,
@@ -394,6 +480,44 @@
             *(E4*)(y + ch * 4) = o;
         }
     }
+}
+
+template <typename E, int MAXP, int NG>
+void gn_one_go(dim3 grid, hipStream_t st, const void* partials, long ldp, int slabs, const void* X, long ldx, void* Y, long ldy, int HW,
+               int G, int cpg, int ppb, float eps, const void* gamma, const void* beta, int silu) {
+    hipLaunchKernelGGL((gn_one_kernel<E, MAXP, NG>), grid, dim3(256), 0, st, (const float2*)partials, ldp, slabs, (const f16*)X, ldx, (f16*)Y,
+                       ldy, HW, G, cpg, ppb, eps, (const f16*)gamma, (const f16*)beta, silu);
+}
+
+struct GnOnePlan { bool ok; int ng, nspan, npr, ppb; };
+GnOnePlan gn_one_plan(int R, int HW, int C, int groups) {
+    const GnOnePlan no = {false, 0, 0, 0, 0};
+    const int cpg = C / groups, slabs = HW / 64;
+    int ng = 1;
+    while (ng <= 4 && (ng * cpg) % 8) ng *= 2;
+    if (ng > 4 || groups % ng) return no;
+    while (ng * cpg < GN_ONE_WIDE && ng * 2 <= 4 && groups % (ng * 2) == 0) ng *= 2;
+    const int span = ng * cpg, n = slabs * cpg;
+    if (span / 8 > 256 || R > 65535 || n > GN_ONE_MAXP * 256) return no;
+    const int nspan = C / span, prows = 256 / (span / 8);
+    int npr = GN_ONE_WGS / (R * nspan); if (npr < 1) npr = 1;
+    int ppb = (HW + npr - 1) / npr; if (ppb < 2 * prows) ppb = 2 * prows;
+    npr = (HW + ppb - 1) / ppb;
+    return {true, ng, nspan, npr, ppb};
+}
+
+bool gn_one_launch(const void* partials, long ldp, const void* X, long ldx, void* Y, long ldy, int R, int HW, int C, int groups,
+                   const void* gamma, const void* beta, float eps, int silu, int dtype, hipStream_t st) {
+    const GnOnePlan pl = gn_one_plan(R, HW, C, groups);
+    if (!pl.ok) return false;
+    const int cpg = C / groups, slabs = HW / 64, ppb = pl.ppb;
+    const dim3 grid(pl.npr, pl.nspan, R);
+#define GN_ONE_CASE(E, N) gn_one_go<E, GN_ONE_MAXP, N>(grid, st, partials, ldp, slabs, X, ldx, Y, ldy, HW, groups, cpg, ppb, eps, gamma, beta, silu)
+#define GN_ONE_NG(E) (pl.ng == 1 ? GN_ONE_CASE(E, 1) : pl.ng == 2 ? GN_ONE_CASE(E, 2) : GN_ONE_CASE(E, 4))
+    if (dtype == IIR_DT_BF16) GN_ONE_NG(bf16); else GN_ONE_NG(f16);
+#undef GN_ONE_NG
+#undef GN_ONE_CASE
+    return true;
 }
 
 }
@@ -434,6 +558,7 @@
     float* part = (float*)workspace;
     float* stat = part + part_floats;
     const hipStream_t st = (hipStream_t)stream;
+    const int silu_on = silu & IIR_GN_SILU;
     int nblk = (1024 + R - 1) / R;
     int ppb = (HW + nblk - 1) / nblk; if (ppb < GN_MIN_PIX) ppb = GN_MIN_PIX;
     nblk = (HW + ppb - 1) / ppb;
@@ -441,8 +566,8 @@
     else hipLaunchKernelGGL(gn_stats_kernel<f16>, dim3(nslab, R), dim3(256), 0, st, (const f16*)X, (long)ldx, HW, C, groups, pps, part);
     const int gblocks = (groups + 7) / 8;
     hipLaunchKernelGGL(gn_finalize_kernel, dim3(R * gblocks), dim3(256), 0, st, (const float*)part, nslab, groups, HW, pps, C / groups, eps, stat, gblocks);
-    if (dtype == IIR_DT_BF16) hipLaunchKernelGGL(gn_apply_kernel<bf16>, dim3(nblk, R), dim3(256), 0, st, (const f16*)X, (long)ldx, (f16*)Y, (long)ldy, HW, C, groups, ppb, (const float*)stat, (const f16*)gamma, (const f16*)beta, silu);
-    else hipLaunchKernelGGL(gn_apply_kernel<f16>, dim3(nblk, R), dim3(256), 0, st, (const f16*)X, (long)ldx, (f16*)Y, (long)ldy, HW, C, groups, ppb, (const float*)stat, (const f16*)gamma, (const f16*)beta, silu);
+    if (dtype == IIR_DT_BF16) hipLaunchKernelGGL(gn_apply_kernel<bf16>, dim3(nblk, R), dim3(256), 0, st, (const f16*)X, (long)ldx, (f16*)Y, (long)ldy, HW, C, groups, ppb, (const float*)stat, (const f16*)gamma, (const f16*)beta, silu_on);
+    else hipLaunchKernelGGL(gn_apply_kernel<f16>, dim3(nblk, R), dim3(256), 0, st, (const f16*)X, (long)ldx, (f16*)Y, (long)ldy, HW, C, groups, ppb, (const float*)stat, (const f16*)gamma, (const f16*)beta, silu_on);
     return iir_launch_status();
 }
 
@@ -454,17 +579,28 @@
     if (C % 8 || C > GN_MAXC || groups <= 0 || groups > 64 || C % groups || ldx % 8 || ldy % 8 || ldp < C) return IIR_EINVAL;
     if (R <= 0 || HW <= 0 || HW % 64 || (dtype != IIR_DT_F16 && dtype != IIR_DT_BF16)) return IIR_EINVAL;
     const int slabs = HW / 64, cpg = C / groups;
-    if ((long)slabs * cpg > 20 * 256) return IIR_EINVAL;
+    if ((long)slabs * cpg > GN_COLS_MAXP_WIDE * 256) return IIR_EINVAL;
     if ((int64_t)R * groups * 2 * 4 > workspace_bytes) return IIR_EINVAL;
     float* stat = (float*)workspace;
     const hipStream_t st = (hipStream_t)stream;
-    hipLaunchKernelGGL(gn_finalize_cols_kernel, dim3(R * groups), dim3(256), 0, st, (const float2*)partials, (long)ldp, slabs, groups, cpg, eps, stat);
+    const int silu_on = silu & IIR_GN_SILU;
+    if (!(silu & IIR_GN_TWO_LAUNCH) && gn_one_launch(partials, ldp, X, ldx, Y, ldy, R, HW, C, groups, gamma, beta, eps, silu_on, dtype, st))
+        return iir_launch_status();
+    if ((long)slabs * cpg > GN_COLS_MAXP * 256)
+        hipLaunchKernelGGL(gn_finalize_cols_kernel<GN_COLS_MAXP_WIDE>, dim3(R * groups), dim3(256), 0, st, (const float2*)partials, (long)ldp, slabs, groups, cpg, eps, stat);
+    else
+        hipLaunchKernelGGL(gn_finalize_cols_kernel<GN_COLS_MAXP>, dim3(R * groups), dim3(256), 0, st, (const float2*)partials, (long)ldp, slabs, groups, cpg, eps, stat);
     int nblk = (1024 + R - 1) / R;
     int ppb = (HW + nblk - 1) / nblk; if (ppb < GN_MIN_PIX) ppb = GN_MIN_PIX;
     nblk = (HW + ppb - 1) / ppb;
-    if (dtype == IIR_DT_BF16) hipLaunchKernelGGL(gn_apply_kernel<bf16>, dim3(nblk, R), dim3(256), 0, st, (const f16*)X, (long)ldx, (f16*)Y, (long)ldy, HW, C, groups, ppb, (const float*)stat, (const f16*)gamma, (const f16*)beta, silu);
-    else hipLaunchKernelGGL(gn_apply_kernel<f16>, dim3(nblk, R), dim3(256), 0, st, (const f16*)X, (long)ldx, (f16*)Y, (long)ldy, HW, C, groups, ppb, (const float*)stat, (const f16*)gamma, (const f16*)beta, silu);
+    if (dtype == IIR_DT_BF16) hipLaunchKernelGGL(gn_apply_kernel<bf16>, dim3(nblk, R), dim3(256), 0, st, (const f16*)X, (long)ldx, (f16*)Y, (long)ldy, HW, C, groups, ppb, (const float*)stat, (const f16*)gamma, (const f16*)beta, silu_on);
+    else hipLaunchKernelGGL(gn_apply_kernel<f16>, dim3(nblk, R), dim3(256), 0, st, (const f16*)X, (long)ldx, (f16*)Y, (long)ldy, HW, C, groups, ppb, (const float*)stat, (const f16*)gamma, (const f16*)beta, silu_on);
     return iir_launch_status();
+}
+
+extern "C" int iir_groupnorm_one_launch(int32_t R, int32_t HW, int32_t C, int32_t groups) {
+    if (R <= 0 || HW <= 0 || HW % 64 || C <= 0 || C % 8 || C > GN_MAXC || groups <= 0 || groups > 64 || C % groups) return 0;
+    return gn_one_plan(R, HW, C, groups).ok ? 1 : 0;
 }
 
 extern "C" int iir_groupnorm_nhwc_f16(const void* X, int64_t ldx, void* Y, int64_t ldy, int32_t R, int32_t HW, int32_t C,
diff --git a/instantir_amd/csrc/pointwise.hip b/instantir_amd/csrc/pointwise.hip
--- a/instantir_amd/csrc/pointwise.hip
+++ b/instantir_amd/csrc/pointwise.hip
@@ -1,4 +1,5 @@
 #include "common.h"
+#include "gn_slab.h"
 #include "../../include/instantir_hip.h"
 
 namespace {
@@ -43,6 +44,39 @@
         for (int j = 0; j < 8; ++j) v[j] = (f16)((float)v[j] + (float)a[j] * s);
     }
     *(f16x8*)(dst + m * ldd + dst_off + ch * 8) = v;
+}
+
+constexpr int CG_ROWS = 256, CG_CB = 64, CG_LD = CG_CB + 8;
+__global__ __launch_bounds__(256) void concat_gn_kernel(const f16* x, long ldx, int cx, const f16* mid, long ldm, const f16* sk, long lds_,
+                                                        int cs, const f16* add, long lda, const float* add_scale, long M,
+                                                        int rows_per_scale, f16* cat, long ldc, float2* gn ) {
+    __shared__ f16 tile[CG_ROWS * CG_LD];
+    const int tid = threadIdx.x, oct = tid & 7, rl = tid >> 3;
+    const int nbx = (cx + CG_CB - 1) / CG_CB;
+    const bool hid = (int)blockIdx.y < nbx;
+    const f16* src = hid ? x : sk; const f16* ad = hid ? mid : add;
+    const long lsrc = hid ? ldx : lds_, lad = hid ? ldm : lda;
+    const int width = hid ? cx : cs, off = hid ? 0 : cx;
+    const int cb0 = (hid ? blockIdx.y : blockIdx.y - nbx) * CG_CB;
+    const int c0 = cb0 + oct * 8, cl = min(c0, width - 8);
+    const long m0 = (long)blockIdx.x * CG_ROWS;
+#pragma unroll 4
+    for (int i = 0; i < CG_ROWS / 32; ++i) {
+        const long row = m0 + i * 32 + rl, m = row < M ? row : M - 1;
+        f16x8 v = *(const f16x8*)(src + m * lsrc + cl);
+        if (ad) {
+            const f16x8 a = *(const f16x8*)(ad + m * lad + cl);
+            const float s = add_scale ? add_scale[m / rows_per_scale] : 1.0f;
+#pragma unroll
+            for (int j = 0; j < 8; ++j) v[j] = (f16)((float)v[j] + (float)a[j] * s);
+        }
+        if (row < M && c0 < width) *(f16x8*)(cat + m * ldc + off + c0) = v;
+        *(f16x8*)(tile + (i * 32 + rl) * CG_LD + oct * 8) = v;
+    }
+    __syncthreads();
+    const int sl = tid >> 6, c = tid & 63;
+    if (m0 + sl * GN_SLAB_ROWS < M && cb0 + c < width)
+        gn[((m0 >> 6) + sl) * (long)(cx + cs) + off + cb0 + c] = gn_slab_partial(tile + sl * GN_SLAB_ROWS * CG_LD + c, CG_LD);
 }
 
 template <typename E>
@@ -247,6 +281,23 @@
     return iir_launch_status();
 }
 
+extern "C" int iir_concat_gn_f16(const void* x, int64_t ldx, int32_t cx, const void* mid_add, int64_t ldm, const void* skip, int64_t lds,
+                                 int32_t cs, const void* add, int64_t lda, const float* add_scale, int64_t M, int32_t rows_per_scale,
+                                 void* cat, int64_t ldc, void* gn_out, void* stream) {
+    (void)hipGetLastError();
+    if (!x || !skip || !cat || !gn_out || (uintptr_t)gn_out % 8 || M <= 0 || M % GN_SLAB_ROWS || M > (1L << 31)) return IIR_EINVAL;
+    if (cx <= 0 || cx % 8 || cs <= 0 || cs % 8 || ldx % 8 || ldx < cx || lds % 8 || lds < cs) return IIR_EINVAL;
+    if (mid_add && (ldm % 8 || ldm < cx)) return IIR_EINVAL;
+    if (add && (lda % 8 || lda < cs)) return IIR_EINVAL;
+    if (ldc % 8 || ldc < cx + cs) return IIR_EINVAL;
+    if (add_scale && rows_per_scale <= 0) return IIR_EINVAL;
+    const dim3 grid((unsigned)((M + CG_ROWS - 1) / CG_ROWS), (cx + CG_CB - 1) / CG_CB + (cs + CG_CB - 1) / CG_CB);
+    hipLaunchKernelGGL(concat_gn_kernel, grid, dim3(256), 0, (hipStream_t)stream, (const f16*)x, (long)ldx, cx, (const f16*)mid_add,
+                       (long)ldm, (const f16*)skip, (long)lds, cs, (const f16*)add, (long)lda, add_scale, (long)M, rows_per_scale,
+                       (f16*)cat, (long)ldc, (float2*)gn_out);
+    return iir_launch_status();
+}
+
 extern "C" int iir_pack_latent_t(const float* x, int32_t B, int32_t C, int32_t HW, void* out, int64_t ldo, int32_t rep,
                                  float scale, int32_t dtype, void* stream) {
     (void)hipGetLastError();
diff --git a/instantir_amd/engine.py b/instantir_amd/engine.py
--- a/instantir_amd/engine.py
+++ b/instantir_amd/engine.py
@@ -113,6 +113,8 @@
         self.fuse_qkv = os.environ.get("IIR_FUSE_QKV", "1") != "0"
         self.ln_fold = os.environ.get("IIR_LN_FOLD", "1") != "0" and not fp8_linear
         self.gn_fuse = os.environ.get("IIR_GN_FUSE", "1") != "0"
+        self.gn_one = os.environ.get("IIR_GN_ONE", "1") != "0"
+        self.cat_fuse = os.environ.get("IIR_CAT_FUSE", "1") != "0" and not fp8_linear
         self.xattn_fuse = os.environ.get("IIR_XATTN_FUSE", "1") != "0"
         self.pag = None
         self.fp8_act = fp8_linear and os.environ.get("IIR_FP8_ACT", "1") != "0"
@@ -325,14 +327,14 @@
         m = A.mark()
         h = A.alloc(R * HW, cin)
         o.groupnorm(x, h, R, HW, w[path + ".norm1.g"], w[path + ".norm1.b"], eps, True, self.cfg.norm_groups, self._gnws,
-                    partials=self._gn_of(x))
+                    partials=self._gn_of(x), one_launch=self.gn_one)
         h2 = A.alloc(R * HW, cout)
         p2 = self._gn_alloc(R * HW, HW, cout, 9 * cin, True) if self._skws is None else None
         o.conv2d(h.view(R, H, W, cin), w[path + ".conv1.w"], h2, bias=w[path + ".conv1.b"],
                  rowbias=temb_all[:, self._temb_slices[path]], rows_per_rb=HW, prefetch=self._pf(w[path + ".conv1.w"]),
                  splitk_ws=self._skws, gn_out=p2)
         h3 = A.alloc(R * HW, cout)
-        o.groupnorm(h2, h3, R, HW, w[path + ".norm2.g"], w[path + ".norm2.b"], eps, True, self.cfg.norm_groups, self._gnws, partials=p2)
+        o.groupnorm(h2, h3, R, HW, w[path + ".norm2.g"], w[path + ".norm2.b"], eps, True, self.cfg.norm_groups, self._gnws, partials=p2, one_launch=self.gn_one)
         if (path + ".conv_shortcut.w") in w:
             sc = A.alloc(R * HW, cout)
             o.gemm(x, w[path + ".conv_shortcut.w"], sc, bias=w[path + ".conv_shortcut.b"])
@@ -451,7 +453,7 @@
         m = A.mark()
         g = A.alloc(R * T, C)
         o.groupnorm(x, g, R, T, w[path + ".norm.g"], w[path + ".norm.b"], 1e-6, False, self.cfg.norm_groups, self._gnws,
-                    partials=self._gn_of(x))
+                    partials=self._gn_of(x), one_launch=self.gn_one)
         h = A.alloc(R * T, C)
         lnst = None
         if self.ln_fold and depth > 0:
@@ -711,12 +713,20 @@
                 cx, cs = x.shape[1], sk.shape[1]
                 cat = A.alloc(R * h * wd, cx + cs)
                 add = down_res[k] if down_res is not None else None
+                pc = None
+                if self.cat_fuse and self.gn_fuse and (h * wd) % 64 == 0 and A.dtype == F16 and \
+                        (h * wd // 64) * ((cx + cs) // cfg.norm_groups) <= ops.GN_PARTIALS_MAX:
+                    pc = A.alloc(R * h * wd // 64 * (cx + cs), 4).view(torch.float32).view(R * h * wd // 64, cx + cs, 2)
                 if self.freeu is not None and i < 2:
                     s_f, b_f = self.freeu[i], self.freeu[2 + i]
                     parts = A.alloc(R * ops.FREEU_SLABS * 7, 2 * cs).view(torch.float32)
                     o.freeu_stats(sk, parts, h, wd, add=add, add_scale=res_scale if add is not None else None)
                     o.freeu_concat(x, sk, cat, parts, h, wd, b_f, s_f, mid_add=pending_mid, add=add,
-                                   add_scale=res_scale if (add is not None or pending_mid is not None) else None)
+                                   add_scale=res_scale if (add is not None or pending_mid is not None) else None, gn_out=pc)
+                    pending_mid = None
+                elif pc is not None:
+                    o.concat_gn(x, sk, cat, pc, mid_add=pending_mid, add=add,
+                                add_scale=res_scale if (add is not None or pending_mid is not None) else None, rows_per_scale=h * wd)
                     pending_mid = None
                 else:
                     o.copy_add(x, cat, 0, add=pending_mid, add_scale=res_scale if pending_mid is not None else None,
@@ -724,6 +734,8 @@
                     pending_mid = None
                     o.copy_add(sk, cat, cx, add=add, add_scale=res_scale if down_res is not None else None,
                                rows_per_scale=h * wd)
+                if pc is not None:
+                    cat._gn_parts = pc
                 x = self._resnet(f"up_blocks.{i}.resnets.{j}", cat, R, h, wd, temb_all)
                 if depth[i] > 0:
                     x = self._transformer(f"up_blocks.{i}.attentions.{j}", x, depth[i], R, h, wd, st, ada)
@@ -735,7 +747,7 @@
         c0 = cfg.block_out_channels[0]
         g = A.alloc(R * h * wd, c0)
         o.groupnorm(x, g, R, h * wd, w["conv_norm_out.g"], w["conv_norm_out.b"], 1e-5, True, cfg.norm_groups, self._gnws,
-                    partials=self._gn_of(x))
+                    partials=self._gn_of(x), one_launch=self.gn_one)
         eps = A.alloc(R * h * wd, cfg.out_channels)
         o.conv2d(g.view(R, h, wd, c0), w["conv_out.w"], eps, bias=w["conv_out.b"])
         return eps
diff --git a/instantir_amd/lib.py b/instantir_amd/lib.py
--- a/instantir_amd/lib.py
+++ b/instantir_amd/lib.py
@@ -106,6 +106,7 @@
     "iir_groupnorm_nhwc_f16": (C.c_int, [_P, _I64, _P, _I64, _I32, _I32, _I32, _I32, _P, _P, _F, _I32, _P, _I64, _P]),
     "iir_groupnorm_nhwc": (C.c_int, [_P, _I64, _P, _I64, _I32, _I32, _I32, _I32, _P, _P, _F, _I32, _P, _I64, _I32, _P]),
     "iir_groupnorm_from_partials": (C.c_int, [_P, _I64, _P, _I64, _P, _I64, _I32, _I32, _I32, _I32, _P, _P, _F, _I32, _P, _I64, _I32, _P]),
+    "iir_groupnorm_one_launch": (C.c_int, [_I32, _I32, _I32, _I32]),
     "iir_groupnorm_workspace_bytes": (C.c_int64, [_I32, _I32]),
     "iir_layernorm_f16": (C.c_int, [_P, _I64, _P, _I64, _I32, _I32, _P, _P, _F, _P, _P, _I64, _I32, _I32, _I32, _I64, _P]),
     "iir_adaln_batch_f16": (C.c_int, [_P, _I32, _I32, _I32, _F, _I64, _I32, _I32, _I64, _P]),
@@ -118,6 +119,9 @@
     "iir_freeu_stats_f16": (C.c_int, [_P, _I64, _P, _I64, _P, _I64, _I32, _I32, _I32, _P, _I64, _P]),
     "iir_freeu_concat_f16": (C.c_int, [_P, _I64, _I32, _P, _I64, _P, _I64, _I32, _P, _I64, _P, _I64, _I32, _I32, _F, _F, _P, _I64,
                                        _P, _I64, _I64, _P]),
+    "iir_freeu_concat_gn_f16": (C.c_int, [_P, _I64, _I32, _P, _I64, _P, _I64, _I32, _P, _I64, _P, _I64, _I32, _I32, _F, _F, _P, _I64,
+                                          _P, _I64, _I64, _P, _P]),
+    "iir_concat_gn_f16": (C.c_int, [_P, _I64, _I32, _P, _I64, _P, _I64, _I32, _P, _I64, _P, _I64, _I32, _P, _I64, _P, _P]),
     "iir_pack_latent": (C.c_int, [_P, _I32, _I32, _I32, _P, _I64, _I32, _F, _P]),
     "iir_unpack_latent": (C.c_int, [_P, _I64, _I32, _I32, _I32, _P, _P]),
     "iir_pack_latent_t": (C.c_int, [_P, _I32, _I32, _I32, _P, _I64, _I32, _F, _I32, _P]),
diff --git a/instantir_amd/ops.py b/instantir_amd/ops.py
--- a/instantir_amd/ops.py
+++ b/instantir_amd/ops.py
@@ -206,7 +206,8 @@
     return L.load().iir_gemm_ln_parts(M, N, K)
 
 
-GN_PARTIALS_MAX = 20 * 256
+GN_SILU, GN_TWO_LAUNCH = 1, 2
+GN_PARTIALS_MAX = 30 * 256
 
 
 def gn_supported(M, N, K, conv=False):
@@ -430,12 +431,17 @@
     return torch.empty(L.load().iir_groupnorm_workspace_bytes(R, groups) // 4, dtype=torch.float32, device=device)
 
 
-def groupnorm(x, out, R, HW, gamma, beta, eps, silu, groups=32, ws=None, partials=None):
+def gn_one_launch(R, HW, C, groups=32):
+    return bool(L.load().iir_groupnorm_one_launch(R, HW, C, groups))
+
+
+def groupnorm(x, out, R, HW, gamma, beta, eps, silu, groups=32, ws=None, partials=None, one_launch=True):
     dt = x.dtype
     _chk2d(x, "x", dt if dt in _DT else torch.float16); _chk2d(out, "out", dt)
     if gamma.dtype != dt or beta.dtype != dt:
         raise ValueError(f"gamma / beta must have the activations' dtype ({dt})")
     Cc = x.shape[1]
+    flags = (GN_SILU if silu else 0) | (0 if one_launch else GN_TWO_LAUNCH)
     if ws is None:
         ws = _gn_workspace(x.device, R, groups)
     if partials is not None:
@@ -444,11 +450,11 @@
             raise ValueError(f"groupnorm(partials=): images of whole 64-row slabs and at most {GN_PARTIALS_MAX} partials per (image, group); "
                              f"got HW={HW}, {Cc // groups} channels per group")
         L.check(L.load().iir_groupnorm_from_partials(partials.data_ptr(), Cc, x.data_ptr(), x.stride(0), out.data_ptr(), out.stride(0),
-                                                     R, HW, Cc, groups, gamma.data_ptr(), beta.data_ptr(), eps, int(silu), ws.data_ptr(),
+                                                     R, HW, Cc, groups, gamma.data_ptr(), beta.data_ptr(), eps, flags, ws.data_ptr(),
                                                      ws.numel() * 4, _DT[dt], _stream()), "iir_groupnorm_from_partials")
         return out
     L.check(L.load().iir_groupnorm_nhwc(x.data_ptr(), x.stride(0), out.data_ptr(), out.stride(0), R, HW, Cc, groups,
-                                        gamma.data_ptr(), beta.data_ptr(), eps, int(silu), ws.data_ptr(),
+                                        gamma.data_ptr(), beta.data_ptr(), eps, flags & ~GN_TWO_LAUNCH, ws.data_ptr(),
                                         ws.numel() * 4, _DT[dt], _stream()), "iir_groupnorm_nhwc")
     return out
 
@@ -506,6 +512,20 @@
     return dst
 
 
+def concat_gn(x, skip, dst, gn_out, mid_add=None, add=None, add_scale=None, rows_per_scale=1):
+    _chk2d(x, "x"); _chk2d(skip, "skip"); _chk2d(dst, "dst")
+    M, cx = x.shape
+    cs = skip.shape[1]
+    if skip.shape[0] != M or dst.shape[0] != M or dst.shape[1] != cx + cs:
+        raise ValueError("concat_gn: x, skip and dst must have the same rows, dst cx + cs columns")
+    _chk_gn_out(gn_out, M, cx + cs)
+    L.check(L.load().iir_concat_gn_f16(x.data_ptr(), x.stride(0), cx, _p(mid_add), mid_add.stride(0) if mid_add is not None else 0,
+                                       skip.data_ptr(), skip.stride(0), cs, _p(add), add.stride(0) if add is not None else 0,
+                                       _p(add_scale), M, rows_per_scale, dst.data_ptr(), dst.stride(0), gn_out.data_ptr(), _stream()),
+            "iir_concat_gn_f16")
+    return dst
+
+
 FREEU_SLABS = 16
 
 
@@ -525,16 +545,20 @@
     return partials
 
 
-def freeu_concat(x, skip, dst, partials, H, W, b, s, dst_off=0, mid_add=None, add=None, add_scale=None):
+def freeu_concat(x, skip, dst, partials, H, W, b, s, dst_off=0, mid_add=None, add=None, add_scale=None, gn_out=None):
     _chk2d(x, "x"); _chk2d(skip, "skip"); _chk2d(dst, "dst")
     M, cx = x.shape
     cs = skip.shape[1]
     if skip.shape[0] != M or dst.shape[0] != M:
         raise ValueError("freeu_concat: x, skip and dst must have the same rows")
-    L.check(L.load().iir_freeu_concat_f16(x.data_ptr(), x.stride(0), cx, _p(mid_add), mid_add.stride(0) if mid_add is not None else 0,
+    if gn_out is not None:
+        _chk_gn_out(gn_out, M, cx + cs)
+        if dst_off or (H * W) % 64:
+            raise ValueError("freeu_concat(gn_out=): dst_off 0 and images of whole 64-row slabs")
+    L.check(L.load().iir_freeu_concat_gn_f16(x.data_ptr(), x.stride(0), cx, _p(mid_add), mid_add.stride(0) if mid_add is not None else 0,
                                           skip.data_ptr(), skip.stride(0), cs, _p(add), add.stride(0) if add is not None else 0,
                                           _p(add_scale), M, H, W, float(b), float(s), partials.data_ptr(), partials.numel() * 4,
-                                          dst.data_ptr(), dst.stride(0), dst_off, _stream()), "iir_freeu_concat_f16")
+                                          dst.data_ptr(), dst.stride(0), dst_off, _p(gn_out), _stream()), "iir_freeu_concat_gn_f16")
     return dst
 
 
diff --git a/instantir_amd/pipeline.py b/instantir_amd/pipeline.py
--- a/instantir_amd/pipeline.py
+++ b/instantir_amd/pipeline.py
@@ -328,7 +328,7 @@
     def _loop_for(self, B, rep, Hl, Wl, st, st_prev, st_agg, lq, reference_latents, previewer_scheduler, guidance_rescale, pag_on=False):
         nets = (self._unet, self._unet_prev, self._agg)
         key = (B, rep, Hl, Wl, reference_latents is not None, float(guidance_rescale or 0.0), self.use_graphs, self.overlap_streams,
-               self.overlap_sft, tuple(None if n is None else (id(n), n.arena_gen, n.inkernel_prefetch, n.gn_fuse) for n in nets),
+               self.overlap_sft, tuple(None if n is None else (id(n), n.arena_gen, n.inkernel_prefetch, n.gn_fuse, n.gn_one, n.cat_fuse) for n in nets),
                self._freeu,
                _sched_form(self.scheduler),
                self._pag_paths if pag_on else None)
```

New measurement: 17.78, median of 6. Within noise of the previous version (+0.5%).
